# Algy/fast-slic

Hardware: AMD Instinct MI355X
Metric: megapixels/sec @10 iters (1280x720 & 4K, K=1600); % HBM roofline (higher is better)
Workload: dtype u8/u16/i32 (integer SLIC); 1 GPU; 1280x720 RGB, K=1600, 10 iters (configs[1]), 8 frames/GPU; frames_per_gpu=8, global_frames=8, slots_per_gpu=6, submissions_per_launch_group=up to 2 (dynamic batching of the pipeline), inputs=device-resident uint8 RGB, device int16 labels, parallelism=frames sharded across GPUs, no collective

## Files before the change

### fast_slic_amd/_binding.py

```python
import ctypes as C
import os
import subprocess
import threading

import numpy as np

ARCH_NAME = "hip/gfx950"
_HERE = os.path.dirname(os.path.abspath(__file__))
_LIB_PATH = os.path.join(_HERE, "libfslic_hip.so")

CLUSTER_DTYPE = np.dtype([
    ("y", "<f4"), ("x", "<f4"), ("r", "<f4"), ("g", "<f4"), ("b", "<f4"), ("a", "<f4"),
    ("number", "<u2"), ("is_active", "u1"), ("is_updatable", "u1"), ("num_members", "<u4"),
])
assert CLUSTER_DTYPE.itemsize == 32

FSLIC_OK, FSLIC_E_INVALID, FSLIC_E_UNSUPPORTED, FSLIC_E_HIP, FSLIC_E_INTERNAL = range(5)


class Params(C.Structure):
    _fields_ = [
        ("max_iter", C.c_int32), ("compactness", C.c_float), ("min_size_factor", C.c_float),
        ("subsample_stride", C.c_int32), ("convert_to_lab", C.c_int32),
        ("manhattan_spatial_dist", C.c_int32), ("preemptive", C.c_int32),
        ("preemptive_thres", C.c_float), ("num_threads", C.c_int32), ("debug_mode", C.c_int32),
        ("abi", C.c_int32), ("variant", C.c_int32), ("reserved", C.c_int32 * 4),
    ]


EXPORTS = [
    "fslic_hip_device_count", "fslic_hip_create", "fslic_hip_destroy", "fslic_hip_initialize_clusters",
    "fslic_hip_iterate", "fslic_hip_iterate_device", "fslic_hip_iterate_batch", "fslic_hip_submit_group",
    "fslic_hip_wait_group", "fslic_hip_rgb_to_lab",
    "fslic_hip_enforce_connectivity", "fslic_hip_enforce_connectivity_nodes", "fslic_hip_last_prelabels", "fslic_hip_last_timing_report",
    "fslic_hip_last_device_times", "fslic_hip_set_launch_timing", "fslic_hip_last_assign_loop", "fslic_hip_last_group_frames", "fslic_hip_last_path", "fslic_hip_last_launch_mode", "fslic_hip_group_done", "fslic_hip_last_error", "fslic_hip_version",
    "fslic_hip_get_connectivity", "fslic_hip_knn_connectivity", "fslic_hip_get_mask_density", "fslic_hip_cluster_density_to_mask",
    "fslic_hip_pipeline_submit", "fslic_hip_pipeline_drain", "fslic_hip_pipeline_batching", "fslic_hip_last_host_topk_frames",
    "fslic_hip_separate_pass_redos", "fslic_hip_uncovered_redos", "fslic_hip_copy_bandwidth", "fslic_hip_last_recorder_report",
    "fslic_hip_debug_lsc_state", "fslic_hip_debug_forms_seen", "fslic_hip_debug_forms_all",
    "fslic_hip_crf_new", "fslic_hip_crf_free", "fslic_hip_crf_copy", "fslic_hip_crf_get_params", "fslic_hip_crf_set_params",
    "fslic_hip_crf_set_compat", "fslic_hip_crf_get_compat", "fslic_hip_crf_num_classes", "fslic_hip_crf_first_time",
    "fslic_hip_crf_last_time", "fslic_hip_crf_num_frames", "fslic_hip_crf_pop_frame", "fslic_hip_crf_push_frame", "fslic_hip_crf_frame",
    "fslic_hip_crf_frame_time", "fslic_hip_crf_frame_set_clusters", "fslic_hip_crf_frame_get_clusters",
    "fslic_hip_crf_frame_set_connectivity", "fslic_hip_crf_frame_set_connectivity_csr", "fslic_hip_crf_frame_get_connectivity",
    "fslic_hip_crf_frame_set_mask", "fslic_hip_crf_frame_set_proba", "fslic_hip_crf_frame_set_unbiased", "fslic_hip_crf_frame_set_unary",
    "fslic_hip_crf_frame_get_unary", "fslic_hip_crf_frame_spatial_energy", "fslic_hip_crf_frame_temporal_energy",
    "fslic_hip_crf_frame_get_inferred", "fslic_hip_crf_frame_reset_inferred", "fslic_hip_crf_initialize", "fslic_hip_crf_inference",
    "fslic_hip_crf_expf_host", "fslic_hip_crf_expf_device",
    "fslic_hip_pool_workspace_size", "fslic_hip_pool", "fslic_hip_pool_finalize", "fslic_hip_unpool",
    "fslic_hip_rag_workspace_size", "fslic_hip_rag_accumulate", "fslic_hip_rag_compact",
    "fslic_hip_overlap_workspace_size", "fslic_hip_overlap_accumulate", "fslic_hip_overlap_compact", "fslic_hip_boundary_match",
    "fslic_hip_crf_tensor_workspace_size", "fslic_hip_crf_tensor_inference",
    "fslic_hip_crf_tensor_grad_workspace_size", "fslic_hip_crf_tensor_inference_saved", "fslic_hip_crf_tensor_backward",
    "fslic_hip_crf_tensor_energies", "fslic_hip_crf_tensor_energies_backward_workspace_size", "fslic_hip_crf_tensor_energies_backward",
    "fslic_hip_crf_tensor_inference_energies", "fslic_hip_crf_tensor_inference_saved_energies", "fslic_hip_crf_tensor_backward_energies",
]

_lib = None
_lib_lock = threading.Lock()

FORM_FAMILIES = {1: "blk", 2: "bin", 3: "pre", 4: "k32", 5: "generic", 6: "generic_rec", 7: "preempt_update"}
FORM_TABLES = {0: "notab", 1: "rowvec", 2: "rowvec16", 3: "2d", 4: "tabs16", 5: "lut"}


def form_name(code):
    code = int(code)
    family = FORM_FAMILIES.get(code & 15, "family%d" % (code & 15))
    if family == "preempt_update":
        return family + (" allpairs" if (code >> 18) & 1 else " lists")
    stride = (code >> 11) & 7
    words = [family]
    if (code >> 4) & 63:
        words.append("r%d" % ((code >> 4) & 63))
    words += ["fused" if (code >> 10) & 1 else "full", "s%d" % stride if stride else "srt",
              FORM_TABLES.get((code >> 14) & 7, "table%d" % ((code >> 14) & 7)), "nolab" if (code >> 17) & 1 else "lab"]
    return " ".join(words)


def _form_codes(fn, *extra):
    buf = (C.c_uint32 * 256)()
    n = int(fn(buf, 256, *extra))
    if n < 0 or n > 256:
        raise RuntimeError("the form record cannot be read (%d)" % n)
    return [int(buf[i]) for i in range(n)]


def forms_seen(clear=False):
    return {form_name(c) for c in _form_codes(load_library().fslic_hip_debug_forms_seen, 1 if clear else 0)}


def forms_all():
    return [form_name(c) for c in _form_codes(load_library().fslic_hip_debug_forms_all)]


def form_codes_all():
    return _form_codes(load_library().fslic_hip_debug_forms_all)


def build_library(force=False):
    csrc = os.path.join(_HERE, "csrc")
    args = ["make", "-s", "-C", csrc]
    if force:
        args.append("-B")
    subprocess.check_call(args)
    return _LIB_PATH


def _preload_torch_hip_runtime():
    import importlib.util
    import sys
    if "torch" in sys.modules:
        return
    try:
        spec = importlib.util.find_spec("torch")
    except (ImportError, ValueError):
        spec = None
    if spec is None or not spec.origin:
        return
    cand = os.path.join(os.path.dirname(spec.origin), "lib", "libamdhip64.so")
    if os.path.exists(cand):
        try:
            C.CDLL(cand, mode=C.RTLD_GLOBAL)
        except OSError:
            pass


def load_library():
    global _lib
    with _lib_lock:
        if _lib is not None:
            return _lib
        _preload_torch_hip_runtime()
        if not os.path.exists(_LIB_PATH):
            raise ImportError(
                "fast_slic_amd: %s is missing; build it with `python -c 'import __graft_entry__ as g; g.build()'` "
                "or `make -C fast_slic_amd/csrc` (there is no CPU fallback)" % _LIB_PATH)
        lib = C.CDLL(os.environ.get("FSLIC_LIB") or _LIB_PATH)
        vp, i32 = C.c_void_p, C.c_int
        lib.fslic_hip_device_count.restype = i32
        lib.fslic_hip_create.argtypes = [i32, i32, C.POINTER(vp)]
        lib.fslic_hip_destroy.argtypes = [vp]
        lib.fslic_hip_destroy.restype = None
        lib.fslic_hip_initialize_clusters.argtypes = [i32, i32, i32, vp, vp]
        lib.fslic_hip_iterate.argtypes = [vp, C.POINTER(Params), i32, i32, i32, vp, vp, vp]
        lib.fslic_hip_iterate_device.argtypes = [vp, i32, C.POINTER(Params), i32, i32, i32, vp, vp, vp]
        lib.fslic_hip_iterate_batch.argtypes = [vp, C.POINTER(Params), i32, i32, i32, i32, vp, vp, vp, i32]
        lib.fslic_hip_submit_group.argtypes = [vp, i32, C.POINTER(Params), i32, i32, i32, i32, vp, vp, vp]
        lib.fslic_hip_wait_group.argtypes = [vp, i32]
        lib.fslic_hip_pipeline_submit.argtypes = [vp, C.POINTER(Params), i32, i32, i32, i32, vp, vp, vp]
        lib.fslic_hip_pipeline_drain.argtypes = [vp, C.POINTER(C.c_double), C.POINTER(C.c_longlong), C.POINTER(C.c_longlong), C.POINTER(C.c_longlong)]
        lib.fslic_hip_pipeline_batching.argtypes = [vp, i32]
        lib.fslic_hip_last_host_topk_frames.argtypes = [vp, i32]
        lib.fslic_hip_separate_pass_redos.argtypes = [vp, i32]
        if hasattr(lib, "fslic_hip_uncovered_redos"):
            lib.fslic_hip_uncovered_redos.argtypes = [vp, i32]
        if hasattr(lib, "fslic_hip_copy_bandwidth"):
            lib.fslic_hip_copy_bandwidth.argtypes = [vp, C.c_size_t, i32, C.POINTER(C.c_double)]
        lib.fslic_hip_group_done.argtypes = [vp, i32]
        lib.fslic_hip_rgb_to_lab.argtypes = [vp, i32, i32, vp, i32, vp]
        lib.fslic_hip_enforce_connectivity.argtypes = [vp, vp, i32, i32, i32, i32]
        if hasattr(lib, "fslic_hip_enforce_connectivity_nodes"):
            lib.fslic_hip_enforce_connectivity_nodes.argtypes = [vp, vp, i32, i32, i32, i32, C.POINTER(C.c_uint32)]
        lib.fslic_hip_last_prelabels.argtypes = [vp, i32, vp]
        if hasattr(lib, "fslic_hip_debug_lsc_state"):
            lib.fslic_hip_debug_lsc_state.argtypes = [vp, i32, i32, i32, vp, vp]
        if hasattr(lib, "fslic_hip_debug_forms_seen"):
            lib.fslic_hip_debug_forms_seen.argtypes = [vp, i32, i32]
            lib.fslic_hip_debug_forms_all.argtypes = [vp, i32]
        lib.fslic_hip_last_timing_report.argtypes = [vp]
        lib.fslic_hip_last_timing_report.restype = C.c_char_p
        if hasattr(lib, "fslic_hip_last_recorder_report"):
            lib.fslic_hip_last_recorder_report.argtypes = [vp, C.POINTER(C.c_char_p), C.POINTER(C.c_size_t)]
        lib.fslic_hip_last_device_times.argtypes = [vp, i32, C.POINTER(C.c_float), C.POINTER(C.c_float)]
        lib.fslic_hip_set_launch_timing.argtypes = [vp, i32]
        lib.fslic_hip_last_assign_loop.argtypes = [vp, i32, C.POINTER(C.c_float), C.POINTER(C.c_double), C.POINTER(C.c_int)]
        lib.fslic_hip_last_group_frames.argtypes = [vp, i32]
        lib.fslic_hip_last_path.argtypes = [vp, i32]
        lib.fslic_hip_last_launch_mode.argtypes = [vp, i32]
        if hasattr(lib, "fslic_hip_lab_force_generic"):
            lib.fslic_hip_lab_force_generic.argtypes = [vp, i32]
        lib.fslic_hip_last_error.restype = C.c_char_p
        lib.fslic_hip_version.restype = C.c_char_p
        lib.fslic_hip_get_connectivity.argtypes = [vp, i32, i32, i32, vp, vp, vp]
        lib.fslic_hip_knn_connectivity.argtypes = [i32, i32, i32, vp, C.c_size_t, vp, vp]
        lib.fslic_hip_get_mask_density.argtypes = [vp, i32, i32, i32, vp, vp, vp, vp]
        lib.fslic_hip_cluster_density_to_mask.argtypes = [vp, i32, i32, i32, vp, vp, vp]
        if hasattr(lib, "fslic_hip_crf_new"):
            _declare_crf(lib)
        if hasattr(lib, "fslic_hip_pool"):
            _declare_pool(lib)
        if hasattr(lib, "fslic_hip_rag_accumulate"):
            _declare_rag(lib)
        if hasattr(lib, "fslic_hip_overlap_accumulate"):
            _declare_compare(lib)
        if hasattr(lib, "fslic_hip_crf_tensor_inference"):
            _declare_crf_tensor(lib)
        _lib = lib
        return lib


def _declare_crf(lib):
    vp, i32, sz, f32 = C.c_void_p, C.c_int, C.c_size_t, C.c_float
    for name, args in [
        ("new", [sz, sz, C.POINTER(vp)]), ("copy", [vp, C.POINTER(vp)]), ("get_params", [vp, vp]), ("set_params", [vp, vp]),
        ("set_compat", [vp, i32, f32]), ("get_compat", [vp, i32, C.POINTER(f32)]), ("num_classes", [vp, C.POINTER(sz), C.POINTER(sz)]),
        ("first_time", [vp]), ("last_time", [vp]), ("pop_frame", [vp]), ("push_frame", [vp, C.POINTER(vp)]),
        ("frame", [vp, i32, C.POINTER(vp)]), ("frame_time", [vp]), ("frame_set_clusters", [vp, vp]), ("frame_get_clusters", [vp, vp]),
        ("frame_set_connectivity", [vp, i32, vp, vp, sz]), ("frame_set_connectivity_csr", [vp, i32, vp, vp]),
        ("frame_get_connectivity", [vp, vp, vp]), ("frame_set_mask", [vp, vp, f32]), ("frame_set_proba", [vp, vp]),
        ("frame_set_unbiased", [vp]), ("frame_set_unary", [vp, vp]), ("frame_get_unary", [vp, vp]),
        ("frame_spatial_energy", [vp, i32, i32, C.POINTER(f32)]), ("frame_temporal_energy", [vp, vp, i32, C.POINTER(f32)]),
        ("frame_get_inferred", [vp, vp]), ("frame_reset_inferred", [vp]), ("initialize", [vp]), ("inference", [vp, vp, sz]),
        ("expf_host", [vp, vp, sz, i32]), ("expf_device", [vp, vp, vp, sz]),
    ]:
        f = getattr(lib, "fslic_hip_crf_" + name)
        f.argtypes = args
        f.restype = i32
    lib.fslic_hip_crf_free.argtypes = [vp]
    lib.fslic_hip_crf_free.restype = None
    lib.fslic_hip_crf_num_frames.argtypes = [vp]
    lib.fslic_hip_crf_num_frames.restype = sz


def _declare_pool(lib):
    vp, i32 = C.c_void_p, C.c_int
    lib.fslic_hip_pool_workspace_size.argtypes = [i32, i32, i32, i32, C.POINTER(C.c_size_t)]
    lib.fslic_hip_pool.argtypes = [i32, vp, i32, i32, i32, i32, i32, i32, vp, vp, i32, vp, C.c_size_t]
    lib.fslic_hip_pool_finalize.argtypes = [i32, vp, i32, i32, i32, i32, vp, C.c_size_t, vp, vp, vp]
    lib.fslic_hip_unpool.argtypes = [i32, vp, i32, i32, i32, i32, i32, vp, vp, i32, vp, C.c_float, vp]
    for name in ("pool_workspace_size", "pool", "pool_finalize", "unpool"):
        getattr(lib, "fslic_hip_" + name).restype = i32


def _declare_rag(lib):
    vp, i32, i64, sz = C.c_void_p, C.c_int, C.c_longlong, C.c_size_t
    lib.fslic_hip_rag_workspace_size.argtypes = [i32, i32, i32, i64, C.POINTER(sz)]
    lib.fslic_hip_rag_accumulate.argtypes = [i32, vp, i32, i32, i32, i32, i32, vp, i32, vp, i32, i64, vp, sz]
    lib.fslic_hip_rag_compact.argtypes = [i32, vp, i32, i32, i64, vp, sz, vp, vp, vp, i64]
# ... 108 lines not shown
        _check(load_library().fslic_hip_get_connectivity(self._h, H, W, int(K), ptr, num.ctypes.data, nb.ctypes.data))
        return num, nb

    def get_mask_density(self, clusters, labels, mask, H, W):
        lp, k1 = self._plane(labels, np.uint16)
        mp, k2 = self._plane(mask, np.uint8)
        cl = np.ascontiguousarray(clusters)
        dens = np.zeros(cl.shape[0], np.uint8)
        _check(load_library().fslic_hip_get_mask_density(self._h, H, W, cl.shape[0], cl.ctypes.data, lp, mp, dens.ctypes.data))
        return dens

    def cluster_density_to_mask(self, labels, densities, H, W, out=None):
        lp, k1 = self._plane(labels, np.uint16)
        d = np.ascontiguousarray(densities, dtype=np.uint8)
        if out is None:
            res = np.empty((H, W), np.uint8)
            op = C.c_void_p(res.ctypes.data)
        else:
            res, op = out, C.c_void_p(int(out))
        _check(load_library().fslic_hip_cluster_density_to_mask(self._h, H, W, d.shape[0], lp, d.ctypes.data, op))
        return res

    def iterate(self, image, clusters, params):
        H, W, _ = image.shape
        labels = np.empty((H, W), np.uint16)
        _check(load_library().fslic_hip_iterate(self._h, C.byref(params), H, W, clusters.shape[0],
                                                image.ctypes.data, clusters.ctypes.data, labels.ctypes.data))
        return labels

    def iterate_device(self, d_rgb_ptr, d_labels_ptr, H, W, clusters, params, slot=0):
        _check(load_library().fslic_hip_iterate_device(self._h, int(slot), C.byref(params), H, W, clusters.shape[0],
                                                       C.c_void_p(d_rgb_ptr), clusters.ctypes.data, C.c_void_p(d_labels_ptr)))

    def iterate_batch(self, rgb_ptrs, cluster_arrays, label_ptrs, H, W, params, device_ptrs):
        n = len(rgb_ptrs)
        K = cluster_arrays[0].shape[0]
        PA = C.c_void_p * n
        a_rgb = PA(*[C.c_void_p(int(p)) for p in rgb_ptrs])
        a_cl = PA(*[C.c_void_p(c.ctypes.data) for c in cluster_arrays])
        a_lab = PA(*[C.c_void_p(int(p)) for p in label_ptrs])
        _check(load_library().fslic_hip_iterate_batch(self._h, C.byref(params), H, W, K, n,
                                                      C.cast(a_rgb, C.c_void_p), C.cast(a_cl, C.c_void_p),
                                                      C.cast(a_lab, C.c_void_p), int(bool(device_ptrs))))

    @staticmethod
    def pointer_array(ptrs):
        PA = C.c_void_p * len(ptrs)
        return PA(*[C.c_void_p(int(p)) for p in ptrs])

    def submit_group(self, slot, a_rgb, a_clusters, a_labels, n, H, W, K, params):
        _check(load_library().fslic_hip_submit_group(self._h, int(slot), C.byref(params), H, W, K, n,
                                                     C.cast(a_rgb, C.c_void_p), C.cast(a_clusters, C.c_void_p),
                                                     C.cast(a_labels, C.c_void_p)))

    def wait_group(self, slot):
        _check(load_library().fslic_hip_wait_group(self._h, int(slot)))

    def pipeline_submit(self, a_rgb, a_clusters, a_labels, n, H, W, K, params):
        _check(load_library().fslic_hip_pipeline_submit(self._h, C.byref(params), H, W, K, n,
                                                        C.cast(a_rgb, C.c_void_p), C.cast(a_clusters, C.c_void_p),
                                                        C.cast(a_labels, C.c_void_p)))

    def pipeline_batching(self, max_frames_per_group):
        _check(load_library().fslic_hip_pipeline_batching(self._h, int(max_frames_per_group)))

    def pipeline_drain(self):
        ms, g, f, h = C.c_double(), C.c_longlong(), C.c_longlong(), C.c_longlong()
        _check(load_library().fslic_hip_pipeline_drain(self._h, C.byref(ms), C.byref(g), C.byref(f), C.byref(h)))
        return {"device_ms": ms.value, "groups": g.value, "frames": f.value, "host_topk_frames": h.value}

    def last_host_topk_frames(self, slot=0):
        return int(load_library().fslic_hip_last_host_topk_frames(self._h, int(slot)))

    def separate_pass_redos(self):
        return sum(int(load_library().fslic_hip_separate_pass_redos(self._h, s)) for s in range(self.n_slots))

    def uncovered_redos(self, slot=None):
        lib = load_library()
        if not hasattr(lib, "fslic_hip_uncovered_redos"):
            return 0
        slots = range(self.n_slots) if slot is None else [int(slot)]
        return sum(int(lib.fslic_hip_uncovered_redos(self._h, s)) for s in slots)

    def copy_bandwidth(self, nbytes=1 << 30, reps=5):
        v = C.c_double()
        _check(load_library().fslic_hip_copy_bandwidth(self._h, C.c_size_t(int(nbytes)), int(reps), C.byref(v)))
        return v.value

    def group_done(self, slot):
        return load_library().fslic_hip_group_done(self._h, int(slot)) != 0

    def last_launch_mode(self, slot=0):
        return int(load_library().fslic_hip_last_launch_mode(self._h, int(slot)))

    def last_prelabels(self, H, W, slot=0):
        out = np.empty((H, W), np.uint16)
        _check(load_library().fslic_hip_last_prelabels(self._h, int(slot), out.ctypes.data))
        return out

    def debug_lsc_state(self, K, z=0, slot=0):
        means, cfeat = np.empty(10, np.float32), np.empty((int(K), 10), np.float32)
        _check(load_library().fslic_hip_debug_lsc_state(self._h, int(slot), int(z), int(K), means.ctypes.data, cfeat.ctypes.data))
        return means, cfeat

    def last_timing_report(self):
        return load_library().fslic_hip_last_timing_report(self._h).decode("utf-8")

    def last_recorder_report(self):
        p, n = C.c_char_p(), C.c_size_t()
        _check(load_library().fslic_hip_last_recorder_report(self._h, C.byref(p), C.byref(n)))
        return C.string_at(p, n.value) if n.value else b""

    def last_device_times(self, slot=0):
        t, f = C.c_float(), C.c_float()
        _check(load_library().fslic_hip_last_device_times(self._h, int(slot), C.byref(t), C.byref(f)))
        return t.value, f.value

    def set_launch_timing(self, on):
        _check(load_library().fslic_hip_set_launch_timing(self._h, int(bool(on))))

    def last_assign_loop(self, slot=0):
        ms, px, n = C.c_float(), C.c_double(), C.c_int()
        _check(load_library().fslic_hip_last_assign_loop(self._h, int(slot), C.byref(ms), C.byref(px), C.byref(n)))
        return ms.value, px.value, n.value

    def last_group_frames(self, slot=0):
        return load_library().fslic_hip_last_group_frames(self._h, int(slot))

    def last_path(self, slot=0):
        return load_library().fslic_hip_last_path(self._h, int(slot))

    def lab_force_generic(self, on):
        _check(load_library().fslic_hip_lab_force_generic(self._h, int(bool(on))))


_default_engines = {}
_engine_lock = threading.Lock()


DEFAULT_ENGINE_SLOTS = 8


def default_engine(device=0):
    with _engine_lock:
        e = _default_engines.get(device)
        if e is None:
            e = Engine(device, DEFAULT_ENGINE_SLOTS)
            _default_engines[device] = e
        return e


def device_count():
    return load_library().fslic_hip_device_count()


def is_supported_arch(arch_name):
    return arch_name == ARCH_NAME


def get_supported_archs():
    return [ARCH_NAME]


def make_params(max_iter, compactness, min_size_factor, subsample_stride, convert_to_lab=True,
                manhattan_spatial_dist=True, preemptive=False, preemptive_thres=0.05, num_threads=-1,
                debug_mode=False, variant=0):
# ... 202 lines not shown
```

### fast_slic_amd/csrc/arena.cpp

```cpp
#include "engine_internal.h"

#include <algorithm>
#include <cmath>

namespace fslic {

void free_slot(Slot& s) {
    for (auto& g : s.graphs) { if (g.exec) hipGraphExecDestroy(g.exec); if (g.graph) hipGraphDestroy(g.graph); }
    s.graphs.clear();
    for (auto& e : s.ev) if (e) hipEventDestroy(e);
    for (auto& e : s.ev_it) if (e) hipEventDestroy(e);
    if (s.st) hipStreamDestroy(s.st);
    s = Slot();
}

int prepare(fslic_engine* e, Slot& s, int H, int W, int K, int S, int G) {
    const size_t N = (size_t)H * W;
    const int sh = [&] { int v = 2; while ((1 << v) < S) v++; return v; }();
    const int ncx = (W + (1 << sh) - 1) >> sh, ncy = (H + (1 << sh) - 1) >> sh;
    const size_t ncell = (size_t)ncx * ncy;
    const size_t P = (size_t)(2 * S + 1);
    if (G < s.cap_frames && s.keyH == H && s.keyW == W && s.keyK == K) G = s.cap_frames;

    int rc;
    if ((rc = s.h_cl.reserve((size_t)G * 4 * K)) || (rc = s.h_misc.reserve((size_t)kStatusWords * kMaxGroup)) ||
        (rc = s.h_lut.reserve(kLutMaxWords)) || (rc = s.h_tab.reserve(3 * kTabMaxBytes / sizeof(uint16_t))) ||
        (rc = s.h_patchf.reserve(P * P)) || (rc = s.h_patch.reserve(P * P)))
        return rc;

    size_t off = 0;
    auto take = [&](size_t bytes) { size_t o = off; off = align_up(off + bytes, 256); return o; };
    const size_t o_patch = take(P * P * 2);
    const size_t o_lut = take(kLutMaxWords * 4);
    const size_t o_tab = take(3 * kTabMaxBytes);
    const size_t o_patchf = take(P * P * 4);
    const size_t shared_bytes = off;
    off = 0;
    const size_t o_lab = take(N * 4), o_labels = take(N * 2);
    const size_t o_cl = take((size_t)K * 4 * 8);
    const size_t o_clf = take((size_t)K * 8 * 4);
    const int pre_cw = (W + 2 * S - 1) / (2 * S), pre_ch = (H + 2 * S - 1) / (2 * S);
    const size_t o_pre = take(((size_t)K * 2 + (size_t)pre_cw * pre_ch + 16) * 4);
    auto pow2ceil = [](int v) { int p2 = 1; while (p2 < v) p2 <<= 1; return p2; };
    const int nbx = pow2ceil(2 * S / 64 + 2), nby = pow2ceil(2 * S / 16 + 2);
    const size_t o_cpart = take((size_t)K * nbx * nby * 6 * 4);
    const size_t o_zero = off;
    const size_t o_sums = take((size_t)K * 6 * 4), o_sums1 = take((size_t)K * 6 * 4);
    const size_t o_cc0 = take(ncell * 4), o_cc1 = take(ncell * 4);
    const size_t o_misc = take(256);
    const size_t o_arrive = take((size_t)K * 4);
    const size_t zero_bytes = off - o_zero;
    const size_t o_ci0 = take(ncell * kCellCap * sizeof(ClusterRec)), o_ci1 = take(ncell * kCellCap * sizeof(ClusterRec));
    const size_t o_ov0 = take((size_t)K * sizeof(ClusterRec)), o_ov1 = take((size_t)K * sizeof(ClusterRec)), o_ov2 = take((size_t)K * sizeof(ClusterRec));
    const size_t ntiles = (size_t)((W + kCcaTile - 1) / kCcaTile) * ((H + kCcaTileH - 1) / kCcaTileH);
    const size_t TT = (size_t)kCcaTilePx;
    const size_t NP = ntiles * TT;
    const size_t o_lid = take(N * 2), o_nrec = take(NP * 16), o_narea = take(NP * 4);
    const size_t o_nfinal = take(NP * 2), o_vedge = take(ntiles * 2 * kCcaTileH * 4), o_roots = take(NP * 4);
    const size_t o_candl = take(ntiles * TT * 4), o_canda = take(ntiles * TT * 4);
    const size_t o_keepl = take((size_t)K * 4), o_keepb = take((size_t)K * 2);
    const size_t o_rgb = take(N * 3), o_out = take(N * 2);
    const size_t frame_bytes = off;
    const size_t total = shared_bytes + frame_bytes * (size_t)G;

    if ((rc = s.arena.reserve(total))) return rc;
    s.cap_frames = G;
    s.frame_bytes = frame_bytes;
    char* b = s.arena + shared_bytes;
    FrameDev& f = s.f;
    f.frame_bytes = frame_bytes;
    f.H = H; f.W = W; f.N = (int)N; f.K = K; f.S = S; f.T = 2 * S + 32; f.T_rcp = 0xFFFFFFFFu / (uint32_t)f.T;
    f.cs_shift = sh; f.ncx = ncx; f.ncy = ncy; f.ncell = (int)ncell;
    f.lab = (uint32_t*)(b + o_lab);
    f.labels = (uint16_t*)(b + o_labels);
    uint32_t* cl = (uint32_t*)(b + o_cl);
    f.cl_yx = cl; f.cl_lab = cl + K; f.cl_n = cl + 2 * (size_t)K; f.cl_moved = cl + 3 * (size_t)K; f.cl_tag = cl + 4 * (size_t)K;
    f.cl_shadow = cl + 5 * (size_t)K;
    f.cl_f = nullptr;
    f.cl_upd = f.cl_act = f.cell_act = f.pre_flags = nullptr;
    f.pre_cw = pre_cw; f.pre_ch = pre_ch;
    s.d_pre = (uint32_t*)(b + o_pre);
    s.d_clf = (float*)(b + o_clf);
    s.d_yx_alt[0] = cl + 6 * (size_t)K; s.d_yx_alt[1] = cl + 7 * (size_t)K;
    f.cl_yx_out = s.d_yx_alt[0];
    f.cpart = (uint32_t*)(b + o_cpart); f.cpart_ns = nbx * nby; f.nbx = nbx;
    f.sums[0] = (uint32_t*)(b + o_sums); f.sums[1] = (uint32_t*)(b + o_sums1);
    f.cell_cnt[0] = (uint32_t*)(b + o_cc0); f.cell_cnt[1] = (uint32_t*)(b + o_cc1);
    uint32_t* misc = (uint32_t*)(b + o_misc);
    s.d_misc = misc;
    f.ovf_cnt[0] = misc + kStSpill0; f.ovf_cnt[1] = misc + kStSpill1; f.err_flag = misc + kStFlags; f.ovf_cnt[2] = misc + kStSpill2;
    f.cl_arrive = (uint32_t*)(b + o_arrive);
    f.cell_items[0] = (ClusterRec*)(b + o_ci0); f.cell_items[1] = (ClusterRec*)(b + o_ci1);
    f.ovf_items[0] = (ClusterRec*)(b + o_ov0); f.ovf_items[1] = (ClusterRec*)(b + o_ov1); f.ovf_items[2] = (ClusterRec*)(b + o_ov2);
    s.d_patch = (uint16_t*)(s.arena + o_patch);
    f.patch2d = s.d_patch;
    s.d_lut = (uint32_t*)(s.arena + o_lut);
    s.d_tab = (uint16_t*)(s.arena + o_tab);
    s.d_patchf = (float*)(s.arena + o_patchf);
    s.pf_variant = -1;
    s.zero_block = b + o_zero; s.zero_bytes = zero_bytes;
    CcaDev& c = s.c;
    c.frame_bytes = frame_bytes;
    c.H = H; c.W = W; c.N = (int)N; c.K = K;
    c.tiles_x = (W + kCcaTile - 1) / kCcaTile;
    c.lid = (uint16_t*)(b + o_lid); c.nrec = (uint4*)(b + o_nrec); c.narea = (uint32_t*)(b + o_narea);
    c.nfinal = (uint16_t*)(b + o_nfinal); c.vedge = (uint32_t*)(b + o_vedge); c.roots = (uint32_t*)(b + o_roots);
    c.counters = misc + kStCca;
    c.cand_leader = (int32_t*)(b + o_candl); c.cand_area = (uint32_t*)(b + o_canda);
#if defined(FSLIC_LAB) && FSLIC_LAB == 4
    f.lab_stamps = c.cand_area;
#endif
    s.d_keep_leader = (int32_t*)(b + o_keepl); s.d_keep_label = (uint16_t*)(b + o_keepb);
    s.d_rgb_stage = (uint8_t*)(b + o_rgb); s.d_out_stage = (uint16_t*)(b + o_out);
    s.keyH = H; s.keyW = W; s.keyK = K;
    s.sp_valid = false;
    (void)e;
    if (knobs().poison) HIPCHK(hipMemsetAsync(s.arena, 0xA5, total, s.st));
    s.stamp_block = b + o_ci0; s.stamp_bytes = o_ov0 - o_ci0;
    HIPCHK(hipMemset2DAsync(s.stamp_block, frame_bytes, 0, s.stamp_bytes, (size_t)G, s.st));
    return FSLIC_OK;
}

int ensure_prepared(fslic_engine* e, Slot& s, int H, int W, int K, int S, int G) {
    G = std::max(G, std::min(e->reserve_frames.load(), (int)kMaxGroup));
    if (s.keyH == H && s.keyW == W && s.keyK == K && s.cap_frames >= G) return FSLIC_OK;
    HIPCHK(hipStreamSynchronize(s.st));
    return prepare(e, s, H, W, K, S, G);
}

int prepare_lsc(Slot& s, int H, int W, int K, int S, int G, float compactness) {
    const size_t lut_floats = 1024 + 2 * (size_t)W + 2 * (size_t)H;
    if (s.lsc_H != H || s.lsc_W != W || s.lsc_K != K || s.lsc_G < G) {
        G = std::max(G, (s.lsc_H == H && s.lsc_W == W && s.lsc_K == K) ? s.lsc_G : 0);
        size_t off = 0;
        auto take = [&](size_t bytes) { size_t o = off; off = align_up(off + bytes, 256); return o; };
        const size_t o_lut = take(lut_floats * 4);
        const size_t shared_bytes = off;
        off = 0;
        const size_t o_hist = take(768 * 4), o_extra = take((size_t)K * kLscExPitch * 8);
        const size_t zero_bytes = off - o_hist;
        const size_t o_means = take(64), o_cfeat = take((size_t)K * kLscCfPitch * 4);
        const size_t frame_bytes = off, total = shared_bytes + frame_bytes * (size_t)G;
        int rc;
        if ((rc = s.lsc_arena.reserve(total)) || (rc = s.h_lsc_lut.reserve(lut_floats))) return rc;
        char* b = s.lsc_arena + shared_bytes;
        LscDev& l = s.l;
        l.frame_bytes = frame_bytes;
        l.hist = (uint32_t*)(b + o_hist); l.extra = (long long*)(b + o_extra);
        l.means = (float*)(b + o_means); l.cfeat = (float*)(b + o_cfeat);
        const float* lut = (const float*)(s.lsc_arena + o_lut);
        l.lut_color = lut; l.lut_x = lut + 1024; l.lut_y = lut + 1024 + 2 * (size_t)W;
        s.lsc_zero = b + o_hist; s.lsc_zero_bytes = zero_bytes; s.lsc_frame_bytes = frame_bytes;
        s.lsc_H = H; s.lsc_W = W; s.lsc_K = K; s.lsc_G = G;
        s.lsc_S = 0;
        if (knobs().poison) HIPCHK(hipMemsetAsync(s.lsc_arena, 0xA5, total, s.st));
    }
    if (s.lsc_S != S || s.lsc_compactness != compactness) {
        const float C_color = 20.0f;
        const float PI = 3.1415926f, halfPI = PI / 2;
        const float ratio = compactness / 100.0f;
        const float C_spatial = C_color * ratio;
        float* t = s.h_lsc_lut;
        for (int X = 0; X < 256; X++) {
            const float theta = halfPI * (X / 255.0f);
            const float cosine = (float)cos((double)theta), sine = (float)sin((double)theta);
            t[512 + X] = C_color * cosine * 2.55f;
            t[768 + X] = C_color * sine * 2.55f;
            t[X] = (float)((double)C_color * cos((double)theta));
            t[256 + X] = (float)((double)C_color * sin((double)theta));
        }
        float* tx = t + 1024;
        float* ty = tx + 2 * (size_t)W;
        const float step = halfPI / S;
        for (int i = 0; i < W; i++) {
            const float theta = i * step;
            tx[i] = (float)((double)C_spatial * cos((double)theta));
            tx[W + i] = (float)((double)C_spatial * sin((double)theta));
        }
        for (int i = 0; i < H; i++) {
            const float theta = i * step;
            ty[i] = (float)((double)C_spatial * cos((double)theta));
            ty[H + i] = (float)((double)C_spatial * sin((double)theta));
        }
        HIPCHK(hipMemcpyAsync(const_cast<float*>(s.l.lut_color), t, lut_floats * 4, hipMemcpyHostToDevice, s.st));
        const double f_max = std::max({(double)C_color, (double)C_color * 2.55, (double)fabsf(C_spatial)});
        const double w_max = 2.0 * C_color * C_color + 4.0 * (C_color * 2.55) * (C_color * 2.55) + 4.0 * (double)C_spatial * C_spatial;
        int bits_f = 20, bits_w = 12;
        while (bits_f > 0 && 1024.0 * f_max * ldexp(1.0, bits_f) >= 2147483648.0) bits_f--;
        const double w_bias = ceil(4.0 * (double)C_spatial * C_spatial);
        while (bits_w > 0 && 1024.0 * (w_max + w_bias) * ldexp(1.0, bits_w) >= 4294967296.0) bits_w--;
        s.l.blk_bias_w = (float)w_bias;
        s.l.blk_fix_f = (float)ldexp(1.0, bits_f); s.l.blk_fix_w = (float)ldexp(1.0, bits_w);
        s.l.blk_shift_f = 20 - bits_f; s.l.blk_shift_w = 12 - bits_w;
        s.lsc_S = S; s.lsc_compactness = compactness;
    }
    return FSLIC_OK;
}

}
```

### fast_slic_amd/csrc/capi.cpp

```cpp
#include "engine_internal.h"
#include "crf.h"
#include "forms.h"

#include <algorithm>
#include <cstdio>
#include <cstdlib>
#include <cstring>
#include <mutex>

using namespace fslic;

static_assert(sizeof(fslic_cluster) == 32, "Cluster ABI (src/fast-slic-common.h:10-23)");

extern "C" {

const char* fslic_hip_last_error(void) { return last_error().c_str(); }
const char* fslic_hip_version(void) { return "fast_slic_amd 0.3 (gfx950)"; }

int fslic_hip_device_count(void) {
    int n = 0;
    if (hipGetDeviceCount(&n) != hipSuccess) return 0;
    return n;
}

int fslic_hip_create(int device, int n_slots, fslic_engine** out) {
    if (!out) return fail(FSLIC_E_INVALID, "out is NULL");
    *out = nullptr;
    if (n_slots < 1 || n_slots > 64) return fail(FSLIC_E_INVALID, "n_slots must be in [1, 64]");
    int n = 0;
    HIPCHK(hipGetDeviceCount(&n));
    if (device < 0 || device >= n) return fail(FSLIC_E_HIP, "no such HIP device");
    HIPCHK(hipSetDevice(device));
    const HostTables& ht = host_tables();
    fslic_engine* e = new fslic_engine();
    e->device = device;
    e->group_size = knobs().group_size;
    e->slots.resize(n_slots);
    for (auto& s : e->slots) {
        if (hipStreamCreateWithFlags(&s.st, hipStreamNonBlocking) != hipSuccess) { fslic_hip_destroy(e); return fail(FSLIC_E_HIP, "hipStreamCreate failed"); }
        for (auto& ev : s.ev)
            if (hipEventCreate(&ev) != hipSuccess) { fslic_hip_destroy(e); return fail(FSLIC_E_HIP, "hipEventCreate failed"); }
        for (auto& ev : s.ev_it)
            if (hipEventCreate(&ev) != hipSuccess) { fslic_hip_destroy(e); return fail(FSLIC_E_HIP, "hipEventCreate failed"); }
        if (s.d_ptrs.reserve(2 * kMaxGroup) || s.h_ptrs.reserve(2 * kMaxGroup) ||
            s.d_gen.reserve(64) || hipMemset(s.d_gen, 0, 256) != hipSuccess) { fslic_hip_destroy(e); return fail(FSLIC_E_HIP, "pointer table allocation failed"); }
    }
    if (e->d_gamma.reserve(sizeof ht.gamma / sizeof ht.gamma[0]) || e->d_labtbl.reserve(sizeof ht.lab / sizeof ht.lab[0])) { fslic_hip_destroy(e); return fail(FSLIC_E_HIP, "hipMalloc(tables) failed"); }
    if (hipMemcpy(e->d_gamma, ht.gamma, sizeof ht.gamma, hipMemcpyHostToDevice) != hipSuccess ||
        hipMemcpy(e->d_labtbl, ht.lab, sizeof ht.lab, hipMemcpyHostToDevice) != hipSuccess) { fslic_hip_destroy(e); return fail(FSLIC_E_HIP, "table upload failed"); }
    e->tables.gamma = e->d_gamma;
    e->tables.labtbl = e->d_labtbl;
    for (int i = 0; i < 9; i++) e->tables.cb[i] = ht.cb[i];
    *out = e;
    return FSLIC_OK;
}

void fslic_hip_destroy(fslic_engine* e) {
    if (!e) return;
    hipSetDevice(e->device);
    for (auto& s : e->slots) stop_slot_thread(e, s);
    for (auto& s : e->slots) {
        if (s.st) hipStreamSynchronize(s.st);
        free_slot(s);
    }
    delete e;
}

static int iterate_on(fslic_engine* e, Slot& s, const fslic_params* p, int H, int W, int K,
                      const uint8_t* d_rgb, fslic_cluster* clusters, uint16_t* d_labels) {
    GroupJob job;
    int rc = fill_job(job, p, H, W, K, 1, &d_rgb, &clusters, &d_labels);
    if (rc) return rc;
    s.launch_timing = e->launch_timing;
    rc = run_group(e, s, job, p->debug_mode != 0);
    if (rc) return rc;
    std::string report;
    rc = make_recorder_report(s, report);
    if (rc) { drain_failed(s); return rc; }
    set_thread_timing_report(make_timing_report(s));
    set_thread_recorder_report(std::move(report));
    return FSLIC_OK;
}

int fslic_hip_iterate_device(fslic_engine* e, int slot, const fslic_params* p, int H, int W, int K,
                             const uint8_t* d_rgb, fslic_cluster* clusters, uint16_t* d_labels) {
    if (!e) return fail(FSLIC_E_INVALID, "engine is NULL");
    if (slot < 0 || slot >= (int)e->slots.size()) return fail(FSLIC_E_INVALID, "slot out of range");
    HIPCHK(hipSetDevice(e->device));
    SlotLease lease(e);
    const int rc = lease.take(slot);
    return rc ? rc : iterate_on(e, e->slots[slot], p, H, W, K, d_rgb, clusters, d_labels);
}

int fslic_hip_iterate(fslic_engine* e, const fslic_params* p, int H, int W, int K, const uint8_t* rgb,
                      fslic_cluster* clusters, uint16_t* labels) {
    if (!e) return fail(FSLIC_E_INVALID, "engine is NULL");
    if (!rgb || !labels || !clusters) return fail(FSLIC_E_INVALID, "NULL pointer argument");
    HIPCHK(hipSetDevice(e->device));
    int S = 0;
    int rc = validate(p, H, W, K, S);
    if (rc) return rc;
    SlotLease lease(e);
    rc = lease.take();
    if (rc) return rc;
    Slot& s = e->slots[lease.slot];
    const size_t N = (size_t)H * W;
    rc = ensure_prepared(e, s, H, W, K, S, 1);
    if (rc) return rc;
    const double t0 = knobs().host_timing ? now_us() : 0.0;
    HIPCHK(hipMemcpyAsync(s.d_rgb_stage, rgb, N * 3, hipMemcpyHostToDevice, s.st));
    const double t1 = knobs().host_timing ? now_us() : 0.0;
    rc = iterate_on(e, s, p, H, W, K, s.d_rgb_stage, clusters, s.d_out_stage);
    if (rc) return rc;
    const double t2 = s.t_begun_us, t3 = knobs().host_timing ? now_us() : 0.0;
    HIPCHK(hipMemcpyAsync(labels, s.d_out_stage, N * 2, hipMemcpyDeviceToHost, s.st));
    HIPCHK(hipStreamSynchronize(s.st));
    if (knobs().host_timing)
        fprintf(stderr, "[fslic host] iterate: frame in %.1f us, group begin %.1f, group finish (wait + write-back) %.1f, labels out %.1f (device %.1f us)\n",
                t1 - t0, t2 - t1, t3 - t2, now_us() - t3, s.total_ms * 1e3);
    return FSLIC_OK;
}

int fslic_hip_last_recorder_report(fslic_engine* e, const char** report, size_t* length) {
    (void)e;
    if (!report || !length) return fail(FSLIC_E_INVALID, "NULL pointer argument");
    const std::string& r = thread_recorder_report();
    *report = r.c_str();
// ... 53 lines not shown
                break;
            }
        Slot& s = e->slots[si];
        GroupJob& job = jobs[(size_t)(first / G)];
        if (!device_ptrs) {
            rc = ensure_prepared(e, s, H, W, K, S, n);
            if (rc) return bail(rc);
            for (int i = 0; i < n; i++) {
                if (hipMemcpyAsync(s.at(s.d_rgb_stage, i), rgb[first + i], N * 3, hipMemcpyHostToDevice, s.st) != hipSuccess)
                    return bail(fail(FSLIC_E_HIP, "frame upload failed"));
                job.d_rgb[i] = s.at(s.d_rgb_stage, i);
                job.d_out[i] = s.at(s.d_out_stage, i);
            }
        }
        s.launch_timing = e->launch_timing;
        inflight.push_back({si, first, n});
        rc = group_begin(e, s, job);
        if (rc) return bail(rc);
    }
    while (!inflight.empty()) {
        const Pending pd = inflight.front();
        inflight.erase(inflight.begin());
        rc = finish_one(pd);
        if (rc) return bail(rc);
    }
    if (n_frames > 0) set_thread_timing_report(make_timing_report(e->slots[0]));
    release_all_slots(e);
    return FSLIC_OK;
}

int fslic_hip_last_prelabels(fslic_engine* e, int slot, uint16_t* prelabels) {
    if (!e || !prelabels) return fail(FSLIC_E_INVALID, "NULL pointer argument");
    if (slot < 0 || slot >= (int)e->slots.size()) return fail(FSLIC_E_INVALID, "slot out of range");
    HIPCHK(hipSetDevice(e->device));
    SlotLease lease(e);
    int rc = lease.take(slot);
    if (rc) return rc;
    Slot& s = e->slots[slot];
    if (!s.have_pre || s.keyH == 0) return fail(FSLIC_E_INVALID, "no frame has been processed on this slot");
    HIPCHK(hipMemcpy(prelabels, s.f.labels, (size_t)s.f.N * 2, hipMemcpyDeviceToHost));
    return FSLIC_OK;
}

int fslic_hip_debug_lsc_state(fslic_engine* e, int slot, int z, int K, float* means10, float* cfeat) {
    if (!e || !means10 || !cfeat) return fail(FSLIC_E_INVALID, "NULL pointer argument");
    if (slot < 0 || slot >= (int)e->slots.size()) return fail(FSLIC_E_INVALID, "slot out of range");
    HIPCHK(hipSetDevice(e->device));
    SlotLease lease(e);
    int rc = lease.take(slot);
    if (rc) return rc;
    Slot& s = e->slots[slot];
    if (!s.have_pre || s.keyH == 0 || s.p.variant != FSLIC_VARIANT_LSC) return fail(FSLIC_E_INVALID, "the slot's last group was not an LSC one");
    if (z < 0 || z >= s.nframes) return fail(FSLIC_E_INVALID, "no such frame in the slot's last group");
    if (K != s.K) return fail(FSLIC_E_INVALID, "K is not that of the slot's last group");
    HIPCHK(hipStreamSynchronize(s.st));
    LscDev l = s.l;
    l.select(z);
    HIPCHK(hipMemcpy(means10, l.means, sizeof(float) * kLscFeat, hipMemcpyDeviceToHost));
    HIPCHK(hipMemcpy2D(cfeat, sizeof(float) * kLscFeat, l.cfeat, sizeof(float) * kLscCfPitch, sizeof(float) * kLscFeat, (size_t)s.K, hipMemcpyDeviceToHost));
    return FSLIC_OK;
}

const char* fslic_hip_last_timing_report(fslic_engine* e) { return e ? thread_timing_report().c_str() : ""; }

int fslic_hip_last_device_times(fslic_engine* e, int slot, float* total_ms, float* full_assign_ms) {
    if (!e || slot < 0 || slot >= (int)e->slots.size()) return fail(FSLIC_E_INVALID, "bad engine/slot");
    if (total_ms) *total_ms = e->slots[slot].total_ms;
    if (full_assign_ms) *full_assign_ms = e->slots[slot].fa_ms;
    return FSLIC_OK;
}

int fslic_hip_set_launch_timing(fslic_engine* e, int on) {
    if (!e) return fail(FSLIC_E_INVALID, "engine is NULL");
    e->launch_timing = on != 0;
    return FSLIC_OK;
}

int fslic_hip_lab_force_generic(fslic_engine* e, int on) {
    if (!e) return fail(FSLIC_E_INVALID, "engine is NULL");
    e->lab_force_generic.store(on != 0);
    return FSLIC_OK;
}

int fslic_hip_last_assign_loop(fslic_engine* e, int slot, float* sum_ms, double* visited_px, int* launches) {
    if (!e || slot < 0 || slot >= (int)e->slots.size()) return fail(FSLIC_E_INVALID, "bad engine/slot");
    const Slot& s = e->slots[slot];
    if (sum_ms) *sum_ms = s.assign_loop_ms;
    if (visited_px) *visited_px = s.assign_loop_px;
    if (launches) *launches = s.n_timed_iters;
    return FSLIC_OK;
}

int fslic_hip_last_group_frames(fslic_engine* e, int slot) {
    if (!e || slot < 0 || slot >= (int)e->slots.size()) return -1;
    return e->slots[slot].nframes;
}

int fslic_hip_last_launch_mode(fslic_engine* e, int slot) {
    if (!e || slot < 0 || slot >= (int)e->slots.size()) return -1;
    return e->slots[slot].last_launch_mode;
}

int fslic_hip_last_path(fslic_engine* e, int slot) {
    if (!e || slot < 0 || slot >= (int)e->slots.size()) return -1;
    return e->slots[slot].last_path;
}

int fslic_hip_last_host_topk_frames(fslic_engine* e, int slot) {
    if (!e || slot < 0 || slot >= (int)e->slots.size()) return -1;
    return e->slots[slot].n_host_topk;
}

int fslic_hip_separate_pass_redos(fslic_engine* e, int slot) {
    if (!e || slot < 0 || slot >= (int)e->slots.size()) return -1;
    return __atomic_load_n(&e->slots[slot].n_separate_redo, __ATOMIC_RELAXED);
}

int fslic_hip_uncovered_redos(fslic_engine* e, int slot) {
    if (!e || slot < 0 || slot >= (int)e->slots.size()) return -1;
    return __atomic_load_n(&e->slots[slot].n_uncovered_redo, __ATOMIC_RELAXED);
}

int fslic_hip_debug_forms_seen(uint32_t* codes, int cap, int clear) {
    if (cap < 0 || (cap > 0 && !codes)) return -1;
    return fslic::forms_seen(codes, cap, clear != 0);
}

int fslic_hip_debug_forms_all(uint32_t* codes, int cap) {
    if (cap < 0 || (cap > 0 && !codes)) return -1;
    const int na = fslic::assign_forms(codes, cap);
    return na + fslic::preempt_forms(codes + std::min(na, cap), std::max(cap - na, 0));
}

#define CRF_LOCK(crf) std::lock_guard<std::mutex> crf_lock__((crf)->mu)

static fslic_crf_frame* crf_frame_at(fslic_crf* crf, int time) {
    if (crf->frames.empty()) return nullptr;
    const long long d = (long long)time - crf->frames.front()->time;
    if (d < 0 || d >= (long long)crf->frames.size()) return nullptr;
    return crf->frames[(size_t)d].get();
}
static void crf_touch_unary(fslic_crf_frame* f) { f->dirty_unary = true; }
static void crf_touch_q(fslic_crf_frame* f) { f->q_on_device = false; f->dirty_q = true; }

int fslic_hip_crf_new(size_t num_classes, size_t num_nodes, fslic_crf** out) {
    if (!out) return fail(FSLIC_E_INVALID, "out is NULL");
    *out = nullptr;
    if (num_classes == 0 || num_nodes == 0) return fail(FSLIC_E_INVALID, "num_classes and num_nodes must be positive");
    if (num_classes >= (1ull << 31) || num_nodes >= (1ull << 31) || (unsigned long long)num_classes * num_nodes >= (1ull << 31))
        return fail(FSLIC_E_INVALID, "num_classes * num_nodes must be below 2^31");
    fslic_crf* crf = new fslic_crf();
    crf->C = num_classes;
    crf->K = num_nodes;
    crf->compat.assign(num_classes, 1.0f);
    crf->params.spatial_w = 10; crf->params.temporal_w = 10;
    crf->params.spatial_srgb = 13; crf->params.temporal_srgb = 13;
    crf->params.spatial_sxy = 80;
    crf->params.spatial_smooth_w = 0; crf->params.spatial_smooth_sxy = 3;
    *out = crf;
    return FSLIC_OK;
}

void fslic_hip_crf_free(fslic_crf* crf) {
    if (!crf) return;
    crf_release_device(crf);
    delete crf;
}

int fslic_hip_crf_copy(fslic_crf* crf, fslic_crf** out) {
    if (!crf || !out) return fail(FSLIC_E_INVALID, "NULL pointer argument");
    *out = nullptr;
    CRF_LOCK(crf);
    for (auto& f : crf->frames) {
        int rc = crf_pull_q(crf, f.get());
        if (rc) return rc;
    }
    fslic_crf* c = new fslic_crf();
    c->C = crf->C; c->K = crf->K; c->next_time = crf->next_time; c->compat = crf->compat; c->params = crf->params;
    for (auto& f : crf->frames) {
        std::unique_ptr<fslic_crf_frame> g(new fslic_crf_frame());
        g->parent = c; g->time = f->time; g->clusters = f->clusters; g->edges = f->edges; g->unaries = f->unaries; g->q = f->q;
        c->frames.push_back(std::move(g));
    }
    *out = c;
    return FSLIC_OK;
}

int fslic_hip_crf_get_params(fslic_crf* crf, fslic_crf_params* out) {
    if (!crf || !out) return fail(FSLIC_E_INVALID, "NULL pointer argument");
    CRF_LOCK(crf);
    *out = crf->params;
    return FSLIC_OK;
}

int fslic_hip_crf_set_params(fslic_crf* crf, const fslic_crf_params* params) {
    if (!crf || !params) return fail(FSLIC_E_INVALID, "NULL pointer argument");
    CRF_LOCK(crf);
    crf->params = *params;
    return FSLIC_OK;
}

int fslic_hip_crf_set_compat(fslic_crf* crf, int cls, float compat_value) {
    if (!crf) return fail(FSLIC_E_INVALID, "NULL pointer argument");
// ... 279 lines not shown
```

### fast_slic_amd/csrc/cca.hip

```cpp
#include "device_common.h"

namespace fslic {

constexpr uint32_t kNoAdopt = 0xFFFFFFFFu;
static __device__ __forceinline__ uint32_t* n_parent(const CcaDev& c, uint32_t n) { return reinterpret_cast<uint32_t*>(c.nrec + n); }
static __device__ __forceinline__ uint32_t n_leader(const CcaDev& c, uint32_t n) { return reinterpret_cast<const uint32_t*>(c.nrec + n)[1]; }
static __device__ __forceinline__ uint32_t n_local(const CcaDev& c, uint32_t n) { return reinterpret_cast<const uint32_t*>(c.nrec + n)[2]; }
static __device__ __forceinline__ uint32_t n_adopt(const CcaDev& c, uint32_t n) { return reinterpret_cast<const uint32_t*>(c.nrec + n)[3]; }

static __device__ __forceinline__ uint32_t lds_ld(uint32_t* p) {
    return __hip_atomic_load(p, __ATOMIC_RELAXED, __HIP_MEMORY_SCOPE_WORKGROUP);
}
static __device__ __forceinline__ void lds_st(uint32_t* p, uint32_t v) {
    __hip_atomic_store(p, v, __ATOMIC_RELAXED, __HIP_MEMORY_SCOPE_WORKGROUP);
}
typedef unsigned long long u64;
static __device__ __forceinline__ uint32_t lane_left0(uint32_t v) { return (uint32_t)__builtin_amdgcn_update_dpp(0, (int)v, 0x138 , 0xF, 0xF, true); }
static __device__ __forceinline__ uint32_t lane_left_or(uint32_t old, uint32_t v) { return (uint32_t)__builtin_amdgcn_update_dpp((int)old, (int)v, 0x138, 0xF, 0xF, false); }
static __device__ __forceinline__ uint32_t rank_in(u64 m) { return __builtin_amdgcn_mbcnt_hi((uint32_t)(m >> 32), __builtin_amdgcn_mbcnt_lo((uint32_t)m, 0u)); }
static __device__ __forceinline__ uint32_t* lds_at(uint32_t* base, uint32_t off) { return reinterpret_cast<uint32_t*>(reinterpret_cast<char*>(base) + off); }
static __device__ __forceinline__ void ldsb_union(uint32_t* par, uint32_t a, uint32_t b) {
    for (;;) {
        for (;;) {
            const uint32_t pa = lds_ld(lds_at(par, a)), pb = lds_ld(lds_at(par, b));
// ... 804 lines not shown
    if (cap > kSelCap) cap = kSelCap;
    const size_t lds = (3 * (size_t)cap + 3 * (size_t)kSelBuckets) * sizeof(uint32_t);
    static_assert(kSelBins <= 3 * kSelBuckets, "the selection histogram reuses the ranking buckets");
    static std::atomic<int> attr_state[64];
    if (!max_dynamic_lds_on_this_device(k_cca_select, (int)((3 * (size_t)kSelCap + 3 * (size_t)kSelBuckets) * sizeof(uint32_t)), attr_state)) {
        while (cap > 1024 && (3 * (size_t)cap + 3 * (size_t)kSelBuckets) * sizeof(uint32_t) > 64 * 1024) cap >>= 1;
        const size_t lds_small = (3 * (size_t)cap + 3 * (size_t)kSelBuckets) * sizeof(uint32_t);
        launch(k_cca_select, dim3(nframes), dim3(1024), lds_small, st, c, cap);
        return;
    }
    launch(k_cca_select, dim3(nframes), dim3(1024), lds, st, c, cap);
}

__global__ __launch_bounds__(256) void k_cca_reset_final(CcaDev c) {
    const uint32_t n = c.counters[0];
    for (uint32_t i = blockIdx.x * blockDim.x + threadIdx.x; i < n; i += gridDim.x * blockDim.x) {
        const uint32_t r = c.roots[i];
        if (*n_parent(c, r) == r) c.nfinal[r] = 0xFFFFu;
    }
}
__global__ void k_cca_set_kept(CcaDev c, const int32_t* __restrict__ leaders, const uint16_t* __restrict__ labels, int n) {
    const int i = blockIdx.x * blockDim.x + threadIdx.x;
    if (i < n) c.nfinal[node_of(c, (uint32_t)leaders[i])] = labels[i];
}
__global__ void k_cca_gather_area(CcaDev c) {
    const uint32_t M = c.counters[1];
    for (uint32_t i = blockIdx.x * blockDim.x + threadIdx.x; i < M; i += gridDim.x * blockDim.x) c.cand_area[i] = c.narea[node_of(c, (uint32_t)c.cand_leader[i])];
}
void launch_cca_gather_area(const CcaDev& c, hipStream_t st) {
    launch(k_cca_gather_area, dim3(64), dim3(256), 0, st, c);
}

void launch_cca_set_kept(const CcaDev& c, const int32_t* d_leaders, const uint16_t* d_labels, int n, hipStream_t st) {
    launch(k_cca_reset_final, dim3(root_pass_blocks(c)), dim3(256), 0, st, c);
    if (n <= 0) return;
    launch(k_cca_set_kept, dim3((n + 255) / 256), dim3(256), 0, st, c, d_leaders, d_labels, n);
}

static __device__ __forceinline__ uint32_t chase_final(const CcaDev& c, uint32_t g) {
    const uint32_t W = (uint32_t)c.W;
    for (;;) {
        const uint32_t cur = n_leader(c, g);
        if (cur == 0) return 0u;
        uint32_t a = n_adopt(c, g);
        if (a == kNoAdopt) {
            const uint32_t t = (cur % W > 0) ? cur - 1 : cur - W;
            a = node_of(c, t);
        }
        g = *n_parent(c, a);
        const uint32_t f = __hip_atomic_load(c.nfinal + g, __ATOMIC_RELAXED, __HIP_MEMORY_SCOPE_AGENT);
        if (f != 0xFFFFu) return f;
    }
}

__global__ __launch_bounds__(256) void k_cca_chain(CcaDev c) {
    c.select(blockIdx.y);
    const uint32_t i0 = blockIdx.x * blockDim.x + threadIdx.x;
    const uint32_t r0 = c.roots[i0];
    const uint32_t n = c.counters[0];
    const uint32_t gstride = gridDim.x * blockDim.x;
    for (uint32_t i = i0; i < n; i += gstride) {
        const uint32_t r = i == i0 ? r0 : c.roots[i];
        const uint32_t g = *n_parent(c, r);
        uint32_t f = __hip_atomic_load(c.nfinal + g, __ATOMIC_RELAXED, __HIP_MEMORY_SCOPE_AGENT);
        if (f == 0xFFFFu) f = chase_final(c, g);
        __hip_atomic_store(c.nfinal + r, (uint16_t)f, __ATOMIC_RELAXED, __HIP_MEMORY_SCOPE_AGENT);
    }
}

static __device__ __forceinline__ uint32_t wave_max_u32(uint32_t v) {
#define FSLIC_DPP_MAX(ctrl) v = max(v, (uint32_t)__builtin_amdgcn_update_dpp(0, (int)v, ctrl, 0xF, 0xF, false))
    FSLIC_DPP_MAX(0xB1); FSLIC_DPP_MAX(0x4E); FSLIC_DPP_MAX(0x141); FSLIC_DPP_MAX(0x140);
#undef FSLIC_DPP_MAX
    return max(max((uint32_t)__builtin_amdgcn_readlane((int)v, 0), (uint32_t)__builtin_amdgcn_readlane((int)v, 16)),
               max((uint32_t)__builtin_amdgcn_readlane((int)v, 32), (uint32_t)__builtin_amdgcn_readlane((int)v, 48)));
}

__global__ __launch_bounds__(256) void k_cca_relabel(CcaDev c, ExportDev ex, int relabel_blocks) {
    const int z = blockIdx.y;
    if ((int)blockIdx.x >= relabel_blocks) {
        const size_t d = (size_t)z * ex.frame_bytes;
        const uint32_t* yx = ex.yx_cur; const uint32_t* rest = ex.lab_n_moved; const uint32_t* misc = ex.misc0;
        FrameDev::adv(yx, d); FrameDev::adv(rest, d); FrameDev::adv(misc, d);
        uint32_t* out = ex.h_cl + (size_t)z * ex.h_stride;
        const int K = ex.K;
        for (int i = ((int)blockIdx.x - relabel_blocks) * blockDim.x + threadIdx.x; i < 4 * K; i += ((int)gridDim.x - relabel_blocks) * blockDim.x)
            out[i] = i < K ? yx[i] : rest[i - K];
        if ((int)blockIdx.x == relabel_blocks && threadIdx.x < kStatusWords) ex.h_misc[kStatusWords * (size_t)z + threadIdx.x] = misc[threadIdx.x];
        return;
    }
    c.select(z);
    constexpr int T = kCcaTile, TH = kCcaTileH;
    const int tiles_x = c.tiles_x, tiles_y = (c.H + TH - 1) / TH;
    const int ntiles = tiles_x * tiles_y;
    const int aligned8 = ((reinterpret_cast<uintptr_t>(c.out) & 7) == 0) ? 1 : 0;
    const bool vec = (c.W & 3) == 0 && aligned8;
    __shared__ __attribute__((aligned(16))) uint16_t s_fin[kCcaTilePx];
    __shared__ uint32_t s_max;
    for (int tile = blockIdx.x; tile < ntiles; tile += relabel_blocks) {
        const int ty = tile / tiles_x, tx = tile - ty * tiles_x;
        const uint16_t* __restrict__ gfin = c.nfinal + (size_t)tile * kCcaTilePx;
        const int x0 = tx * T + 4 * (int)(threadIdx.x & 15);
        const int r0 = (int)(threadIdx.x >> 4);
        if (tile != (int)blockIdx.x) __syncthreads();
        if (threadIdx.x == 0) s_max = 0u;
        __syncthreads();
        if (vec) {
            uint2 v[2];
            bool ok[2];
            uint32_t mx = 0;
#pragma unroll
            for (int h = 0; h < 2; ++h) {
                const int y = ty * TH + r0 + 16 * h;
                ok[h] = y < c.H && x0 < c.W;
                v[h] = make_uint2(0u, 0u);
                if (ok[h]) v[h] = *reinterpret_cast<const uint2*>(c.lid + (size_t)y * c.W + x0);
                mx = max(max(mx, max(v[h].x & 0xFFFFu, v[h].x >> 16)), max(v[h].y & 0xFFFFu, v[h].y >> 16));
            }
            mx = wave_max_u32(mx);
            if ((threadIdx.x & 63) == 0) atomicMax(&s_max, mx);
            __syncthreads();
            const uint32_t cnt = min(s_max + 1u, (uint32_t)kCcaTilePx);
            for (uint32_t i = threadIdx.x; i * 8u < cnt; i += 256u) reinterpret_cast<uint4*>(s_fin)[i] = reinterpret_cast<const uint4*>(gfin)[i];
            __syncthreads();
#pragma unroll
            for (int h = 0; h < 2; ++h) {
                if (!ok[h]) continue;
                const int y = ty * TH + r0 + 16 * h;
                uint2 o;
                o.x = (uint32_t)s_fin[v[h].x & 0xFFFFu] | ((uint32_t)s_fin[v[h].x >> 16] << 16);
                o.y = (uint32_t)s_fin[v[h].y & 0xFFFFu] | ((uint32_t)s_fin[v[h].y >> 16] << 16);
                st_stream(reinterpret_cast<uint2*>(c.out + (size_t)y * c.W + x0), o);
            }
        } else {
#pragma unroll
            for (int h = 0; h < 2; ++h) {
                const int y = ty * TH + r0 + 16 * h;
                if (y >= c.H) continue;
                for (int q = 0; q < 4; ++q) {
                    const int x = x0 + q;
                    if (x < c.W) st_stream(c.out + (size_t)y * c.W + x, gfin[c.lid[(size_t)y * c.W + x]]);
                }
            }
        }
    }
}

void launch_cca_phase2(const CcaDev& c, int nframes, hipStream_t st, const ExportDev* ex_) {
    launch(k_cca_chain, dim3(root_pass_blocks(c), nframes), dim3(256), 0, st, c);
    int blocks = c.tiles_x * ((c.H + kCcaTileH - 1) / kCcaTileH);
    const int cap = (16384 + nframes - 1) / nframes;
    if (blocks > cap) blocks = cap;
    if (blocks < 1) blocks = 1;
    ExportDev ex{};
    if (ex_) ex = *ex_;
    const int eb = ex.K > 0 ? (4 * ex.K + 1023) / 1024 : 0;
    launch(k_cca_relabel, dim3(blocks + eb, nframes), dim3(256), 0, st, c, ex, blocks);
}

}
```

### fast_slic_amd/csrc/engine_internal.h

```cpp
#pragma once
#include "kernels.h"
#include "launch.h"
#include "../../include/fslic_hip.h"

#include <algorithm>
#include <atomic>
#include <condition_variable>
#include <deque>
#include <cstdint>
#include <memory>
#include <mutex>
#include <string>
#include <thread>
#include <vector>

namespace fslic {

int fail(int code, const std::string& msg);
const std::string& last_error();
void set_last_error(const std::string& msg);

#define HIPCHK(expr)                                                                            \
    do {                                                                                        \
        hipError_t e__ = (expr);                                                                \
        if (e__ != hipSuccess)                                                                  \
            return ::fslic::fail(FSLIC_E_HIP, std::string(#expr) + ": " + hipGetErrorString(e__)); \
    } while (0)

inline int clampi(int v, int lo, int hi) { return v < lo ? lo : (v > hi ? hi : v); }
inline float clampf(float v, float lo, float hi) { return v < lo ? lo : (v > hi ? hi : v); }
inline size_t align_up(size_t v, size_t a) { return (v + a - 1) / a * a; }
double now_us();

template <class T, bool kDevice>
class Buffer {
    T* p_ = nullptr;
    size_t cap_ = 0;
public:
    Buffer() = default;
    Buffer(Buffer&& o) noexcept : p_(o.p_), cap_(o.cap_) { o.p_ = nullptr; o.cap_ = 0; }
    Buffer& operator=(Buffer&& o) noexcept { std::swap(p_, o.p_); std::swap(cap_, o.cap_); return *this; }
    ~Buffer() { release(); }
    operator T*() const { return p_; }
    T* get() const { return p_; }
    void release() {
        if (p_) (void)(kDevice ? hipFree(p_) : hipHostFree(p_));
        p_ = nullptr; cap_ = 0;
    }
    int reserve(size_t count) {
        if (p_ && cap_ >= count) return FSLIC_OK;
        release();
        const size_t bytes = std::max<size_t>(count * sizeof(T), 16);
        const hipError_t err = kDevice ? hipMalloc((void**)&p_, bytes) : hipHostMalloc((void**)&p_, bytes);
        if (err != hipSuccess) {
            p_ = nullptr;
            return fail(FSLIC_E_HIP, std::string(kDevice ? "hipMalloc(" : "hipHostMalloc(") + std::to_string(bytes) + " bytes): " + hipGetErrorString(err));
        }
        cap_ = count;
        return FSLIC_OK;
    }
};
template <class T> using Pinned = Buffer<T, false>;
template <class T> using Device = Buffer<T, true>;

struct GroupJob {
    fslic_params p{};
    int H = 0, W = 0, K = 0, n = 0;
    const uint8_t* d_rgb[kMaxGroup] = {};
    fslic_cluster* clusters[kMaxGroup] = {};
    uint16_t* d_out[kMaxGroup] = {};
    void append(const GroupJob& j) {
        for (int i = 0; i < j.n; i++) { d_rgb[n + i] = j.d_rgb[i]; clusters[n + i] = j.clusters[i]; d_out[n + i] = j.d_out[i]; }
        n += j.n;
    }
};

struct Knobs {
    int group_size;
    bool use_graphs, poison, host_timing;
    int fuse_bin;
    int blocks_scale;
};
const Knobs& knobs();

constexpr int kDenseCap = 8192;
constexpr size_t kTabMaxBytes = 40960;
constexpr size_t kLutMaxWords = 12288;

struct HostTables {
    uint16_t gamma[256];
    uint16_t lab[8194];
    int cb[9];
};
const HostTables& host_tables();

struct Slot {
    hipStream_t st = nullptr;
    hipEvent_t ev[6] = {nullptr, nullptr, nullptr, nullptr, nullptr, nullptr};
    static constexpr int kMaxTimedIters = 16;
    hipEvent_t ev_it[2 * kMaxTimedIters] = {};
    int n_timed_iters = 0;
    float assign_loop_ms = 0;
    double assign_loop_px = 0;
    Device<char> arena;
    int cap_frames = 0;
    size_t frame_bytes = 0;
    FrameDev f{};
    CcaDev c{};
    char* zero_block = nullptr;
    size_t zero_bytes = 0;
    char* stamp_block = nullptr;
    size_t stamp_bytes = 0;
    uint32_t* d_misc = nullptr;
    uint32_t* d_yx_alt[2] = {nullptr, nullptr};
    uint8_t* d_rgb_stage = nullptr;
    uint16_t* d_out_stage = nullptr;
    int32_t* d_keep_leader = nullptr;
    uint16_t* d_keep_label = nullptr;
    Device<void*> d_ptrs;
    Pinned<void*> h_ptrs;
    uint16_t* d_patch = nullptr;
    uint32_t* d_lut = nullptr;
    Pinned<uint32_t> h_lut;
    uint16_t* d_tab = nullptr;
    Pinned<uint16_t> h_tab;
    Pinned<uint32_t> h_cl;
    Pinned<uint32_t> h_misc;
    Pinned<uint16_t> h_patch;
    Pinned<int32_t> h_cand_leader;
    Pinned<uint32_t> h_cand_area;
    Device<uint32_t> d_gen;
    uint64_t gen_host = 0;
    uint32_t gen_span_prev = 0;
    uint32_t gen_step = 0;
    int keyH = 0, keyW = 0, keyK = 0;
    struct GraphEntry {
        std::vector<unsigned char> key;
        hipGraph_t graph = nullptr;
        hipGraphExec_t exec = nullptr;
        int seen = 0;
        bool failed = false;
    };
    std::vector<GraphEntry> graphs;
    int last_launch_mode = 0;
    bool launch_timing = false;
    double t_begun_us = 0;
    bool nap_wait = false;
    double recent_wait_us[4] = {1e30, 1e30, 1e30, 1e30};
    unsigned recent_wait_i = 0;
    unsigned long long recent_wait_key = 0;
    int H = 0, W = 0, K = 0, S = 0;
    int nframes = 0;
    bool generic = false;
    fslic_params p{};
    fslic_cluster* clusters[kMaxGroup] = {};
    float total_ms = 0, fa_ms = 0, lab_ms = 0, loop_ms = 0, cca_ms = 0;
    int last_path = 0;
    int n_host_topk = 0;
    int n_separate_redo = 0;
    int n_uncovered_redo = 0;
    bool store_labels = false;
    bool store_seen_credit = false;
    int store_H = 0, store_W = 0, store_K = 0;
    fslic_params store_p{};
    bool have_pre = false;
    bool busy = false;
    bool pending = false;
    int wanted = 0;
    struct Async {
        std::thread worker;
        bool has_job = false, done = false, quit = false;
        GroupJob job;
        int rc = 0;
        std::string err;
        bool from_queue = false;
        int jobs = 0;
    };
    std::unique_ptr<Async> async;
    uint32_t* d_pre = nullptr;
    Pinned<uint32_t> h_upd;
    float* d_clf = nullptr;
    Pinned<float> h_clf;
    float* d_patchf = nullptr;
    Pinned<float> h_patchf;
    int pf_S = 0, pf_shift = -1, pf_variant = -1;
    float pf_compactness = -1.0f;
    bool pf_manhattan = true;
    Device<char> lsc_arena;
    size_t lsc_frame_bytes = 0, lsc_zero_bytes = 0;
    char* lsc_zero = nullptr;
    LscDev l{};
    Pinned<float> h_lsc_lut;
    int lsc_H = 0, lsc_W = 0, lsc_K = 0, lsc_G = 0, lsc_S = 0;
    float lsc_compactness = -1.0f;
    bool sp_valid = false, sp_tiled_ok = false, sp_manhattan = true, sp_patch_uploaded = false;
    int sp_S = 0, sp_shift = 0, sp_stride = 0;
    float sp_compactness = 0.0f;
    bool recording = false;
    Device<char> d_rec;
    std::vector<fslic_cluster> rec_clusters;

    template <class T> T* at(T* p, int frame) const { return reinterpret_cast<T*>(reinterpret_cast<char*>(p) + (size_t)frame * frame_bytes); }
};

inline uint32_t* status(const Slot& s, int frame) { return s.h_misc + (size_t)kStatusWords * frame; }

inline void cluster_position(bool moved, uint32_t yx, const float* centroid, const fslic_cluster& in, int H, int W, float& y, float& x) {
    if (moved && centroid) { y = centroid[0]; x = centroid[1]; }
    else if (moved) { y = (float)(yx >> 16); x = (float)(yx & 0xFFFFu); }
    else { x = clampf(in.x, 0.0f, (float)(W - 1)); y = clampf(in.y, 0.0f, (float)(H - 1)); }
}

}

struct fslic_engine {
    int device = 0;
    int group_size = 8;
    bool launch_timing = false;
    std::vector<fslic::Slot> slots;
    fslic::Device<uint16_t> d_gamma, d_labtbl;
    fslic::LabTables tables{};
    std::mutex mu;
    std::condition_variable cv;
    std::condition_variable cv_work;
    int pipe_rc = 0;
    std::string pipe_err;
    double pipe_device_ms = 0;
    long long pipe_groups = 0, pipe_frames = 0, pipe_host_topk = 0;
    std::deque<fslic::GroupJob> pipe_q;
    int pipe_inflight = 0;
    int pipe_batch_frames = 0;
    bool pipe_gathering = false;
    double pipe_last_submit_us = 0;
    std::atomic<int> reserve_frames{0};
    int sync_waiters = 0;
    std::atomic<int> lab_force_generic{0};
};

extern "C" int fslic_hip_lab_force_generic(fslic_engine* e, int on);

namespace fslic {

int configure_spatial(Slot& s, int S, const fslic_params* p);
int configure_patchf(Slot& s, int S, const fslic_params* p);

void free_slot(Slot& s);
int prepare(fslic_engine* e, Slot& s, int H, int W, int K, int S, int G);
int ensure_prepared(fslic_engine* e, Slot& s, int H, int W, int K, int S, int G);
int prepare_lsc(Slot& s, int H, int W, int K, int S, int G, float compactness);

int validate(const fslic_params* p, int H, int W, int K, int& S);
int fill_job(GroupJob& j, const fslic_params* p, int H, int W, int K, int n,
             const uint8_t* const* d_rgb, fslic_cluster* const* clusters, uint16_t* const* d_out);
int check_job(const GroupJob& j, int& S);
int upload_ptrs(Slot& s, int n, const uint8_t* const* d_rgb, uint16_t* const* d_out);
CcaDev cca_view(const Slot& s, int i0, const uint16_t* d_in0, size_t in_stride, int K, int min_threshold);
void cca_enqueue(Slot& s, const CcaDev& c, int i0, int n, const ExportDev* ex = nullptr);
int cca_finish_group(Slot& s, int first, int n, const uint16_t* d_in0, size_t in_stride, int K, int thres);
int group_begin(fslic_engine* e, Slot& s, const GroupJob& job, bool record = false);
int group_finish(fslic_engine* e, Slot& s);
void drain_failed(Slot& s);
int run_group(fslic_engine* e, Slot& s, const GroupJob& job, bool record = false);
std::string make_timing_report(const Slot& s);
void set_thread_timing_report(const std::string& json);
const std::string& thread_timing_report();
int make_recorder_report(Slot& s, std::string& out);
void set_thread_recorder_report(std::string&& json);
const std::string& thread_recorder_report();

int acquire_slot(fslic_engine* e, int want, int& slot);
int acquire_all_slots(fslic_engine* e);
void release_slot(fslic_engine* e, int slot);
void release_all_slots(fslic_engine* e);
void stop_slot_thread(fslic_engine* e, Slot& s);
struct SlotLease {
    fslic_engine* e;
    int slot = -1;
    explicit SlotLease(fslic_engine* e_) : e(e_) {}
    int take(int want = -1) { return acquire_slot(e, want, slot); }
    ~SlotLease() { if (slot >= 0) release_slot(e, slot); }
};

}
```

### fast_slic_amd/csrc/group.cpp

```cpp
#include "engine_internal.h"
#include "forms.h"

#include <time.h>

#include <algorithm>
#include <charconv>
#include <chrono>
#include <cmath>
#include <cstdio>
#include <cstring>
#include <numeric>

namespace fslic {

double now_us() {
    return std::chrono::duration<double, std::micro>(std::chrono::steady_clock::now().time_since_epoch()).count();
}

int validate(const fslic_params* p, int H, int W, int K, int& S) {
    if (!p) return fail(FSLIC_E_INVALID, "params is NULL");
    static_assert(sizeof(fslic_params) == 64 && offsetof(fslic_params, abi) == 40 && offsetof(fslic_params, variant) == 44, "fslic_params layout (include/fslic_hip.h)");
    if (p->abi != FSLIC_PARAMS_ABI) return fail(FSLIC_E_INVALID, "fslic_params.abi != FSLIC_PARAMS_ABI: the caller was built against another layout of the struct (include/fslic_hip.h)");
    if (p->reserved[0] | p->reserved[1] | p->reserved[2] | p->reserved[3]) return fail(FSLIC_E_INVALID, "fslic_params.reserved must be 0");
    if (H <= 0 || W <= 0) return fail(FSLIC_E_INVALID, "H and W must be positive");
    if (H > 32767 || W > 32767) return fail(FSLIC_E_INVALID, "H and W must fit int16 (src/context.cpp:262)");
    if ((long long)H * W >= (1ll << 31)) return fail(FSLIC_E_INVALID, "H*W must fit int32");
    if (K <= 0 || K >= 65534) return fail(FSLIC_E_INVALID, "num_components must be in [1, 65533] (cfast_slic.pyx:24-27)");
    if (p->subsample_stride < 1 || p->subsample_stride > 255) return fail(FSLIC_E_INVALID, "subsample_stride must be in [1, 255]");
    if (p->max_iter < 0) return fail(FSLIC_E_INVALID, "max_iter must be >= 0");
    if (p->preemptive && !std::isfinite(p->preemptive_thres)) return fail(FSLIC_E_INVALID, "preemptive_thres must be finite");
    if (p->variant < FSLIC_VARIANT_SLIC || p->variant > FSLIC_VARIANT_REALDIST_NOQ) return fail(FSLIC_E_UNSUPPORTED, "unknown variant");
    if (!(p->compactness > 0.0f) || !std::isfinite(p->compactness)) return fail(FSLIC_E_INVALID, "compactness must be a positive finite number");
    S = (int)(int16_t)sqrt(H * W / K);
    if (S < 1) return fail(FSLIC_E_INVALID, "num_components exceeds the number of pixels (S == 0)");
    return FSLIC_OK;
}

int fill_job(GroupJob& j, const fslic_params* p, int H, int W, int K, int n,
             const uint8_t* const* d_rgb, fslic_cluster* const* clusters, uint16_t* const* d_out) {
    if (n < 1 || n > (int)kMaxGroup || !d_rgb || !clusters || !d_out) return fail(FSLIC_E_INVALID, "bad group arguments");
    if (!p) return fail(FSLIC_E_INVALID, "params is NULL");
    for (int i = 0; i < n; i++)
        if (reinterpret_cast<uintptr_t>(d_out[i]) & 1) return fail(FSLIC_E_INVALID, "d_labels[" + std::to_string(i) + "] is not 2-byte aligned");
    j.p = *p; j.H = H; j.W = W; j.K = K; j.n = n;
    for (int i = 0; i < n; i++) { j.d_rgb[i] = d_rgb[i]; j.clusters[i] = clusters[i]; j.d_out[i] = d_out[i]; }
    return FSLIC_OK;
}

int check_job(const GroupJob& j, int& S) {
    if (j.n < 1 || j.n > (int)kMaxGroup) return fail(FSLIC_E_INVALID, "bad group arguments");
    const int rc = validate(&j.p, j.H, j.W, j.K, S);
    if (rc) return rc;
    for (int i = 0; i < j.n; i++)
        if (!j.clusters[i] || !j.d_rgb[i] || !j.d_out[i]) return fail(FSLIC_E_INVALID, "NULL pointer argument");
    return FSLIC_OK;
}

void select_kept_sorted(const int32_t* leader, const uint32_t* area, uint32_t M, int K,
                        int32_t* keep_leader, uint16_t* keep_label, uint32_t& n_keep) {
    if ((size_t)K >= (size_t)M) {
        for (uint32_t i = 0; i < M; i++) { keep_leader[i] = leader[i]; keep_label[i] = (uint16_t)i; }
        n_keep = M;
        return;
    }
    std::vector<uint32_t> order(M);
    std::iota(order.begin(), order.end(), 0u);
    auto by_area = [&](uint32_t a, uint32_t b) { return area[a] > area[b]; };
    std::partial_sort(order.begin(), order.begin() + K, order.end(), by_area);
    std::vector<uint8_t> kept(M, 0);
    for (int i = 0; i < K; i++) kept[order[i]] = 1;
    uint32_t n = 0;
    for (uint32_t i = 0; i < M; i++)
        if (kept[i]) { keep_leader[n] = leader[i]; keep_label[n] = (uint16_t)n; n++; }
    n_keep = n;
}

CcaDev cca_view(const Slot& s, int i0, const uint16_t* d_in0, size_t in_stride, int K, int min_threshold) {
    CcaDev c = s.c;
    c.in = d_in0; c.in_stride = in_stride; c.K = K; c.min_threshold = min_threshold;
    c.outs = nullptr;
    c.out = nullptr;
    FrameDev::adv(c.in, (size_t)i0 * in_stride);
    const size_t d = (size_t)i0 * c.frame_bytes;
    FrameDev::adv(c.lid, d); FrameDev::adv(c.nrec, d); FrameDev::adv(c.narea, d);
    FrameDev::adv(c.nfinal, d); FrameDev::adv(c.vedge, d); FrameDev::adv(c.roots, d);
    FrameDev::adv(c.counters, d);
    FrameDev::adv(c.cand_leader, d); FrameDev::adv(c.cand_area, d);
    c.outs = reinterpret_cast<uint16_t* const*>(s.d_ptrs + kMaxGroup + i0);
    return c;
}

int upload_ptrs(Slot& s, int n, const uint8_t* const* d_rgb, uint16_t* const* d_out) {
    for (int i = 0; i < kMaxGroup; i++) {
        s.h_ptrs[i] = (i < n && d_rgb) ? const_cast<uint8_t*>(d_rgb[i]) : nullptr;
        s.h_ptrs[kMaxGroup + i] = (i < n && d_out) ? d_out[i] : nullptr;
    }
    HIPCHK(hipMemcpyAsync(s.d_ptrs, s.h_ptrs, sizeof(void*) * 2 * kMaxGroup, hipMemcpyHostToDevice, s.st));
    return FSLIC_OK;
}

void cca_enqueue(Slot& s, const CcaDev& c, int i0, int n, const ExportDev* ex) {
    (void)i0;
    launch_cca_phase1(c, n, s.st);
    launch_cca_select(c, n, s.st);
    launch_cca_phase2(c, n, s.st, ex);
}

int cca_finish_group(Slot& s, int first, int n, const uint16_t* d_in0, size_t in_stride, int K, int thres) {
    int n_slow = 0;
    for (int i = first; i < first + n; i++) n_slow += status(s, i)[kStSelect] == kSelectHost;
    if (n_slow == 0) return FSLIC_OK;
    for (int i = first; i < first + n && n_slow; i++) {
        const uint32_t* hm = status(s, i);
        if (hm[kStSelect] != kSelectHost) continue;
        const CcaDev c1 = cca_view(s, i, d_in0, in_stride, K, thres);
        int32_t* d_dl = s.at(s.c.cand_leader, i);
        uint32_t* d_da = s.at(s.c.cand_area, i);
        const uint32_t M = hm[kStCands];
        const size_t cap = std::max<size_t>((size_t)M * 2, 16384);
        int rc;
        if ((rc = s.h_cand_leader.reserve(cap)) || (rc = s.h_cand_area.reserve(cap))) return rc;
        launch_cca_gather_area(c1, s.st);
        HIPCHK(hipMemcpyAsync(s.h_cand_leader, d_dl, sizeof(int32_t) * M, hipMemcpyDeviceToHost, s.st));
        HIPCHK(hipMemcpyAsync(s.h_cand_area, d_da, sizeof(uint32_t) * M, hipMemcpyDeviceToHost, s.st));
        HIPCHK(hipStreamSynchronize(s.st));
        std::vector<uint32_t> order(M);
        std::iota(order.begin(), order.end(), 0u);
        std::sort(order.begin(), order.end(), [&](uint32_t a, uint32_t b) { return s.h_cand_leader[a] < s.h_cand_leader[b]; });
        int32_t* sl = s.h_cand_leader + M;
        uint32_t* sa = s.h_cand_area + M;
        for (uint32_t q = 0; q < M; q++) { sl[q] = s.h_cand_leader[order[q]]; sa[q] = s.h_cand_area[order[q]]; }
        int32_t* kl = s.h_cand_leader;
        uint16_t* kb = reinterpret_cast<uint16_t*>(s.h_cand_area.get());
        uint32_t n_keep = 0;
        select_kept_sorted(sl, sa, M, K, kl, kb, n_keep);
        int32_t* d_kl = s.at(s.d_keep_leader, i);
        uint16_t* d_kb = s.at(s.d_keep_label, i);
        if (n_keep) {
            HIPCHK(hipMemcpyAsync(d_kl, kl, sizeof(int32_t) * n_keep, hipMemcpyHostToDevice, s.st));
            HIPCHK(hipMemcpyAsync(d_kb, kb, sizeof(uint16_t) * n_keep, hipMemcpyHostToDevice, s.st));
        }
        launch_cca_set_kept(c1, d_kl, d_kb, (int)n_keep, s.st);
        launch_cca_phase2(c1, 1, s.st);
    }
    HIPCHK(hipStreamSynchronize(s.st));
    return FSLIC_OK;
}

void stage_group(fslic_engine* e, Slot& s, int i0, int n, bool timed) {
    const int H = s.H, W = s.W, K = s.K;
    for (int z = 0; z < n; z++) {
        const fslic_cluster* cl = s.clusters[i0 + z];
        uint32_t* h = s.h_cl + (size_t)(i0 + z) * 4 * K;
        for (int k = 0; k < K; k++) {
            const int y = clampi((int)cl[k].y, 0, H - 1), x = clampi((int)cl[k].x, 0, W - 1);
            h[k] = ((uint32_t)y << 16) | (uint32_t)x;
        }
    }
    if (s.p.variant == FSLIC_VARIANT_REALDIST_NOQ) {
        for (int z = 0; z < n; z++) {
            const fslic_cluster* cl = s.clusters[i0 + z];
            float* h = s.h_clf + (size_t)(i0 + z) * 8 * K;
            for (int k = 0; k < K; k++) {
                h[8 * k + 0] = clampf(cl[k].y, 0.0f, (float)(H - 1));
                h[8 * k + 1] = clampf(cl[k].x, 0.0f, (float)(W - 1));
                for (int q = 2; q < 8; q++) h[8 * k + q] = 0.0f;
            }
        }
    }
    if (timed) {
        s.n_timed_iters = 0; s.assign_loop_px = 0;
        const int stride = s.p.subsample_stride;
        int rem = 0;
        for (int it = 0; it < s.p.max_iter && s.launch_timing && it < Slot::kMaxTimedIters; it++) {
            s.n_timed_iters = it + 1;
            s.assign_loop_px += (double)visited_rows(H, rem, stride) * W * n;
            rem = (rem + 1) % stride;
        }
    }
}

static bool cluster_pass_fused(const FrameDev& f, const fslic_params& p, int n, int W, int H, bool generic, bool separate_cluster_pass) {
    const int stride = p.subsample_stride;
    const int assign_blocks = assign_blocks8(W, visited_rows(H, 0, stride), n);
#if defined(FSLIC_LAB) && FSLIC_LAB == 3
    const bool fuse_wanted = false;
    (void)assign_blocks;
#else
    const bool fuse_wanted = knobs().fuse_bin == 2 || (knobs().fuse_bin == 1 && assign_blocks <= kBlocksFuseBin);
#endif
    const bool plain_slic = p.variant == FSLIC_VARIANT_SLIC && p.preemptive == 0;
    const bool every_pass_has_rows = H >= stride;
    return fuse_wanted && !separate_cluster_pass && plain_slic && !generic && every_pass_has_rows && blk_kernel_applies(f, stride);
}

static bool label_free_allowed(const Slot& s) { return !s.store_labels; }

static int min_size_threshold(const Slot& s) { return (int)round((double)(s.S * s.S) * (double)s.p.min_size_factor); }

constexpr int kRecWords = 16;
struct RecLayout {
    size_t N, K, nsnap, dsize, dist_off, cl_off, bytes;
};
static RecLayout rec_layout(const Slot& s) {
    RecLayout L{};
    L.N = (size_t)s.H * s.W; L.K = (size_t)s.K; L.nsnap = (size_t)s.p.max_iter + 1;
    L.dsize = s.p.variant == FSLIC_VARIANT_SLIC ? 2 : 4;
    auto up = [](size_t v) { return (v + 255) & ~(size_t)255; };
    L.dist_off = up(L.nsnap * L.N * 2);
    L.cl_off = L.dist_off + up(L.nsnap * L.N * L.dsize);
    L.bytes = L.cl_off + up(L.nsnap * kRecWords * L.K * 4);
    return L;
}

int enqueue_frames(fslic_engine* e, Slot& s, int i0, int n, bool generic, bool timed, bool separate_cluster_pass = false, bool store_labels = false) {
    const fslic_params* p = &s.p;
    const int K = s.K, S = s.S;
    FrameDev f = s.f;
    f.rgbs = nullptr;
    f.select(i0);
    f.rgbs = reinterpret_cast<const uint8_t* const*>(s.d_ptrs + i0);
    const size_t fb = s.frame_bytes;

    const bool need_patch = generic || (p->preemptive != 0 && p->variant == FSLIC_VARIANT_SLIC && !blk_kernel_applies(f, p->subsample_stride));
    if ((p->preemptive != 0 || p->variant == FSLIC_VARIANT_REALDIST_NOQ || (need_patch && !s.sp_patch_uploaded)) && recording_unsupported()) return FSLIC_OK;
    if (need_patch && !s.sp_patch_uploaded) {
        HIPCHK(hipMemcpyAsync(s.d_patch, s.h_patch, (size_t)(2 * S + 1) * (2 * S + 1) * sizeof(uint16_t), hipMemcpyHostToDevice, s.st));
        s.sp_patch_uploaded = true;
    }
    const bool pre = p->preemptive != 0;
    if (pre) {
        uint32_t* base = s.at(s.d_pre, i0);
        f.cl_upd = base; f.cl_act = base + K; f.cell_act = base + 2 * (size_t)K; f.pre_flags = f.cell_act + (size_t)f.pre_cw * f.pre_ch;
        for (int z = 0; z < n; z++) {
            uint32_t* bz = s.at(s.d_pre, i0 + z);
            HIPCHK(hipMemsetD32Async((hipDeviceptr_t)bz, 2, (size_t)K, s.st));
            HIPCHK(hipMemsetD32Async((hipDeviceptr_t)(bz + 2 * (size_t)K + (size_t)f.pre_cw * f.pre_ch), 1, 1, s.st));
        }
    }
    const bool noq = p->variant == FSLIC_VARIANT_REALDIST_NOQ;
    if (noq) {
        f.cl_f = s.at(s.d_clf, i0);
        HIPCHK(hipMemcpy2DAsync(f.cl_f, fb, s.h_clf + (size_t)i0 * 8 * K, sizeof(float) * 8 * (size_t)K,
                                sizeof(float) * 8 * (size_t)K, (size_t)n, hipMemcpyHostToDevice, s.st));
    }

    if (timed) HIPCHK(hipEventRecord(s.ev[0], s.st));
    f.gen_base = s.d_gen;
    const bool fusebin = cluster_pass_fused(f, *p, n, s.W, s.H, generic, separate_cluster_pass);
    const bool lazy_labels = p->variant == FSLIC_VARIANT_SLIC && !generic && p->preemptive == 0 && !fusebin;
    const bool label_free = lazy_labels && !store_labels && label_free_allowed(s) && p->max_iter >= 1 && !s.recording && blk_kernel_applies(f, p->subsample_stride);
    launch_rgb_to_lab(f, n, p->convert_to_lab, e->tables, !lazy_labels, s.st, s.gen_step,
                      s.at(s.zero_block, i0), s.zero_bytes, f.cl_n, 2 * (size_t)K, s.h_cl + (size_t)i0 * 4 * K, 4 * (size_t)K);
    if (timed) HIPCHK(hipEventRecord(s.ev[1], s.st));
    f.gen_off = 1;
    PassGeom pg{};
    uint32_t* const yx_up = f.cl_yx;
    uint32_t* const yx_a = yx_up + 6 * (size_t)K;
    uint32_t* const yx_b = yx_up + 7 * (size_t)K;
    f.cl_yx = yx_up; f.cl_yx_out = yx_a;
    const int stride = p->subsample_stride;
    const bool lsc = p->variant == FSLIC_VARIANT_LSC;
    launch_bin_clusters(f, n, 0, 0, 0, pg, s.st);
    uint32_t* yx_cur = yx_a;
    int rem = 0;
    LscDev l = s.l;
    if (lsc) {
        l.select(i0);
        HIPCHK(clear_rows(s.lsc_zero + (size_t)i0 * s.lsc_frame_bytes, s.lsc_frame_bytes, s.lsc_zero_bytes, (size_t)n, s.st));
        launch_lsc_prepare(f, l, n, s.st);
    }
    const bool rec = s.recording && n == 1;
    const RecLayout rl = rec ? rec_layout(s) : RecLayout{};
    auto rec_dist = [&](int idx) -> void* { return rec ? s.d_rec + rl.dist_off + (size_t)idx * rl.N * rl.dsize : nullptr; };
    auto snapshot = [&](int idx, const uint32_t* yx) -> int {
        HIPCHK(hipMemcpyAsync(s.d_rec + (size_t)idx * rl.N * 2, f.labels, rl.N * 2, hipMemcpyDeviceToDevice, s.st));
        uint32_t* c = reinterpret_cast<uint32_t*>(s.d_rec + rl.cl_off) + (size_t)idx * kRecWords * K;
        const size_t kb = sizeof(uint32_t) * (size_t)K;
        HIPCHK(hipMemcpyAsync(c, yx, kb, hipMemcpyDeviceToDevice, s.st));
        HIPCHK(hipMemcpyAsync(c + K, f.cl_lab, kb, hipMemcpyDeviceToDevice, s.st));
        HIPCHK(hipMemcpyAsync(c + 2 * (size_t)K, f.cl_n, kb, hipMemcpyDeviceToDevice, s.st));
        HIPCHK(hipMemcpyAsync(c + 3 * (size_t)K, f.cl_moved, kb, hipMemcpyDeviceToDevice, s.st));
        if (pre) {
            HIPCHK(hipMemcpyAsync(c + 4 * (size_t)K, f.cl_upd, kb, hipMemcpyDeviceToDevice, s.st));
            HIPCHK(hipMemcpyAsync(c + 5 * (size_t)K, f.cl_act, kb, hipMemcpyDeviceToDevice, s.st));
        }
        if (noq) HIPCHK(hipMemcpyAsync(c + 6 * (size_t)K, f.cl_f, 8 * kb, hipMemcpyDeviceToDevice, s.st));
        return FSLIC_OK;
    };
    if (rec) {
        HIPCHK(hipMemsetAsync(s.d_rec + rl.dist_off, 0, rl.N * rl.dsize, s.st));
        if (p->max_iter > 0) {
            if (rl.dsize == 2) HIPCHK(hipMemsetAsync(rec_dist(1), 0xFF, (size_t)p->max_iter * rl.N * 2, s.st));
            else HIPCHK(hipMemsetD32Async((hipDeviceptr_t)rec_dist(1), 0x7F7FFFFFu, (size_t)p->max_iter * rl.N, s.st));
        }
        HIPCHK(hipMemsetAsync(s.d_rec + rl.cl_off, 0, rl.nsnap * kRecWords * rl.K * 4, s.st));
        const int rc = snapshot(0, yx_up);
        if (rc) return rc;
    }
    const bool rd = p->variant == FSLIC_VARIANT_REALDIST || p->variant == FSLIC_VARIANT_REALDIST_L2 || noq;
    const bool rd_l2 = p->variant == FSLIC_VARIANT_REALDIST_L2;
    float noq_coef = 1.0f / ((float)S / p->compactness);
    noq_coef *= (1 << (p->convert_to_lab ? 1 : 0));
    const bool noq_manhattan = p->manhattan_spatial_dist != 0;
    const float pre_l1_thres = std::max(roundf(2 * S * p->preemptive_thres), 1.0f);
    for (int it = 0; rd && it < p->max_iter; it++) {
        const bool tme = timed && s.launch_timing && it < Slot::kMaxTimedIters;
        f.cl_yx = yx_cur; f.cl_yx_out = (yx_cur == yx_a) ? yx_b : yx_a;
        if (tme) HIPCHK(hipEventRecord(s.ev_it[2 * it], s.st));
        float* const dist = static_cast<float*>(rec_dist(it + 1));
        if (noq) launch_noq_assign(f, noq_coef, noq_manhattan, n, rem, stride, it & 1, it & 1, true, s.st, dist);
        else launch_rd_assign(f, s.d_patchf, rd_l2, n, rem, stride, it & 1, it & 1, true, s.st, dist);
        if (tme) HIPCHK(hipEventRecord(s.ev_it[2 * it + 1], s.st));
        launch_member_sums(f, n, rem, stride, it & 1, noq ? 1 : 0, s.st);
        f.gen_off++;
        pg = PassGeom{};
        if (pre) launch_preempt_update(f, n, (it + 1) & 1, it & 1, false, pre_l1_thres, s.st);
        else launch_bin_clusters(f, n, 1, (it + 1) & 1, it & 1, pg, s.st);
        yx_cur = f.cl_yx_out;
        if (rec) { const int rc = snapshot(it + 1, yx_cur); if (rc) return rc; }
        rem = (rem + 1) % stride;
    }
    for (int it = 0; lsc && it < p->max_iter; it++) {
        const bool tme = timed && s.launch_timing && it < Slot::kMaxTimedIters;
        f.cl_yx = yx_cur; f.cl_yx_out = (yx_cur == yx_a) ? yx_b : yx_a;
        if (tme) HIPCHK(hipEventRecord(s.ev_it[2 * it], s.st));
        launch_lsc_assign(f, l, n, rem, stride, it & 1, it & 1, !pre, s.st, static_cast<float*>(rec_dist(it + 1)));
        if (tme) HIPCHK(hipEventRecord(s.ev_it[2 * it + 1], s.st));
        if (pre) {
            launch_lsc_pre_sums(f, n, rem, stride, it & 1, s.st);
            f.gen_off++;
            launch_preempt_update(f, n, (it + 1) & 1, it & 1, false, pre_l1_thres, s.st);
            launch_lsc_pre_feats(f, l, n, rem, stride, s.st);
        } else {
            f.gen_off++;
            pg = PassGeom{};
            launch_bin_clusters_lsc(f, l, n, (it + 1) & 1, it & 1, s.st);
        }
        yx_cur = f.cl_yx_out;
        if (rec) { const int rc = snapshot(it + 1, yx_cur); if (rc) return rc; }
        rem = (rem + 1) % stride;
    }
    int full_obuf = -1;
    for (int it = 0; fusebin && it < p->max_iter; it++) {
        const bool tme = timed && s.launch_timing && it < Slot::kMaxTimedIters;
        f.cl_yx = yx_a; f.cl_yx_out = yx_a;
        f.fv_mod = lazy_labels && it < stride ? 1 : 0; f.fv_from = 0;
        if (tme) HIPCHK(hipEventRecord(s.ev_it[2 * it], s.st));
        launch_assign_fused_bin(f, n, rem, stride, it, s.st);
        if (tme) HIPCHK(hipEventRecord(s.ev_it[2 * it + 1], s.st));
        f.gen_off++;
        yx_cur = yx_a;
        rem = (rem + 1) % stride;
        full_obuf = (it + 1) % 3;
    }
    if (fusebin && full_obuf < 0) full_obuf = 0;
    for (int it = 0; !fusebin && !lsc && !rd && it < p->max_iter; it++) {
        pg = PassGeom{};
        const bool tme = timed && s.launch_timing && it < Slot::kMaxTimedIters;
        if (tme) HIPCHK(hipEventRecord(s.ev_it[2 * it], s.st));
        f.fv_mod = lazy_labels && it < stride ? 1 : 0; f.fv_from = 0;
        if (rec) launch_assign_generic(f, n, rem, stride, it & 1, it & 1, true, s.st, static_cast<uint16_t*>(rec_dist(it + 1)));
        else if (generic || (pre && !launch_assign_pre(f, n, rem, stride, it & 1, it & 1, s.st))) launch_assign_generic(f, n, rem, stride, it & 1, it & 1, true, s.st);
        else if (!pre) pg = launch_assign(f, n, rem, stride, it & 1, it & 1, true, s.st, -1, label_free);
        if (tme) HIPCHK(hipEventRecord(s.ev_it[2 * it + 1], s.st));
        f.gen_off++;
        f.cl_yx = yx_cur; f.cl_yx_out = (yx_cur == yx_a) ? yx_b : yx_a;
        if (pre) launch_preempt_update(f, n, (it + 1) & 1, it & 1, false, pre_l1_thres, s.st);
        else launch_bin_clusters(f, n, 1, (it + 1) & 1, it & 1, pg, s.st);
        yx_cur = f.cl_yx_out;
        if (rec) { const int rc = snapshot(it + 1, yx_cur); if (rc) return rc; }
        rem = (rem + 1) % stride;
    }
    int full_buf = p->max_iter & 1;
    if (pre) {
        f.gen_off++;
        f.cl_yx = yx_cur;
        launch_preempt_update(f, n, (p->max_iter + 1) & 1, 0, true, pre_l1_thres, s.st);
        full_buf = (p->max_iter + 1) & 1;
    }
    if (timed) HIPCHK(hipEventRecord(s.ev[2], s.st));
    f.fv_mod = lazy_labels && p->max_iter < stride ? stride : 0; f.fv_from = p->max_iter < stride ? std::max(p->max_iter, 0) : 0;
    if (label_free) { f.fv_mod = 1; f.fv_from = 0; }
    f.fv_rcp = f.fv_mod > 1 ? 0xFFFFFFFFu / (uint32_t)f.fv_mod : 0u;
    if (lsc) { f.cl_yx = yx_cur; launch_lsc_assign(f, l, n, 0, 1, full_buf, 0, false, s.st); }
    else if (noq) { f.cl_yx = yx_cur; launch_noq_assign(f, noq_coef, noq_manhattan, n, 0, 1, full_buf, 0, false, s.st); }
    else if (rd) { f.cl_yx = yx_cur; launch_rd_assign(f, s.d_patchf, rd_l2, n, 0, 1, full_buf, 0, false, s.st); }
    else if (generic) launch_assign_generic(f, n, 0, 1, full_buf, 0, false, s.st);
    else (void)launch_assign(f, n, 0, 1, full_buf, 0, false, s.st, full_obuf, label_free);
    if (timed) HIPCHK(hipEventRecord(s.ev[3], s.st));
    const CcaDev c = cca_view(s, i0, s.f.labels, fb, K, min_size_threshold(s));
    ExportDev ex{};
    ex.frame_bytes = fb; ex.K = K; ex.yx_cur = yx_cur; ex.lab_n_moved = yx_up + K; ex.misc0 = s.at(s.d_misc, i0);
    ex.h_cl = s.h_cl + (size_t)i0 * 4 * K; ex.h_stride = 4 * (size_t)K; ex.h_misc = status(s, i0);
    cca_enqueue(s, c, i0, n, &ex);
    if (timed) HIPCHK(hipEventRecord(s.ev[4], s.st));
    if (pre) HIPCHK(hipMemcpy2DAsync(s.h_upd + (size_t)i0 * K, sizeof(uint32_t) * (size_t)K, f.cl_upd, fb,
                                     sizeof(uint32_t) * (size_t)K, (size_t)n, hipMemcpyDeviceToHost, s.st));
    if (noq) HIPCHK(hipMemcpy2DAsync(s.h_clf + (size_t)i0 * 8 * K, sizeof(float) * 8 * (size_t)K, f.cl_f, fb,
                                     sizeof(float) * 8 * (size_t)K, (size_t)n, hipMemcpyDeviceToHost, s.st));
    return FSLIC_OK;
}

GraphRecorder*& current_recorder() {
    static thread_local GraphRecorder* rec = nullptr;
    return rec;
}

int launch_group(fslic_engine* e, Slot& s, int n) {
    s.last_launch_mode = 0;
    {
        const uint64_t span = (uint64_t)s.p.max_iter + 3u;
        if (s.gen_host + 2 * (s.gen_span_prev + span) >= 0xC0000000ull) {
            HIPCHK(hipMemsetAsync(s.d_gen, 0, 256, s.st));
            HIPCHK(hipMemset2DAsync(s.stamp_block, s.frame_bytes, 0, s.stamp_bytes, (size_t)s.cap_frames, s.st));
            s.gen_host = 0;
        }
        s.gen_step = s.gen_span_prev ? s.gen_span_prev : (uint32_t)span;
        s.gen_span_prev = (uint32_t)span;
        s.gen_host += s.gen_step;
    }
    if (s.recording) return enqueue_frames(e, s, 0, n, s.generic, true, true);
    if (!knobs().use_graphs || s.launch_timing) return enqueue_frames(e, s, 0, n, s.generic, true);
    std::vector<unsigned char> key;
    auto put = [&](const void* p, size_t bytes) { const unsigned char* b = (const unsigned char*)p; key.insert(key.end(), b, b + bytes); };
    const int hdr[9] = {s.H, s.W, s.K, s.S, n, s.generic ? 1 : 0, (int)s.gen_step, s.sp_patch_uploaded ? 1 : 0, label_free_allowed(s) ? 1 : 0};
    const void* const ptrs[9] = {s.h_cl, s.h_misc, s.d_ptrs, s.h_patch, s.d_gen, s.lsc_zero, s.d_patchf, s.h_clf, s.h_upd};
    put(hdr, sizeof hdr); put(ptrs, sizeof ptrs); put(&s.p, sizeof s.p); put(&s.f, sizeof s.f); put(&s.c, sizeof s.c);
    if (s.p.variant == FSLIC_VARIANT_LSC) put(&s.l, sizeof s.l);
    Slot::GraphEntry* ge = nullptr;
    for (auto& g : s.graphs) if (g.key == key) { ge = &g; break; }
    if (!ge) {
        if (s.graphs.size() >= 8) {
            if (s.graphs.front().exec) hipGraphExecDestroy(s.graphs.front().exec);
            if (s.graphs.front().graph) hipGraphDestroy(s.graphs.front().graph);
            s.graphs.erase(s.graphs.begin());
        }
        s.graphs.emplace_back();
        ge = &s.graphs.back();
        ge->key = key;
        if (s.store_seen_credit && s.store_labels) ge->seen = 1;
        s.store_seen_credit = false;
    }
    if (!ge->exec) {
        if (ge->failed || ge->seen++ == 0) return enqueue_frames(e, s, 0, n, s.generic, true);
        GraphRecorder rec;
        if (hipGraphCreate(&rec.graph, 0) != hipSuccess) { ge->failed = true; (void)hipGetLastError(); return enqueue_frames(e, s, 0, n, s.generic, true); }
        current_recorder() = &rec;
        const int rc = enqueue_frames(e, s, 0, n, s.generic, false);
        current_recorder() = nullptr;
        if (rc != FSLIC_OK || rec.err != hipSuccess || rec.nodes == 0 || hipGraphInstantiate(&ge->exec, rec.graph, nullptr, nullptr, 0) != hipSuccess) {
            hipGraphDestroy(rec.graph);
            ge->exec = nullptr; ge->failed = true;
            (void)hipGetLastError();
            if (rc != FSLIC_OK) return rc;
            return enqueue_frames(e, s, 0, n, s.generic, true);
        }
        ge->graph = rec.graph;
        s.last_launch_mode = 1;
    } else {
        s.last_launch_mode = 2;
    }
    HIPCHK(hipEventRecord(s.ev[0], s.st));
    HIPCHK(hipGraphLaunch(ge->exec, s.st));
    HIPCHK(hipEventRecord(s.ev[4], s.st));
    return FSLIC_OK;
}

int group_begin(fslic_engine* e, Slot& s, const GroupJob& job, bool record) {
    const double t_begin = now_us();
    const fslic_params* p = &job.p;
    const int H = job.H, W = job.W, K = job.K, n = job.n;
    int S = 0;
    s.recording = false;
    int rc = check_job(job, S);
    if (rc) return rc;
    if (record && n != 1) return fail(FSLIC_E_INTERNAL, "a recording group holds one frame");
    rc = ensure_prepared(e, s, H, W, K, S, n);
    if (rc) return rc;
    const int cap_frames = s.cap_frames;
    s.H = H; s.W = W; s.K = K; s.S = S; s.p = *p; s.nframes = n;
    if (s.store_labels && !(H == s.store_H && W == s.store_W && K == s.store_K && memcmp(&s.store_p, p, sizeof(fslic_params)) == 0)) { s.store_labels = false; s.store_seen_credit = false; }
    std::copy(job.clusters, job.clusters + n, s.clusters);
    rc = configure_spatial(s, S, p);
    if (rc) return rc;
    if (p->variant == FSLIC_VARIANT_LSC) {
        rc = prepare_lsc(s, H, W, K, S, cap_frames, p->compactness);
        if (rc) return rc;
    }
    if (p->variant == FSLIC_VARIANT_REALDIST || p->variant == FSLIC_VARIANT_REALDIST_L2) {
        rc = configure_patchf(s, S, p);
        if (rc) return rc;
    }
    if (p->variant == FSLIC_VARIANT_REALDIST_NOQ && (rc = s.h_clf.reserve((size_t)s.cap_frames * K * 8))) return rc;
    rc = upload_ptrs(s, n, job.d_rgb, job.d_out);
    if (rc) return rc;
    if (record) {
        s.rec_clusters.assign(job.clusters[0], job.clusters[0] + K);
        s.recording = true;
        const size_t need = rec_layout(s).bytes;
        if (s.d_rec.reserve(need)) {
            (void)hipGetLastError();
            s.recording = false;
            return fail(FSLIC_E_HIP, "debug_mode: hipMalloc of the snapshot ring (" + std::to_string(need) + " bytes) failed");
        }
    }
    s.generic = p->variant == FSLIC_VARIANT_SLIC && (e->lab_force_generic.load() != 0 || !s.sp_tiled_ok || record);
    if (p->preemptive && (rc = s.h_upd.reserve((size_t)s.cap_frames * K))) return rc;
    stage_group(e, s, 0, n, true);
    rc = launch_group(e, s, n);
    if (rc) return rc;
    s.have_pre = true;
    s.last_path = s.generic ? 1 : 0;
    if (knobs().host_timing) {
        fprintf(stderr, "[fslic host] group_begin n=%d: %.1f us | slot %d begin %.1f .. %.1f\n", n, now_us() - t_begin, (int)(&s - e->slots.data()), t_begin, now_us());
        s.t_begun_us = now_us();
    }
    return FSLIC_OK;
}

static int nap_wait(Slot& s) {
    const double t0 = now_us();
    HIPCHK(hipEventRecord(s.ev[5], s.st));
    const unsigned long long key = ((unsigned long long)(uint32_t)s.H << 48) ^ ((unsigned long long)(uint32_t)s.W << 32) ^ ((unsigned long long)(uint32_t)s.K << 16) ^
                                   ((unsigned long long)(uint32_t)s.nframes << 8) ^ ((unsigned long long)(uint32_t)s.p.max_iter << 4) ^ (unsigned long long)(uint32_t)s.p.variant ^
                                   ((unsigned long long)(uint32_t)s.p.preemptive << 60) ^ ((unsigned long long)(uint32_t)s.p.subsample_stride << 56);
    if (key != s.recent_wait_key) {
        s.recent_wait_key = key;
        for (double& w : s.recent_wait_us) w = 1e30;
    }
    double shortest = 1e30;
    for (double w : s.recent_wait_us) shortest = std::min(shortest, w);
    auto nap = [](double us) { struct timespec ts; ts.tv_sec = 0; ts.tv_nsec = (long)(us * 1000.0); nanosleep(&ts, nullptr); };
    if (shortest < 1e29 && shortest * 0.5 > 30.0) nap(std::min(shortest * 0.5, 20000.0));
    for (;;) {
        const hipError_t q = hipEventQuery(s.ev[5]);
        if (q == hipSuccess) break;
        if (q != hipErrorNotReady) return fail(FSLIC_E_HIP, std::string("hipEventQuery: ") + hipGetErrorString(q));
        nap(10.0);
    }
    s.recent_wait_us[s.recent_wait_i++ & 3] = now_us() - t0;
    return FSLIC_OK;
}

int group_finish(fslic_engine* e, Slot& s) {
    const double t_begin = now_us();
    if (s.nap_wait) { const int rc = nap_wait(s); if (rc) return rc; }
    HIPCHK(hipStreamSynchronize(s.st));
    const double t_sync = now_us();
    const int n = s.nframes, K = s.K, H = s.H, W = s.W;
    auto elapsed = [](float& ms, hipEvent_t a, hipEvent_t b) { if (hipEventElapsedTime(&ms, a, b) != hipSuccess) { ms = 0; (void)hipGetLastError(); } };
    elapsed(s.total_ms, s.ev[0], s.ev[4]);
    if (s.last_launch_mode == 0) {
        elapsed(s.lab_ms, s.ev[0], s.ev[1]);
        elapsed(s.loop_ms, s.ev[1], s.ev[2]);
        elapsed(s.fa_ms, s.ev[2], s.ev[3]);
        elapsed(s.cca_ms, s.ev[3], s.ev[4]);
    } else {
        s.lab_ms = s.loop_ms = s.fa_ms = s.cca_ms = 0;
    }
    s.assign_loop_ms = 0;
    for (int it = 0; it < s.n_timed_iters; it++) {
        float ms = 0;
        elapsed(ms, s.ev_it[2 * it], s.ev_it[2 * it + 1]);
        s.assign_loop_ms += ms;
    }
    const int thres = min_size_threshold(s);
    const double t_ev = now_us();
    int n_host_topk = 0;
    for (int i = 0; i < n; i++) {
        const uint32_t* hm = status(s, i);
        n_host_topk += hm[kStSelect] == kSelectHost;
        for (int attempt = 0; attempt < 2 && !s.generic && hm[kStFlags] != 0; attempt++) {
            const bool overflow = (hm[kStFlags] & kFlagListOverflow) != 0;
            const bool uncovered = (hm[kStFlags] & kFlagUncoveredPixel) != 0;
            if (uncovered && !overflow) {
                if (!s.store_labels) s.store_seen_credit = true;
                s.store_labels = true; s.store_H = H; s.store_W = W; s.store_K = K; s.store_p = s.p;
                __atomic_fetch_add(&s.n_uncovered_redo, 1, __ATOMIC_RELAXED);
            }
            if (knobs().host_timing) fprintf(stderr, "[fslic host] frame %d redone with %s\n", i, overflow ? "the generic kernel (candidate-list overflow)" : uncovered ? "storing assign passes (uncovered pixel)" : "the separate cluster pass (stale pixel)");
            stage_group(e, s, i, 1, false);
            s.gen_step = s.gen_span_prev;
            s.gen_host += s.gen_step;
            int rc = enqueue_frames(e, s, i, 1, overflow, false, true, true);
            if (rc) return rc;
            HIPCHK(hipStreamSynchronize(s.st));
            if (overflow) {
                if (hm[kStFlags] != 0) return fail(FSLIC_E_INTERNAL, "generic path reported a candidate overflow");
                s.last_path = 1;
            } else if (!uncovered) {
                __atomic_fetch_add(&s.n_separate_redo, 1, __ATOMIC_RELAXED);
            }
        }
        if (!s.generic && hm[kStFlags] != 0) return fail(FSLIC_E_INTERNAL, "a redone frame still carries a kernel flag");
    }
    {
        int rc = cca_finish_group(s, 0, n, s.f.labels, s.frame_bytes, K, thres);
        if (rc) return rc;
    }
    s.n_host_topk = n_host_topk;
    const double t_cca = now_us();
    const bool noq = s.p.variant == FSLIC_VARIANT_REALDIST_NOQ;
    for (int i = 0; i < n; i++) {
        const uint32_t* yx = s.h_cl + (size_t)i * 4 * K;
        const uint32_t* lab = yx + K;
        const uint32_t* nm = yx + 2 * (size_t)K;
        const uint32_t* moved = yx + 3 * (size_t)K;
        fslic_cluster* cl = s.clusters[i];
        for (int k = 0; k < K; k++) {
            cl[k].r = (float)(lab[k] & 255u);
            cl[k].g = (float)((lab[k] >> 8) & 255u);
            cl[k].b = (float)((lab[k] >> 16) & 255u);
            const float* c = noq ? s.h_clf + ((size_t)i * K + k) * 8 : nullptr;
            if (moved[k] && c) { cl[k].r = c[2]; cl[k].g = c[3]; cl[k].b = c[4]; }
            cluster_position(moved[k] != 0, yx[k], c, cl[k], H, W, cl[k].y, cl[k].x);
            if (s.p.max_iter > 0) cl[k].num_members = nm[k];
            cl[k].is_updatable = s.p.preemptive ? (uint8_t)s.h_upd[(size_t)i * K + k] : 2;
            cl[k].is_active = 1;
        }
    }
    if (knobs().host_timing)
        fprintf(stderr, "[fslic host] group_finish n=%d slot %d at %.1f .. %.1f: sync wait %.1f us, events %.1f us, host top-K (%d frames) %.1f us, write-back %.1f us (device %.1f us)\n",
                n, (int)(&s - e->slots.data()), t_begin, now_us(), t_sync - t_begin, t_ev - t_sync, n_host_topk, t_cca - t_ev, now_us() - t_cca, s.total_ms * 1e3);
    return FSLIC_OK;
}

void drain_failed(Slot& s) {
    const std::string msg = last_error();
    (void)hipStreamSynchronize(s.st);
    (void)hipGetLastError();
    set_last_error(msg);
}

int run_group(fslic_engine* e, Slot& s, const GroupJob& job, bool record) {
    int rc = group_begin(e, s, job, record);
    if (rc == FSLIC_OK) rc = group_finish(e, s);
    if (rc != FSLIC_OK) drain_failed(s);
    return rc;
}

std::string make_timing_report(const Slot& s) {
    char buf[1024];
    auto us = [](float ms) { return (long long)(ms * 1000.0f); };
    snprintf(buf, sizeof buf,
             "{\"name\": \"iterate\", \"duration\": %lld, \"children\": ["
             "{\"name\": \"cielab_conversion\", \"duration\": %lld, \"children\": []},"
             "{\"name\": \"assign_update_loop\", \"duration\": %lld, \"children\": []},"
             "{\"name\": \"full_assign\", \"duration\": %lld, \"children\": []},"
             "{\"name\": \"enforce_connectivity\", \"duration\": %lld, \"children\": []}]}",
             us(s.total_ms), us(s.lab_ms), us(s.loop_ms), us(s.fa_ms), us(s.cca_ms));
    return buf;
}

namespace {
thread_local std::string t_timing;
thread_local std::string t_recorder;

inline char* put_u(char* o, uint64_t v) { return std::to_chars(o, o + 24, v).ptr; }
inline char* put_i(char* o, int64_t v) { return std::to_chars(o, o + 24, v).ptr; }
inline char* put_f(char* o, float v) { return std::to_chars(o, o + 32, (double)v, std::chars_format::general, 6).ptr; }
inline char* put_s(char* o, const char* s) { const size_t n = strlen(s); memcpy(o, s, n); return o + n; }
inline char* header(char* o, int H, int W) {
    o = put_s(o, "{\"height\": "); o = put_i(o, H);
    o = put_s(o, ", \"width\": "); o = put_i(o, W);
    return put_s(o, ", \"snapshots\": [");
}
}

void set_thread_timing_report(const std::string& json) { t_timing = json; }
const std::string& thread_timing_report() { return t_timing; }
void set_thread_recorder_report(std::string&& json) { t_recorder = std::move(json); }
const std::string& thread_recorder_report() { return t_recorder; }

int make_recorder_report(Slot& s, std::string& out) {
    const int H = s.H, W = s.W, K = s.K;
    if (!s.recording) {
        char buf[96];
        char* o = header(buf, H, W);
        o = put_s(o, "]}");
        out.assign(buf, o);
        return FSLIC_OK;
    }
    const RecLayout L = rec_layout(s);
    std::vector<char> ring(L.bytes);
    HIPCHK(hipMemcpyAsync(ring.data(), s.d_rec, L.bytes, hipMemcpyDeviceToHost, s.st));
    HIPCHK(hipStreamSynchronize(s.st));
    const bool pre = s.p.preemptive != 0, noq = s.p.variant == FSLIC_VARIANT_REALDIST_NOQ;
    const size_t per_dist = L.dsize == 2 ? 6 : 16;
    out.resize(96 + L.nsnap * (96 + L.K * 320 + L.N * (6 + per_dist)));
    char* const o0 = &out[0];
    char* o = header(o0, H, W);
    const fslic_cluster* const cin = s.rec_clusters.data();
    for (size_t i = 0; i < L.nsnap; i++) {
        if (i) *o++ = ',';
        o = put_s(o, "{\"iteration\": "); o = put_i(o, (int64_t)i - 1);
        o = put_s(o, ", \"clusters\": [");
        const uint32_t* c = reinterpret_cast<const uint32_t*>(ring.data() + L.cl_off) + i * kRecWords * L.K;
        for (int k = 0; k < K; k++) {
            const fslic_cluster& a = cin[k];
            const uint32_t lab = c[K + k];
            float y = a.y, x = a.x, r = (float)(lab & 255u), g = (float)((lab >> 8) & 255u), b = (float)((lab >> 16) & 255u);
            uint32_t upd = 2, act = a.is_active, nm = a.num_members;
            if (i > 0) {
                const bool moved = c[3 * (size_t)K + k] != 0;
                const float* cf = noq ? reinterpret_cast<const float*>(c + 6 * (size_t)K) + 8 * (size_t)k : nullptr;
                if (moved && cf) { r = cf[2]; g = cf[3]; b = cf[4]; }
                cluster_position(moved, c[k], cf, a, H, W, y, x);
// ... 41 lines not shown
```

### fast_slic_amd/csrc/host_utils.cpp

```cpp
#include "engine_internal.h"
#include "forms.h"

#include <algorithm>
#include <cmath>
#include <cstring>
#include <mutex>

using namespace fslic;

extern "C" {

int fslic_hip_initialize_clusters(int H, int W, int K, const uint8_t* rgb, fslic_cluster* cl) {
    if (!rgb || !cl) return fail(FSLIC_E_INVALID, "NULL pointer argument");
    if (H <= 0 || W <= 0 || K <= 0) return FSLIC_OK;
    const int n_y = (int)sqrt((double)K);
    std::vector<int> n_xs(n_y, K / n_y);
    int remainder = K % n_y, row = 0;
    while (remainder-- > 0) {
        n_xs[row]++;
        row += 2;
        if (row >= n_y) row = 1 % n_y;
    }
    const int h = (H + n_y - 1) / n_y;
    int acc = 0;
// ... 197 lines not shown
        if ((rc = device_scratch((size_t)cap * 4, d_pair)) || (rc = device_scratch((size_t)cap * 8, d_key)) || (rc = device_scratch(8, d_cnt))) return rc;
        HIPCHK(hipMemsetAsync(d_pair.p, 0xFF, (size_t)cap * 4, st));
        HIPCHK(hipMemsetAsync(d_key.p, 0xFF, (size_t)cap * 8, st));
        HIPCHK(hipMemsetAsync(d_cnt.p, 0, 8, st));
        launch_adjacent_pairs((const uint16_t*)d_lab.p, H, W, K, (uint32_t*)d_pair.p, (unsigned long long*)d_key.p, cap, (uint32_t*)d_cnt.p, st);
        uint32_t cnt[2] = {0, 0};
        HIPCHK(hipMemcpyAsync(cnt, d_cnt.p, 8, hipMemcpyDeviceToHost, st));
        HIPCHK(hipStreamSynchronize(st));
        if (cnt[1] != 0 || cnt[0] > cap / 2) continue;
        h_pair.resize(cap); h_key.resize(cap);
        HIPCHK(hipMemcpyAsync(h_pair.data(), d_pair.p, (size_t)cap * 4, hipMemcpyDeviceToHost, st));
        HIPCHK(hipMemcpyAsync(h_key.data(), d_key.p, (size_t)cap * 8, hipMemcpyDeviceToHost, st));
        HIPCHK(hipStreamSynchronize(st));
        break;
    }
    std::vector<std::pair<unsigned long long, uint32_t>> ev;
    for (uint32_t i = 0; i < cap; i++)
        if (h_pair[i] != 0xFFFFFFFFu) ev.emplace_back(h_key[i], h_pair[i]);
    std::sort(ev.begin(), ev.end());
    for (const auto& x : ev) {
        const uint32_t a = x.second >> 16, b = x.second & 0xFFFFu;
        if (num_neighbors[a] >= kMaxConn || num_neighbors[b] >= kMaxConn) continue;
        neighbors[(size_t)a * kMaxConn + num_neighbors[a]++] = b;
        neighbors[(size_t)b * kMaxConn + num_neighbors[b]++] = a;
    }
    return FSLIC_OK;
}

int fslic_hip_knn_connectivity(int H, int W, int K, const fslic_cluster* clusters, size_t n_neighbors, int* num_neighbors, uint32_t* neighbors) {
    if (!clusters || !num_neighbors || (!neighbors && n_neighbors)) return fail(FSLIC_E_INVALID, "NULL pointer argument");
    if (H <= 0 || W <= 0 || K <= 0) return fail(FSLIC_E_INVALID, "H, W and K must be positive");
    const int S = std::max((int)std::sqrt((double)(H * W / K)), 1);
    const int nh = (H + S - 1) / S, nw = (W + S - 1) / S;
    std::vector<std::vector<int>> cells((size_t)nh * nw);
    for (int i = 0; i < K; i++) {
        const float v = std::fmaf(clusters[i].y / (float)S, (float)nw, clusters[i].x / (float)S);
        if (!(v >= 0.0f) || (size_t)v >= cells.size()) return fail(FSLIC_E_INVALID, "cluster centre outside the image");
        cells[(size_t)v].push_back(i);
    }
    std::vector<std::pair<int, int>> heap;
    for (int i = 0; i < K; i++) {
        const fslic_cluster& c = clusters[i];
        const int ccx = (int)(c.x / (float)S), ccy = (int)(c.y / (float)S);
        heap.clear();
        for (int cy = std::max(ccy - 3, 0); cy < std::min(nh, ccy + 3); cy++) {
            for (int cx = std::max(ccx - 3, 0); cx < std::min(nw, ccx + 3); cx++) {
                for (int j : cells[(size_t)cy * nw + cx]) {
                    if (j == i) continue;
                    const float dx = clusters[j].x - c.x, dy = clusters[j].y - c.y;
                    const int distance = (int)((dx < 0 ? -dx : dx) + (dy < 0 ? -dy : dy));
                    if (!heap.empty() && heap.front().first <= distance) continue;
                    heap.push_back(std::pair<int, int>(distance, j));
                    std::push_heap(heap.begin(), heap.end());
                    while (heap.size() > n_neighbors) {
                        std::pop_heap(heap.begin(), heap.end());
                        heap.pop_back();
                    }
                }
            }
        }
        num_neighbors[i] = (int)heap.size();
        for (size_t j = 0; j < n_neighbors; j++) neighbors[(size_t)i * n_neighbors + j] = j < heap.size() ? clusters[heap[j].second].number : 0u;
    }
    return FSLIC_OK;
}

int fslic_hip_copy_bandwidth(fslic_engine* e, size_t bytes, int reps, double* gb_per_s) {
    if (!e || !gb_per_s) return fail(FSLIC_E_INVALID, "NULL pointer argument");
    if (bytes < 16 || reps < 1) return fail(FSLIC_E_INVALID, "bytes and reps must be positive");
    bytes &= ~(size_t)15;
    SlotLease lease(e);
    int rc = lease.take();
    if (rc) return rc;
    Slot& s = e->slots[lease.slot];
    HIPCHK(hipSetDevice(e->device));
    Device<char> a, b;
    if (a.reserve(bytes) || b.reserve(bytes)) {
        (void)hipGetLastError();
        return fail(FSLIC_E_HIP, "hipMalloc failed for the copy probe");
    }
    hipError_t err = hipMemsetAsync(a, 1, bytes, s.st);
    double best = 0.0;
    for (int r = 0; r <= reps && err == hipSuccess; r++) {
        err = hipEventRecord(s.ev[0], s.st);
        launch_copy16(a, b, bytes, s.st);
        if (err == hipSuccess) err = hipEventRecord(s.ev[1], s.st);
        if (err == hipSuccess) err = hipStreamSynchronize(s.st);
        float ms = 0.0f;
        if (err == hipSuccess) err = hipEventElapsedTime(&ms, s.ev[0], s.ev[1]);
        if (r > 0 && ms > 0.0f) best = std::max(best, 2.0 * (double)bytes / ((double)ms * 1e-3) / 1e9);
    }
    if (err != hipSuccess) return fail(FSLIC_E_HIP, std::string("copy probe: ") + hipGetErrorString(err));
    *gb_per_s = best;
    return FSLIC_OK;
}

}

namespace fslic {
namespace {
constexpr int kFormCap = 128;
std::mutex g_forms_mu;
uint32_t g_forms[kFormCap];
int g_nforms = 0;
bool g_forms_overflow = false;
}
void note_form(uint32_t code) {
    std::lock_guard<std::mutex> lock(g_forms_mu);
    for (int i = 0; i < g_nforms; i++)
        if (g_forms[i] == code) return;
    if (g_nforms < kFormCap) g_forms[g_nforms++] = code;
    else g_forms_overflow = true;
}
int forms_seen(uint32_t* codes, int cap, bool clear) {
    std::lock_guard<std::mutex> lock(g_forms_mu);
    const int n = g_forms_overflow ? -2 : g_nforms;
    for (int i = 0; codes && i < g_nforms && i < cap; i++) codes[i] = g_forms[i];
    if (clear) { g_nforms = 0; g_forms_overflow = false; }
    return n;
}
}
```

### fast_slic_amd/csrc/kernels.h

```cpp
#pragma once
#include <hip/hip_runtime.h>
#include <stdint.h>

#ifndef FSLIC_EXP
#define FSLIC_EXP 0
#endif

namespace fslic {

constexpr int kTileW = 64;
constexpr int kWavesPerBlock = 4;
constexpr int kRowsPerWave = 8;
constexpr int kCellCap = 8;
constexpr int kAccSlots = 16;
constexpr int kAccCopies = 8;
#ifndef FSLIC_BLK_COPIES
#define FSLIC_BLK_COPIES 4
#endif
constexpr int kBlkCopies = FSLIC_BLK_COPIES;
constexpr uint32_t kHuge = 0x40000000u;
constexpr int kCcaTile = 64;
constexpr int kCcaTileH = 32;
constexpr int kCcaTilePx = kCcaTile * kCcaTileH;
#ifndef FSLIC_MAX_GROUP
// ... 101 lines not shown
        adv(sums[0], d); adv(sums[1], d); adv(cpart, d);
        adv(cell_cnt[0], d); adv(cell_cnt[1], d); adv(cell_items[0], d); adv(cell_items[1], d);
        adv(ovf_cnt[0], d); adv(ovf_cnt[1], d); adv(ovf_cnt[2], d); adv(ovf_items[0], d); adv(ovf_items[1], d); adv(ovf_items[2], d);
        adv(cl_arrive, d);
        adv(err_flag, d);
#if defined(FSLIC_LAB) && FSLIC_LAB == 4
        adv(lab_stamps, d);
#endif
    }
};

struct PassGeom {
    int rem, stride, Hv;
    int BH;
    int use_slots;
};
inline int visited_rows(int H, int rem, int stride) { return (H - rem + stride - 1) / stride; }
int blocks_scale();
inline int assign_blocks8(int W, int Hv, int nframes) {
    const long long b = (long long)nframes * ((W + kTileW - 1) / kTileW) * ((Hv + kWavesPerBlock * 8 - 1) / (kWavesPerBlock * 8)) * blocks_scale();
    return b > 0x7FFFFFFFll ? 0x7FFFFFFF : (int)b;
}

struct CcaDev {
    size_t frame_bytes;
    uint16_t* const* outs;
    size_t in_stride;
    int H, W, N, K;
    int min_threshold;
    const uint16_t* in;
    uint16_t* out;
    int tiles_x;
    uint16_t* lid;
    uint4* nrec;
    uint32_t* narea;
    uint16_t* nfinal;
    uint32_t* vedge;
    uint32_t* roots;
    uint32_t* counters;
    int32_t* cand_leader;
    uint32_t* cand_area;
    __host__ __device__ __forceinline__ void select(int z) {
        out = outs[z];
        FrameDev::adv(in, (size_t)z * in_stride);
        const size_t d = (size_t)z * frame_bytes;
        FrameDev::adv(lid, d); FrameDev::adv(nrec, d); FrameDev::adv(narea, d);
        FrameDev::adv(nfinal, d); FrameDev::adv(vedge, d); FrameDev::adv(roots, d);
        FrameDev::adv(counters, d);
        FrameDev::adv(cand_leader, d); FrameDev::adv(cand_area, d);
    }
};

constexpr int kLscFeat = 10;
constexpr int kLscCfPitch = 16;
constexpr int kLscExPitch = 12;
constexpr float kLscFixF = 1048576.0f, kLscFixW = 4096.0f;
struct LscDev {
    size_t frame_bytes;
    uint32_t* hist;
    float* means;
    float* cfeat;
    long long* extra;
    const float* lut_color;
    const float* lut_x;
    const float* lut_y;
    float blk_fix_f, blk_fix_w;
    int blk_shift_f, blk_shift_w;
    float blk_bias_w;
    __host__ __device__ __forceinline__ void select(int z) {
        const size_t d = (size_t)z * frame_bytes;
        FrameDev::adv(hist, d); FrameDev::adv(means, d);
        FrameDev::adv(cfeat, d); FrameDev::adv(extra, d);
    }
};

struct LabTables {
    const uint16_t* gamma;
    const uint16_t* labtbl;
    int cb[9];
};

void launch_rgb_to_lab(const FrameDev& f, int nframes, int convert, const LabTables& t, bool init_labels, hipStream_t st, uint32_t gen_step = 0,
                       void* zero_a = nullptr, size_t zero_a_bytes = 0, uint32_t* zero_b = nullptr, size_t zero_b_words = 0,
                       const uint32_t* stage_yx = nullptr, size_t stage_stride = 0);
void launch_bin_clusters(const FrameDev& f, int nframes, int mode, int buf, int sbuf, const PassGeom& pg, hipStream_t st,
                         const uint32_t* src_yx = nullptr, size_t src_stride = 0);
void launch_bin_clusters_lsc(const FrameDev& f, const LscDev& l, int nframes, int buf, int sbuf, hipStream_t st);

bool blk_kernel_applies(const FrameDev& f, int stride);
PassGeom launch_assign(const FrameDev& f, int nframes, int rem, int stride, int buf, int sbuf, bool fuse_update, hipStream_t st, int obuf = -1,
                       bool label_free = false);
void launch_assign_fused_bin(const FrameDev& f, int nframes, int rem, int stride, int it, hipStream_t st);
void launch_assign_generic(const FrameDev& f, int nframes, int rem, int stride, int buf, int sbuf, bool fuse_update, hipStream_t st,
                           uint16_t* rec_dist = nullptr);
bool launch_assign_pre(const FrameDev& f, int nframes, int rem, int stride, int buf, int sbuf, hipStream_t st);
void launch_lsc_prepare(const FrameDev& f, const LscDev& l, int nframes, hipStream_t st);
void launch_lsc_assign(const FrameDev& f, const LscDev& l, int nframes, int rem, int stride, int buf, int sbuf, bool stale_sums, hipStream_t st,
                       float* rec_dist = nullptr);
void launch_lsc_pre_sums(const FrameDev& f, int nframes, int rem, int stride, int sbuf, hipStream_t st);
void launch_lsc_pre_feats(const FrameDev& f, const LscDev& l, int nframes, int rem, int stride, hipStream_t st);
void launch_rd_assign(const FrameDev& f, const float* patchf, bool l2, int nframes, int rem, int stride, int buf, int sbuf, bool stale_sums, hipStream_t st,
                      float* rec_dist = nullptr);
void launch_member_sums(const FrameDev& f, int nframes, int rem, int stride, int sbuf, int margin, hipStream_t st);
void launch_noq_assign(const FrameDev& f, float coef, bool manhattan, int nframes, int rem, int stride, int buf, int sbuf, bool stale_sums, hipStream_t st,
                       float* rec_dist = nullptr);
void launch_preempt_update(const FrameDev& f, int nframes, int buf, int sbuf, bool rebin_all, float l1_thres, hipStream_t st);
void launch_cca_phase1(const CcaDev& c, int nframes, hipStream_t st);
void launch_cca_select(const CcaDev& c, int nframes, hipStream_t st);
struct ExportDev {
    size_t frame_bytes;
    int K;
    const uint32_t* yx_cur;
    const uint32_t* lab_n_moved;
    const uint32_t* misc0;
    uint32_t* h_cl;
    size_t h_stride;
    uint32_t* h_misc;
};
void launch_cca_phase2(const CcaDev& c, int nframes, hipStream_t st, const ExportDev* ex = nullptr);
void launch_cca_gather_area(const CcaDev& c, hipStream_t st);
void launch_cca_set_kept(const CcaDev& c, const int32_t* d_leaders, const uint16_t* d_labels, int n, hipStream_t st);

void launch_mask_sums(const uint16_t* labels, const uint8_t* mask, uint32_t* sums, int H, int W, int K, hipStream_t st);
void launch_density_to_mask(const uint16_t* labels, const uint8_t* dens, uint8_t* out, size_t N, int K, hipStream_t st);
void launch_adjacent_pairs(const uint16_t* labels, int H, int W, int K, uint32_t* tab_pair, unsigned long long* tab_key,
                           uint32_t cap, uint32_t* counters, hipStream_t st);

void launch_copy16(const void* src, void* dst, size_t bytes, hipStream_t st);

}
```

### fast_slic_amd/csrc/lab.hip

```cpp
#include <cstdio>
#include <cstdlib>
#include "device_common.h"

namespace fslic {

struct LabConst { uint32_t c01[3], c2[3]; };
typedef unsigned short lab_us2 __attribute__((ext_vector_type(2)));

static __device__ __forceinline__ uint32_t lab_px(uint32_t R, uint32_t G, uint32_t B,
                                                  const uint32_t* sg, const uint16_t* sl, const LabConst& k) {
    const uint32_t sr = sg[R << 5], sgv = sg[G << 5], sb = sg[B << 5];
    const lab_us2 rg = __builtin_bit_cast(lab_us2, sr | (sgv << 16));
    auto row = [&](int i) -> int {
        return (int)(__builtin_amdgcn_udot2(rg, __builtin_bit_cast(lab_us2, k.c01[i]), __umul24(k.c2[i], sb), false) >> 16);
    };
    const int xr = row(0), yr = row(1), zr = row(2);
    const int fx = sl[xr], fy = sl[yr], fz = sl[zr];
    const int ciel = 116 * fy - (16 << 13);
    const int ciea = 500 * (fx - fy) + (128 << 13);
    const int cieb = 200 * (fy - fz) + (128 << 13);
    int l = (int)((unsigned)ciel >> 12);
    int a = (int)((unsigned)ciea >> 12) - 128;
    int b = (int)((unsigned)cieb >> 12) - 128;
    l = min(max(l, 0), 255);
    a = min(max(a, 0), 255);
    b = min(max(b, 0), 255);
    return (uint32_t)l | ((uint32_t)a << 8) | ((uint32_t)b << 16);
}

template <bool CONVERT>
__global__ __launch_bounds__(1024) void k_rgb_to_lab(FrameDev f, const uint16_t* __restrict__ g_gamma,
                                                     const uint16_t* __restrict__ g_labtbl, LabConst kc, int init_labels, uint32_t gen_step,
                                                     char* zero_a, unsigned zero_a_quads, uint32_t* zero_b, unsigned zero_b_words,
                                                     const uint32_t* __restrict__ stage_yx, size_t stage_stride, int stage_K, int conv_blocks) {
    __shared__ uint32_t s_gamma32[CONVERT ? 256 * 32 : 1];
    __shared__ uint16_t s_lab[8194];
    if (gen_step && blockIdx.x == 0 && blockIdx.y == 0 && threadIdx.x == 0) *f.gen_base += gen_step;
    f.select(blockIdx.y);
    if ((int)blockIdx.x >= conv_blocks) {
        const uint32_t* src = stage_yx + (size_t)blockIdx.y * stage_stride;
        for (int i = ((int)blockIdx.x - conv_blocks) * (int)blockDim.x + (int)threadIdx.x; i < stage_K; i += ((int)gridDim.x - conv_blocks) * (int)blockDim.x)
            f.cl_yx[i] = src[i];
        return;
    }
    const uint8_t* __restrict__ rgb = f.rgb;
    uint32_t* __restrict__ lab = f.lab;
    uint16_t* __restrict__ labels_init = init_labels ? f.labels : nullptr;
    const int N = f.N;
    const int aligned4 = ((reinterpret_cast<uintptr_t>(rgb) & 3) == 0) ? 1 : 0;
    const int nquad = aligned4 ? (N >> 2) : 0;
    const int gstride = conv_blocks * blockDim.x;
    int q = blockIdx.x * blockDim.x + threadIdx.x;
    uint32_t w0 = 0, w1 = 0, w2 = 0;
    if (q < nquad) {
        const uint32_t* src = reinterpret_cast<const uint32_t*>(rgb) + 3 * (size_t)q;
        w0 = src[0]; w1 = src[1]; w2 = src[2];
    }
    uint32_t tg0 = 0, tg1 = 0, tg2 = 0, tg3 = 0, tl0 = 0, tl1 = 0, tl2 = 0, tl3 = 0, tl4 = 0;
    if (CONVERT) {
        const uint32_t* gt = reinterpret_cast<const uint32_t*>(g_labtbl);
        const uint32_t* gg = reinterpret_cast<const uint32_t*>(g_gamma) + 4 * (threadIdx.x >> 5);
        tg0 = gg[0]; tg1 = gg[1]; tg2 = gg[2]; tg3 = gg[3];
        tl0 = gt[threadIdx.x]; tl1 = gt[1024 + threadIdx.x]; tl2 = gt[2048 + threadIdx.x]; tl3 = gt[3072 + threadIdx.x];
        if (threadIdx.x == 0) tl4 = gt[4096];
    }
    const uint32_t* const s_gamma = s_gamma32 + (CONVERT ? (threadIdx.x & 31) : 0);
    if (CONVERT) {
        uint32_t* sl = reinterpret_cast<uint32_t*>(s_lab);
        uint32_t* const gd = s_gamma32 + ((threadIdx.x >> 5) * 8) * 32 + (threadIdx.x & 31);
        gd[0 * 32] = tg0 & 0xFFFFu; gd[1 * 32] = tg0 >> 16; gd[2 * 32] = tg1 & 0xFFFFu; gd[3 * 32] = tg1 >> 16;
        gd[4 * 32] = tg2 & 0xFFFFu; gd[5 * 32] = tg2 >> 16; gd[6 * 32] = tg3 & 0xFFFFu; gd[7 * 32] = tg3 >> 16;
        sl[threadIdx.x] = tl0; sl[1024 + threadIdx.x] = tl1; sl[2048 + threadIdx.x] = tl2; sl[3072 + threadIdx.x] = tl3;
        if (threadIdx.x == 0) sl[4096] = tl4;
        __syncthreads();
    }
    while (q < nquad) {
        const int qn = q + gstride;
        uint32_t n0 = 0, n1 = 0, n2 = 0;
        if (qn < nquad) {
            const uint32_t* src = reinterpret_cast<const uint32_t*>(rgb) + 3 * (size_t)qn;
            n0 = src[0]; n1 = src[1]; n2 = src[2];
        }
        uint32_t r0 = w0 & 255, g0 = (w0 >> 8) & 255, b0 = (w0 >> 16) & 255;
        uint32_t r1 = w0 >> 24, g1 = w1 & 255, b1 = (w1 >> 8) & 255;
        uint32_t r2 = (w1 >> 16) & 255, g2 = w1 >> 24, b2 = w2 & 255;
        uint32_t r3 = (w2 >> 8) & 255, g3 = (w2 >> 16) & 255, b3 = w2 >> 24;
        uint4 o;
        if (CONVERT) {
            o.x = lab_px(r0, g0, b0, s_gamma, s_lab, kc);
            o.y = lab_px(r1, g1, b1, s_gamma, s_lab, kc);
            o.z = lab_px(r2, g2, b2, s_gamma, s_lab, kc);
            o.w = lab_px(r3, g3, b3, s_gamma, s_lab, kc);
        } else {
            o.x = r0 | (g0 << 8) | (b0 << 16);
            o.y = r1 | (g1 << 8) | (b1 << 16);
            o.z = r2 | (g2 << 8) | (b2 << 16);
            o.w = r3 | (g3 << 8) | (b3 << 16);
        }
        st_stream(reinterpret_cast<uint4*>(lab) + q, o);
        if (labels_init) st_stream(reinterpret_cast<uint2*>(labels_init) + q, make_uint2(0xFFFFFFFFu, 0xFFFFFFFFu));
        w0 = n0; w1 = n1; w2 = n2;
        q = qn;
    }
    for (int p = (nquad << 2) + blockIdx.x * blockDim.x + threadIdx.x; p < N; p += gstride) {
        const uint32_t r = rgb[3 * (size_t)p], g = rgb[3 * (size_t)p + 1], b = rgb[3 * (size_t)p + 2];
        st_stream(lab + p, CONVERT ? lab_px(r, g, b, s_gamma, s_lab, kc) : (r | (g << 8) | (b << 16)));
        if (labels_init) st_stream(labels_init + p, (uint16_t)0xFFFFu);
    }
    {
        const size_t fo = (size_t)blockIdx.y * f.frame_bytes;
        const unsigned t0 = blockIdx.x * blockDim.x + threadIdx.x, ts = (unsigned)conv_blocks * blockDim.x;
        if (zero_a) { uint4* za = reinterpret_cast<uint4*>(zero_a + fo); for (unsigned i = t0; i < zero_a_quads; i += ts) za[i] = make_uint4(0u, 0u, 0u, 0u); }
        if (zero_b) { uint32_t* zb = reinterpret_cast<uint32_t*>(reinterpret_cast<char*>(zero_b) + fo); for (unsigned i = t0; i < zero_b_words; i += ts) zb[i] = 0u; }
    }
}

void launch_rgb_to_lab(const FrameDev& f, int nframes, int convert, const LabTables& t, bool init_labels, hipStream_t st, uint32_t gen_step,
                       void* zero_a, size_t zero_a_bytes, uint32_t* zero_b, size_t zero_b_words, const uint32_t* stage_yx, size_t stage_stride) {
    LabConst kc;
    for (int i = 0; i < 3; i++) {
        for (int j = 0; j < 3; j++)
            if (t.cb[3 * i + j] < 0 || t.cb[3 * i + j] > 0xFFFF) { fprintf(stderr, "fslic: RGB->XYZ coefficient outside 16 bits\n"); abort(); }
        kc.c01[i] = (uint32_t)t.cb[3 * i] | ((uint32_t)t.cb[3 * i + 1] << 16);
        kc.c2[i] = (uint32_t)t.cb[3 * i + 2];
    }
    int blocks = (f.N / 4 + 1023) / 1024;
    const int cap = (512 + nframes - 1) / nframes;
    if (blocks > cap) blocks = cap;
    if (blocks < 1) blocks = 1;
    const int stage_blocks = stage_yx ? (f.K + 1023) / 1024 : 0;
    if (convert)
        launch(k_rgb_to_lab<true>, dim3(blocks + stage_blocks, nframes), dim3(1024), 0, st, f, t.gamma, t.labtbl, kc, init_labels ? 1 : 0, gen_step, (char*)zero_a, (unsigned)(zero_a_bytes / 16), zero_b, (unsigned)zero_b_words,
               stage_yx, stage_stride, f.K, blocks);
    else
        launch(k_rgb_to_lab<false>, dim3(blocks + stage_blocks, nframes), dim3(1024), 0, st, f, t.gamma, t.labtbl, kc, init_labels ? 1 : 0, gen_step, (char*)zero_a, (unsigned)(zero_a_bytes / 16), zero_b, (unsigned)zero_b_words,
               stage_yx, stage_stride, f.K, blocks);
}

}
```

### fast_slic_amd/csrc/pipeline.cpp

```cpp
#include "engine_internal.h"

#include <algorithm>
#include <chrono>
#include <cstdio>
#include <cstdlib>
#include <cstring>

#include <sys/prctl.h>

namespace fslic {

namespace {
thread_local std::string g_err;
}
int fail(int code, const std::string& msg) {
    g_err = msg;
    return code;
}
const std::string& last_error() { return g_err; }
void set_last_error(const std::string& msg) { g_err = msg; }

namespace {
Knobs read_knobs() {
    Knobs k;
// ... 12 lines not shown
const Knobs g_knobs = read_knobs();
}
const Knobs& knobs() { return g_knobs; }
int blocks_scale() { return g_knobs.blocks_scale; }

namespace {
bool self_collecting(const Slot& s) { return s.pending && s.async && s.async->from_queue; }
}

namespace {
struct WakeWorkers {
    fslic_engine* e; bool armed = false;
    explicit WakeWorkers(fslic_engine* e_) : e(e_) {}
    ~WakeWorkers() { if (armed) e->cv_work.notify_all(); }
};
}

int acquire_slot(fslic_engine* e, int want, int& slot) {
    WakeWorkers wake(e);
    std::unique_lock<std::mutex> lk(e->mu);
    const int ns = (int)e->slots.size();
    if (want >= ns) return fail(FSLIC_E_INVALID, "slot out of range");
    auto got = [&](int i) { e->slots[i].busy = true; slot = i; return FSLIC_OK; };
    for (;;) {
        if (want >= 0) {
            Slot& s = e->slots[want];
            if (s.pending && !self_collecting(s)) return fail(FSLIC_E_INVALID, "the slot still owns an unfinished group (call fslic_hip_wait_group first)");
            if (!s.pending && !s.busy) return got(want);
        } else {
            bool any_usable = false;
            for (int i = 0; i < ns; i++) {
                Slot& s = e->slots[i];
                if (s.pending) { any_usable = any_usable || self_collecting(s); continue; }
                any_usable = true;
                if (!s.busy) return got(i);
            }
            if (!any_usable) return fail(FSLIC_E_INVALID, "every slot owns an unfinished asynchronous group");
        }
        int& waiting = want >= 0 ? e->slots[want].wanted : e->sync_waiters;
        waiting++;
        e->cv.wait(lk);
        waiting--;
        wake.armed = true;
    }
}

int acquire_all_slots(fslic_engine* e) {
    WakeWorkers wake(e);
    std::unique_lock<std::mutex> lk(e->mu);
    for (;;) {
        bool free_all = true;
        for (const Slot& s : e->slots) {
            if (s.pending && !self_collecting(s)) return fail(FSLIC_E_INVALID, "a slot still owns an unfinished group");
            free_all = free_all && !s.busy && !s.pending;
        }
        if (free_all) break;
        e->sync_waiters++;
        e->cv.wait(lk);
        e->sync_waiters--;
        wake.armed = true;
    }
    for (Slot& s : e->slots) s.busy = true;
    return FSLIC_OK;
}

void release_slot(fslic_engine* e, int slot) {
    {
        std::lock_guard<std::mutex> lk(e->mu);
        e->slots[slot].busy = false;
    }
    e->cv.notify_all(); e->cv_work.notify_all();
}

void release_all_slots(fslic_engine* e) {
    {
        std::lock_guard<std::mutex> lk(e->mu);
        for (Slot& s : e->slots) s.busy = false;
    }
    e->cv.notify_all(); e->cv_work.notify_all();
}

namespace {

void pipeline_collect(fslic_engine* e, Slot& s) {
    Slot::Async& a = *s.async;
    if (a.rc != FSLIC_OK && e->pipe_rc == FSLIC_OK) { e->pipe_rc = a.rc; e->pipe_err = a.err; }
    e->pipe_device_ms += s.total_ms;
    e->pipe_groups += 1;
    e->pipe_frames += s.nframes;
    e->pipe_host_topk += s.n_host_topk;
    s.pending = false;
}

bool same_work(const GroupJob& a, const GroupJob& b) {
    return a.H == b.H && a.W == b.W && a.K == b.K && memcmp(&a.p, &b.p, sizeof(fslic_params)) == 0;
}

void slot_worker(fslic_engine* e, Slot* s) {
    Slot::Async& a = *s->async;
    (void)hipSetDevice(e->device);
    (void)prctl(PR_SET_TIMERSLACK, 1000UL);
    for (;;) {
        bool took = false;
        {
            std::unique_lock<std::mutex> lk(e->mu);
            e->cv_work.wait(lk, [&] { return a.has_job || a.quit || (!e->pipe_q.empty() && !e->pipe_gathering && !s->busy && !s->pending && e->sync_waiters == 0 && s->wanted == 0); });
            if (a.quit) return;
            if (!a.has_job) {
                GroupJob& g = a.job;
                const int unit = e->pipe_q.front().n;
                g = e->pipe_q.front(); g.n = 0; a.jobs = 0;
                const int limit = std::min(e->pipe_batch_frames, (int)kMaxGroup);
                auto gather = [&](int max_jobs) {
                    while (!e->pipe_q.empty() && a.jobs < max_jobs) {
                        const GroupJob& j = e->pipe_q.front();
                        if (a.jobs > 0 && (!same_work(j, g) || g.n + j.n > limit)) break;
                        g.append(j); a.jobs++;
                        e->pipe_q.pop_front();
                    }
                };
                gather(kMaxGroup);
                s->pending = true;
                a.done = false; a.from_queue = true;
                e->pipe_inflight++;
                if (g.n + unit <= limit && e->pipe_q.empty() && !e->pipe_gathering && now_us() - e->pipe_last_submit_us < 50.0) {
                    e->pipe_gathering = true;
                    e->cv_work.wait_for(lk, std::chrono::microseconds(100), [&] { return !e->pipe_q.empty() || a.quit; });
                    e->pipe_gathering = false;
                    gather(kMaxGroup);
                }
                s->launch_timing = e->launch_timing;
                a.has_job = true;
                took = true;
            }
        }
        if (took) { e->cv.notify_all(); e->cv_work.notify_all(); }
        s->nap_wait = true;
        const int rc = run_group(e, *s, a.job);
        s->nap_wait = false;
        {
            std::lock_guard<std::mutex> lk(e->mu);
            a.rc = rc;
            a.err = rc ? last_error() : std::string();
            a.has_job = false;
            a.done = true;
            if (a.from_queue) {
                pipeline_collect(e, *s);
                a.from_queue = false;
                e->pipe_inflight--;
            }
        }
        e->cv.notify_all();
    }
}

void ensure_worker(fslic_engine* e, Slot& s) {
    if (s.async) return;
    s.async.reset(new Slot::Async());
    s.async->worker = std::thread(slot_worker, e, &s);
}

void hand_over(fslic_engine* e, Slot& s, const GroupJob& job) {
    ensure_worker(e, s);
    Slot::Async& a = *s.async;
    a.job = job; a.from_queue = false; a.jobs = 1;
    s.launch_timing = e->launch_timing;
    a.done = false;
    a.has_job = true;
    s.pending = true;
}

int checked_job(GroupJob& job, fslic_engine* e, const fslic_params* p, int H, int W, int K, int n_frames,
                const uint8_t* const* d_rgb, fslic_cluster* const* clusters, uint16_t* const* d_labels) {
    if (!e) return fail(FSLIC_E_INVALID, "engine is NULL");
    int S = 0;
    const int rc = fill_job(job, p, H, W, K, n_frames, d_rgb, clusters, d_labels);
    return rc ? rc : check_job(job, S);
}

}

void stop_slot_thread(fslic_engine* e, Slot& s) {
    if (!s.async) return;
    {
        std::lock_guard<std::mutex> lk(e->mu);
        s.async->quit = true;
    }
    e->cv_work.notify_all();
    if (s.async->worker.joinable()) s.async->worker.join();
    s.async.reset();
}

}

using namespace fslic;

extern "C" {

int fslic_hip_submit_group(fslic_engine* e, int slot, const fslic_params* p, int H, int W, int K, int n_frames,
                           const uint8_t* const* d_rgb, fslic_cluster* const* clusters, uint16_t* const* d_labels) {
    GroupJob job;
    int rc = checked_job(job, e, p, H, W, K, n_frames, d_rgb, clusters, d_labels);
    if (rc) return rc;
    if (slot < 0 || slot >= (int)e->slots.size()) return fail(FSLIC_E_INVALID, "slot out of range");
    {
        std::unique_lock<std::mutex> lk(e->mu);
        Slot& s = e->slots[slot];
        for (;;) {
            if (s.pending && !self_collecting(s)) return fail(FSLIC_E_INVALID, "the slot still owns an unfinished group (call fslic_hip_wait_group first)");
            if (!s.busy && !s.pending) break;
            e->cv.wait(lk);
        }
        hand_over(e, s, job);
    }
    e->cv_work.notify_all();
    return FSLIC_OK;
}

int fslic_hip_wait_group(fslic_engine* e, int slot) {
    if (!e) return fail(FSLIC_E_INVALID, "engine is NULL");
    if (slot < 0 || slot >= (int)e->slots.size()) return fail(FSLIC_E_INVALID, "slot out of range");
    Slot& s = e->slots[slot];
    int rc;
    {
        std::unique_lock<std::mutex> lk(e->mu);
        if (!s.pending) return FSLIC_OK;
        Slot::Async& a = *s.async;
        e->cv.wait(lk, [&] { return a.done; });
        rc = a.rc;
        if (rc) set_last_error(a.err);
        s.pending = false;
        if (rc == FSLIC_OK) set_thread_timing_report(make_timing_report(s));
    }
    e->cv.notify_all(); e->cv_work.notify_all();
    return rc;
}

int fslic_hip_group_done(fslic_engine* e, int slot) {
    if (!e || slot < 0 || slot >= (int)e->slots.size()) return -1;
    std::lock_guard<std::mutex> lk(e->mu);
    Slot& s = e->slots[slot];
    if (!s.pending) return 1;
    return s.async->done ? 1 : 0;
}

int fslic_hip_pipeline_submit(fslic_engine* e, const fslic_params* p, int H, int W, int K, int n_frames,
                              const uint8_t* const* d_rgb, fslic_cluster* const* clusters, uint16_t* const* d_labels) {
    GroupJob job;
    int rc = checked_job(job, e, p, H, W, K, n_frames, d_rgb, clusters, d_labels);
    if (rc) return rc;
    {
        std::unique_lock<std::mutex> lk(e->mu);
        for (Slot& s : e->slots) ensure_worker(e, s);
        const size_t cap = 2 * e->slots.size();
        e->cv.wait(lk, [&] { return e->pipe_rc != FSLIC_OK || e->pipe_q.size() < cap; });
        if (e->pipe_rc != FSLIC_OK) { set_last_error(e->pipe_err); return e->pipe_rc; }
        e->pipe_q.push_back(job);
        e->pipe_last_submit_us = now_us();
    }
    e->cv_work.notify_all();
    return FSLIC_OK;
}

int fslic_hip_pipeline_batching(fslic_engine* e, int max_frames_per_group) {
    if (!e) return fail(FSLIC_E_INVALID, "engine is NULL");
    if (max_frames_per_group < 0 || max_frames_per_group > (int)kMaxGroup) return fail(FSLIC_E_INVALID, "frames per group out of range");
    std::lock_guard<std::mutex> lk(e->mu);
    e->pipe_batch_frames = max_frames_per_group;
    e->reserve_frames.store(max_frames_per_group);
    return FSLIC_OK;
}

int fslic_hip_pipeline_drain(fslic_engine* e, double* device_ms, long long* groups, long long* frames, long long* host_topk_frames) {
    if (!e) return fail(FSLIC_E_INVALID, "engine is NULL");
    int rc;
    {
        std::unique_lock<std::mutex> lk(e->mu);
        e->cv.wait(lk, [&] { return e->pipe_q.empty() && e->pipe_inflight == 0; });
        rc = e->pipe_rc;
        if (rc) set_last_error(e->pipe_err);
        if (device_ms) *device_ms = e->pipe_device_ms;
        if (groups) *groups = e->pipe_groups;
        if (frames) *frames = e->pipe_frames;
        if (host_topk_frames) *host_topk_frames = e->pipe_host_topk;
        e->pipe_rc = FSLIC_OK; e->pipe_err.clear();
        e->pipe_device_ms = 0; e->pipe_groups = 0; e->pipe_frames = 0; e->pipe_host_topk = 0;
    }
    e->cv.notify_all();
    return rc;
}

}
```

### include/fslic_hip.h

```cpp
#ifndef FSLIC_HIP_H
#define FSLIC_HIP_H

#include <stddef.h>
#include <stdint.h>

#ifdef __cplusplus
extern "C" {
#endif

#define FSLIC_HIP_ARCH_NAME "hip/gfx950"

enum {
    FSLIC_OK = 0,
    FSLIC_E_INVALID = 1,
    FSLIC_E_UNSUPPORTED = 2,
    FSLIC_E_HIP = 3,
    FSLIC_E_INTERNAL = 4
};

typedef struct fslic_cluster {
    float y, x, r, g, b, a;
    uint16_t number;
    uint8_t is_active;
    uint8_t is_updatable;
// ... 18 lines not shown
#define FSLIC_PARAMS_ABI 0x46533033

enum {
    FSLIC_VARIANT_SLIC = 0,
    FSLIC_VARIANT_LSC = 1,
    FSLIC_VARIANT_REALDIST = 2,
    FSLIC_VARIANT_REALDIST_L2 = 3,
    FSLIC_VARIANT_REALDIST_NOQ = 4
};

typedef struct fslic_engine fslic_engine;

int fslic_hip_device_count(void);

int fslic_hip_create(int device, int n_slots, fslic_engine** out);
void fslic_hip_destroy(fslic_engine* e);

int fslic_hip_initialize_clusters(int H, int W, int K, const uint8_t* rgb, fslic_cluster* clusters);

int fslic_hip_iterate(fslic_engine* e, const fslic_params* p, int H, int W, int K,
                      const uint8_t* rgb, fslic_cluster* clusters, uint16_t* labels);

int fslic_hip_iterate_device(fslic_engine* e, int slot, const fslic_params* p, int H, int W, int K,
                             const uint8_t* d_rgb, fslic_cluster* clusters, uint16_t* d_labels);

int fslic_hip_iterate_batch(fslic_engine* e, const fslic_params* p, int H, int W, int K, int n_frames,
                            const uint8_t* const* rgb, fslic_cluster* const* clusters,
                            uint16_t* const* labels, int device_ptrs);

int fslic_hip_submit_group(fslic_engine* e, int slot, const fslic_params* p, int H, int W, int K, int n_frames,
                           const uint8_t* const* d_rgb, fslic_cluster* const* clusters, uint16_t* const* d_labels);
int fslic_hip_wait_group(fslic_engine* e, int slot);
int fslic_hip_group_done(fslic_engine* e, int slot);

int fslic_hip_pipeline_submit(fslic_engine* e, const fslic_params* p, int H, int W, int K, int n_frames,
                              const uint8_t* const* d_rgb, fslic_cluster* const* clusters, uint16_t* const* d_labels);
int fslic_hip_pipeline_drain(fslic_engine* e, double* device_ms, long long* groups, long long* frames,
                             long long* host_topk_frames);
int fslic_hip_pipeline_batching(fslic_engine* e, int max_frames_per_group);


int fslic_hip_rgb_to_lab(fslic_engine* e, int H, int W, const uint8_t* rgb, int convert, uint8_t* lab4);

int fslic_hip_enforce_connectivity(fslic_engine* e, uint16_t* labels, int H, int W, int K, int min_threshold);
int fslic_hip_enforce_connectivity_nodes(fslic_engine* e, uint16_t* labels, int H, int W, int K, int min_threshold, uint32_t* n_nodes);


int fslic_hip_get_connectivity(fslic_engine* e, int H, int W, int K, const uint16_t* labels,
                               int* num_neighbors, uint32_t* neighbors);

int fslic_hip_knn_connectivity(int H, int W, int K, const fslic_cluster* clusters, size_t n_neighbors,
                               int* num_neighbors, uint32_t* neighbors);

int fslic_hip_get_mask_density(fslic_engine* e, int H, int W, int K, const fslic_cluster* clusters,
                               const uint16_t* labels, const uint8_t* mask, uint8_t* densities);

int fslic_hip_cluster_density_to_mask(fslic_engine* e, int H, int W, int K, const uint16_t* labels,
                                      const uint8_t* densities, uint8_t* result);

int fslic_hip_last_prelabels(fslic_engine* e, int slot, uint16_t* prelabels);

int fslic_hip_debug_lsc_state(fslic_engine* e, int slot, int z, int K, float* means10, float* cfeat);

const char* fslic_hip_last_timing_report(fslic_engine* e);

int fslic_hip_last_recorder_report(fslic_engine* e, const char** report, size_t* length);

int fslic_hip_last_device_times(fslic_engine* e, int slot, float* total_ms, float* full_assign_ms);

int fslic_hip_set_launch_timing(fslic_engine* e, int on);
int fslic_hip_last_assign_loop(fslic_engine* e, int slot, float* sum_ms, double* visited_px, int* launches);

int fslic_hip_last_group_frames(fslic_engine* e, int slot);

int fslic_hip_last_launch_mode(fslic_engine* e, int slot);

int fslic_hip_last_path(fslic_engine* e, int slot);

int fslic_hip_last_host_topk_frames(fslic_engine* e, int slot);

int fslic_hip_separate_pass_redos(fslic_engine* e, int slot);

int fslic_hip_uncovered_redos(fslic_engine* e, int slot);

int fslic_hip_debug_forms_seen(uint32_t* codes, int cap, int clear);
int fslic_hip_debug_forms_all(uint32_t* codes, int cap);

int fslic_hip_copy_bandwidth(fslic_engine* e, size_t bytes, int reps, double* gb_per_s);

typedef struct fslic_crf fslic_crf;
typedef struct fslic_crf_frame fslic_crf_frame;
typedef struct fslic_crf_params {
    float spatial_w, temporal_w, spatial_srgb, temporal_srgb, spatial_sxy, spatial_smooth_w, spatial_smooth_sxy;
} fslic_crf_params;

int fslic_hip_crf_new(size_t num_classes, size_t num_nodes, fslic_crf** out);
void fslic_hip_crf_free(fslic_crf* crf);
int fslic_hip_crf_copy(fslic_crf* crf, fslic_crf** out);
int fslic_hip_crf_get_params(fslic_crf* crf, fslic_crf_params* out);
int fslic_hip_crf_set_params(fslic_crf* crf, const fslic_crf_params* params);
int fslic_hip_crf_set_compat(fslic_crf* crf, int cls, float compat_value);
int fslic_hip_crf_get_compat(fslic_crf* crf, int cls, float* out);
int fslic_hip_crf_num_classes(fslic_crf* crf, size_t* num_classes, size_t* num_nodes);
int fslic_hip_crf_first_time(fslic_crf* crf);
int fslic_hip_crf_last_time(fslic_crf* crf);
size_t fslic_hip_crf_num_frames(fslic_crf* crf);
int fslic_hip_crf_pop_frame(fslic_crf* crf);
int fslic_hip_crf_push_frame(fslic_crf* crf, fslic_crf_frame** out);
int fslic_hip_crf_frame(fslic_crf* crf, int time, fslic_crf_frame** out);
int fslic_hip_crf_frame_time(fslic_crf_frame* frame);
int fslic_hip_crf_frame_set_clusters(fslic_crf_frame* frame, const fslic_cluster* clusters);
int fslic_hip_crf_frame_get_clusters(fslic_crf_frame* frame, fslic_cluster* clusters);
int fslic_hip_crf_frame_set_connectivity(fslic_crf_frame* frame, int num_rows, const int* num_neighbors, const uint32_t* neighbors,
                                         size_t stride);
int fslic_hip_crf_frame_set_connectivity_csr(fslic_crf_frame* frame, int num_rows, const int64_t* offsets, const uint32_t* indices);
int fslic_hip_crf_frame_get_connectivity(fslic_crf_frame* frame, int64_t* offsets, uint32_t* indices);
int fslic_hip_crf_frame_set_mask(fslic_crf_frame* frame, const int32_t* classes, float confidence);
int fslic_hip_crf_frame_set_proba(fslic_crf_frame* frame, const float* probas);
int fslic_hip_crf_frame_set_unbiased(fslic_crf_frame* frame);
int fslic_hip_crf_frame_set_unary(fslic_crf_frame* frame, const float* unary_energies);
int fslic_hip_crf_frame_get_unary(fslic_crf_frame* frame, float* unary_energies);
int fslic_hip_crf_frame_spatial_energy(fslic_crf_frame* frame, int node_i, int node_j, float* out);
int fslic_hip_crf_frame_temporal_energy(fslic_crf_frame* frame, fslic_crf_frame* other_frame, int node_i, float* out);
int fslic_hip_crf_frame_get_inferred(fslic_crf_frame* frame, float* probas);
int fslic_hip_crf_frame_reset_inferred(fslic_crf_frame* frame);
int fslic_hip_crf_initialize(fslic_crf* crf);
int fslic_hip_crf_inference(fslic_crf* crf, fslic_engine* e, size_t max_iter);
int fslic_hip_crf_expf_host(const float* in, float* out, size_t n, int use_libm);
int fslic_hip_crf_expf_device(fslic_engine* e, const float* in, float* out, size_t n);

enum { FSLIC_POOL_SUM = 0, FSLIC_POOL_MEAN = 1, FSLIC_POOL_MAX = 2 };
enum { FSLIC_LABEL_U16 = 0 , FSLIC_LABEL_I32 = 1, FSLIC_LABEL_I64 = 2 };
int fslic_hip_pool_workspace_size(int N, int C, int K, int reduce, size_t* bytes);
int fslic_hip_pool(int device, void* stream, int N, int C, int H, int W, int K, int reduce, const float* features,
                   const void* labels, int label_type, void* workspace, size_t workspace_bytes);
int fslic_hip_pool_finalize(int device, void* stream, int N, int C, int K, int reduce, const void* workspace, size_t workspace_bytes,
                            float* values, int32_t* counts, int32_t* argmax);
int fslic_hip_unpool(int device, void* stream, int N, int C, int H, int W, int K, const float* values, const void* labels,
                     int label_type, const int32_t* argmax, float fill, float* out);

int fslic_hip_rag_workspace_size(int N, int K, int C, long long capacity, size_t* bytes);
int fslic_hip_rag_accumulate(int device, void* stream, int N, int H, int W, int K, int connectivity, const void* labels, int label_type,
                             const uint8_t* image, int C, long long capacity, void* workspace, size_t workspace_bytes);
int fslic_hip_rag_compact(int device, void* stream, int N, int C, long long capacity, void* workspace, size_t workspace_bytes,
                          int64_t* keys, int32_t* boundary, int64_t* contrast, long long max_edges);

int fslic_hip_overlap_workspace_size(int N, long long capacity, size_t* bytes);
int fslic_hip_overlap_accumulate(int device, void* stream, int N, int H, int W, int K, int M, const void* labels, int label_type,
                                 const void* other, int other_type, long long capacity, void* workspace, size_t workspace_bytes);
int fslic_hip_overlap_compact(int device, void* stream, int N, long long capacity, void* workspace, size_t workspace_bytes,
                              int64_t* keys, int32_t* count, long long max_pairs);
int fslic_hip_boundary_match(int device, void* stream, int N, int H, int W, const void* labels, int label_type,
                             const void* other, int other_type, int tolerance, int64_t* counts);

int fslic_hip_crf_tensor_workspace_size(int N, int C, int K, long long nnz, size_t* bytes);
int fslic_hip_crf_tensor_inference(int device, void* stream, int N, int C, int K, int temporal, int max_iter,
                                   const fslic_crf_params* params, const float* compat, const float* yxrgb, const int32_t* members,
                                   const int64_t* offsets, const int32_t* indices, long long nnz,
                                   const float* unaries, const float* q0 , float* q_out,
                                   void* workspace, size_t workspace_bytes);

int fslic_hip_crf_tensor_grad_workspace_size(int N, int C, int K, long long nnz, int backward, int with_compat, size_t* bytes);
int fslic_hip_crf_tensor_inference_saved(int device, void* stream, int N, int C, int K, int temporal, int max_iter,
                                         const fslic_crf_params* params, const float* compat, const float* yxrgb, const int32_t* members,
                                         const int64_t* offsets, const int32_t* indices, long long nnz,
                                         const float* unaries, const float* q0 , float* q_all,
// ... 42 lines not shown
```

Before: 69220 megapixels/sec.

## Double-buffer pinned staging per slot to overlap consecutive pipeline groups

Each slot now keeps two pinned host buffer sets (cluster export, status, pointer table, events) selected by a parity index. Kernels reach these buffers through a device pointer table instead of baked-in host pointers. The pipeline worker can therefore start the next queued group on a slot before finishing host-side completion of the previous one, overlapping host postprocessing and launch overhead with device work. The cost is much more complex in-flight bookkeeping: a host-fallback path re-makes the earlier group current, and this adds risk around error handling and ordering.

```diff
diff --git a/fast_slic_amd/_binding.py b/fast_slic_amd/_binding.py
--- a/fast_slic_amd/_binding.py
+++ b/fast_slic_amd/_binding.py
@@ -36,7 +36,7 @@
     "fslic_hip_last_device_times", "fslic_hip_set_launch_timing", "fslic_hip_last_assign_loop", "fslic_hip_last_group_frames", "fslic_hip_last_path", "fslic_hip_last_launch_mode", "fslic_hip_group_done", "fslic_hip_last_error", "fslic_hip_version",
     "fslic_hip_get_connectivity", "fslic_hip_knn_connectivity", "fslic_hip_get_mask_density", "fslic_hip_cluster_density_to_mask",
     "fslic_hip_pipeline_submit", "fslic_hip_pipeline_drain", "fslic_hip_pipeline_batching", "fslic_hip_last_host_topk_frames",
-    "fslic_hip_separate_pass_redos", "fslic_hip_uncovered_redos", "fslic_hip_copy_bandwidth", "fslic_hip_last_recorder_report",
+    "fslic_hip_separate_pass_redos", "fslic_hip_uncovered_redos", "fslic_hip_overlapped_groups", "fslic_hip_pipeline_overlap", "fslic_hip_copy_bandwidth", "fslic_hip_last_recorder_report",
     "fslic_hip_debug_lsc_state", "fslic_hip_debug_forms_seen", "fslic_hip_debug_forms_all",
     "fslic_hip_crf_new", "fslic_hip_crf_free", "fslic_hip_crf_copy", "fslic_hip_crf_get_params", "fslic_hip_crf_set_params",
     "fslic_hip_crf_set_compat", "fslic_hip_crf_get_compat", "fslic_hip_crf_num_classes", "fslic_hip_crf_first_time",
@@ -154,6 +154,10 @@
         lib.fslic_hip_separate_pass_redos.argtypes = [vp, i32]
         if hasattr(lib, "fslic_hip_uncovered_redos"):
             lib.fslic_hip_uncovered_redos.argtypes = [vp, i32]
+        if hasattr(lib, "fslic_hip_overlapped_groups"):
+            lib.fslic_hip_overlapped_groups.argtypes = [vp]
+            lib.fslic_hip_overlapped_groups.restype = C.c_longlong
+            lib.fslic_hip_pipeline_overlap.argtypes = [vp, i32]
         if hasattr(lib, "fslic_hip_copy_bandwidth"):
             lib.fslic_hip_copy_bandwidth.argtypes = [vp, C.c_size_t, i32, C.POINTER(C.c_double)]
         lib.fslic_hip_group_done.argtypes = [vp, i32]
@@ -428,6 +432,15 @@
         slots = range(self.n_slots) if slot is None else [int(slot)]
         return sum(int(lib.fslic_hip_uncovered_redos(self._h, s)) for s in slots)
 
+    def overlapped_groups(self):
+        lib = load_library()
+        if not hasattr(lib, "fslic_hip_overlapped_groups"):
+            return 0
+        return int(lib.fslic_hip_overlapped_groups(self._h))
+
+    def pipeline_overlap(self, on):
+        _check(load_library().fslic_hip_pipeline_overlap(self._h, int(bool(on))))
+
     def copy_bandwidth(self, nbytes=1 << 30, reps=5):
         v = C.c_double()
         _check(load_library().fslic_hip_copy_bandwidth(self._h, C.c_size_t(int(nbytes)), int(reps), C.byref(v)))
diff --git a/fast_slic_amd/csrc/arena.cpp b/fast_slic_amd/csrc/arena.cpp
--- a/fast_slic_amd/csrc/arena.cpp
+++ b/fast_slic_amd/csrc/arena.cpp
@@ -8,7 +8,7 @@
 void free_slot(Slot& s) {
     for (auto& g : s.graphs) { if (g.exec) hipGraphExecDestroy(g.exec); if (g.graph) hipGraphDestroy(g.graph); }
     s.graphs.clear();
-    for (auto& e : s.ev) if (e) hipEventDestroy(e);
+    for (auto& ps : s.set) for (auto& e : ps.ev) if (e) hipEventDestroy(e);
     for (auto& e : s.ev_it) if (e) hipEventDestroy(e);
     if (s.st) hipStreamDestroy(s.st);
     s = Slot();
@@ -23,8 +23,9 @@
     if (G < s.cap_frames && s.keyH == H && s.keyW == W && s.keyK == K) G = s.cap_frames;
 
     int rc;
-    if ((rc = s.h_cl.reserve((size_t)G * 4 * K)) || (rc = s.h_misc.reserve((size_t)kStatusWords * kMaxGroup)) ||
-        (rc = s.h_lut.reserve(kLutMaxWords)) || (rc = s.h_tab.reserve(3 * kTabMaxBytes / sizeof(uint16_t))) ||
+    for (PinnedSet& ps : s.set)
+        if ((rc = ps.h_cl.reserve((size_t)G * 4 * K)) || (rc = ps.h_misc.reserve((size_t)kStatusWords * kMaxGroup))) return rc;
+    if ((rc = s.h_lut.reserve(kLutMaxWords)) || (rc = s.h_tab.reserve(3 * kTabMaxBytes / sizeof(uint16_t))) ||
         (rc = s.h_patchf.reserve(P * P)) || (rc = s.h_patch.reserve(P * P)))
         return rc;
 
@@ -121,9 +122,14 @@
     return FSLIC_OK;
 }
 
+bool prepared_for(const fslic_engine* e, const Slot& s, int H, int W, int K, int G) {
+    G = std::max(G, std::min(e->reserve_frames.load(), (int)kMaxGroup));
+    return s.keyH == H && s.keyW == W && s.keyK == K && s.cap_frames >= G;
+}
+
 int ensure_prepared(fslic_engine* e, Slot& s, int H, int W, int K, int S, int G) {
+    if (prepared_for(e, s, H, W, K, G)) return FSLIC_OK;
     G = std::max(G, std::min(e->reserve_frames.load(), (int)kMaxGroup));
-    if (s.keyH == H && s.keyW == W && s.keyK == K && s.cap_frames >= G) return FSLIC_OK;
     HIPCHK(hipStreamSynchronize(s.st));
     return prepare(e, s, H, W, K, S, G);
 }
diff --git a/fast_slic_amd/csrc/capi.cpp b/fast_slic_amd/csrc/capi.cpp
--- a/fast_slic_amd/csrc/capi.cpp
+++ b/fast_slic_amd/csrc/capi.cpp
@@ -38,11 +38,11 @@
     e->slots.resize(n_slots);
     for (auto& s : e->slots) {
         if (hipStreamCreateWithFlags(&s.st, hipStreamNonBlocking) != hipSuccess) { fslic_hip_destroy(e); return fail(FSLIC_E_HIP, "hipStreamCreate failed"); }
-        for (auto& ev : s.ev)
+        for (auto& ps : s.set) for (auto& ev : ps.ev)
             if (hipEventCreate(&ev) != hipSuccess) { fslic_hip_destroy(e); return fail(FSLIC_E_HIP, "hipEventCreate failed"); }
         for (auto& ev : s.ev_it)
             if (hipEventCreate(&ev) != hipSuccess) { fslic_hip_destroy(e); return fail(FSLIC_E_HIP, "hipEventCreate failed"); }
-        if (s.d_ptrs.reserve(2 * kMaxGroup) || s.h_ptrs.reserve(2 * kMaxGroup) ||
+        if (s.d_ptrs.reserve(kPtrTable) || s.set[0].h_ptrs.reserve(kPtrTable) || s.set[1].h_ptrs.reserve(kPtrTable) ||
             s.d_gen.reserve(64) || hipMemset(s.d_gen, 0, 256) != hipSuccess) { fslic_hip_destroy(e); return fail(FSLIC_E_HIP, "pointer table allocation failed"); }
     }
     if (e->d_gamma.reserve(sizeof ht.gamma / sizeof ht.gamma[0]) || e->d_labtbl.reserve(sizeof ht.lab / sizeof ht.lab[0])) { fslic_hip_destroy(e); return fail(FSLIC_E_HIP, "hipMalloc(tables) failed"); }
@@ -262,6 +262,14 @@
     return FSLIC_OK;
 }
 
+int fslic_hip_debug_fail_group(fslic_engine* e, int what, int after) {
+    if (!e || what < -1 || what > 2 || after < 0) return fail(FSLIC_E_INVALID, "bad arguments");
+    e->debug_fail_what.store(-1);
+    e->debug_fail_after.store(after);
+    e->debug_fail_what.store(what);
+    return FSLIC_OK;
+}
+
 int fslic_hip_last_assign_loop(fslic_engine* e, int slot, float* sum_ms, double* visited_px, int* launches) {
     if (!e || slot < 0 || slot >= (int)e->slots.size()) return fail(FSLIC_E_INVALID, "bad engine/slot");
     const Slot& s = e->slots[slot];
@@ -299,6 +307,11 @@
 int fslic_hip_uncovered_redos(fslic_engine* e, int slot) {
     if (!e || slot < 0 || slot >= (int)e->slots.size()) return -1;
     return __atomic_load_n(&e->slots[slot].n_uncovered_redo, __ATOMIC_RELAXED);
+}
+
+long long fslic_hip_overlapped_groups(fslic_engine* e) {
+    if (!e) return -1;
+    return e->overlapped_groups.load(std::memory_order_relaxed);
 }
 
 int fslic_hip_debug_forms_seen(uint32_t* codes, int cap, int clear) {
diff --git a/fast_slic_amd/csrc/cca.hip b/fast_slic_amd/csrc/cca.hip
--- a/fast_slic_amd/csrc/cca.hip
+++ b/fast_slic_amd/csrc/cca.hip
@@ -910,11 +910,11 @@
         const size_t d = (size_t)z * ex.frame_bytes;
         const uint32_t* yx = ex.yx_cur; const uint32_t* rest = ex.lab_n_moved; const uint32_t* misc = ex.misc0;
         FrameDev::adv(yx, d); FrameDev::adv(rest, d); FrameDev::adv(misc, d);
-        uint32_t* out = ex.h_cl + (size_t)z * ex.h_stride;
+        uint32_t* out = ex.tab[0] + ex.h_off + (size_t)z * ex.h_stride;
         const int K = ex.K;
         for (int i = ((int)blockIdx.x - relabel_blocks) * blockDim.x + threadIdx.x; i < 4 * K; i += ((int)gridDim.x - relabel_blocks) * blockDim.x)
             out[i] = i < K ? yx[i] : rest[i - K];
-        if ((int)blockIdx.x == relabel_blocks && threadIdx.x < kStatusWords) ex.h_misc[kStatusWords * (size_t)z + threadIdx.x] = misc[threadIdx.x];
+        if ((int)blockIdx.x == relabel_blocks && threadIdx.x < kStatusWords) ex.tab[1][ex.misc_off + kStatusWords * (size_t)z + threadIdx.x] = misc[threadIdx.x];
         return;
     }
     c.select(z);
diff --git a/fast_slic_amd/csrc/engine_internal.h b/fast_slic_amd/csrc/engine_internal.h
--- a/fast_slic_amd/csrc/engine_internal.h
+++ b/fast_slic_amd/csrc/engine_internal.h
@@ -94,9 +94,33 @@
 };
 const HostTables& host_tables();
 
+constexpr int kPtrStage = 2 * kMaxGroup, kPtrExport = kPtrStage + 1, kPtrStatus = kPtrStage + 2, kPtrTable = kPtrStage + 3;
+
+struct PinnedSet {
+    hipEvent_t ev[6] = {nullptr, nullptr, nullptr, nullptr, nullptr, nullptr};
+    Pinned<uint32_t> h_cl;
+    Pinned<uint32_t> h_misc;
+    Pinned<void*> h_ptrs;
+};
+
+struct InFlight {
+    GroupJob job;
+    int S = 0;
+    int par = 0;
+    bool generic = false;
+    int launch_mode = 0;
+    double t_begun_us = 0;
+    float total_ms = 0;
+    int n_host_topk = 0;
+};
+
 struct Slot {
     hipStream_t st = nullptr;
-    hipEvent_t ev[6] = {nullptr, nullptr, nullptr, nullptr, nullptr, nullptr};
+    PinnedSet set[2];
+    int par = 0;
+    InFlight fl[2];
+    PinnedSet& pin() { return set[par]; }
+    const PinnedSet& pin() const { return set[par]; }
     static constexpr int kMaxTimedIters = 16;
     hipEvent_t ev_it[2 * kMaxTimedIters] = {};
     int n_timed_iters = 0;
@@ -118,14 +142,11 @@
     int32_t* d_keep_leader = nullptr;
     uint16_t* d_keep_label = nullptr;
     Device<void*> d_ptrs;
-    Pinned<void*> h_ptrs;
     uint16_t* d_patch = nullptr;
     uint32_t* d_lut = nullptr;
     Pinned<uint32_t> h_lut;
     uint16_t* d_tab = nullptr;
     Pinned<uint16_t> h_tab;
-    Pinned<uint32_t> h_cl;
-    Pinned<uint32_t> h_misc;
     Pinned<uint16_t> h_patch;
     Pinned<int32_t> h_cand_leader;
     Pinned<uint32_t> h_cand_area;
@@ -203,7 +224,8 @@
     template <class T> T* at(T* p, int frame) const { return reinterpret_cast<T*>(reinterpret_cast<char*>(p) + (size_t)frame * frame_bytes); }
 };
 
-inline uint32_t* status(const Slot& s, int frame) { return s.h_misc + (size_t)kStatusWords * frame; }
+inline uint32_t* status(const Slot& s, int frame) { return s.pin().h_misc + (size_t)kStatusWords * frame; }
+inline uint32_t* status(const Slot& s, int par, int frame) { return s.set[par].h_misc + (size_t)kStatusWords * frame; }
 
 inline void cluster_position(bool moved, uint32_t yx, const float* centroid, const fslic_cluster& in, int H, int W, float& y, float& x) {
     if (moved && centroid) { y = centroid[0]; x = centroid[1]; }
@@ -234,10 +256,14 @@
     double pipe_last_submit_us = 0;
     std::atomic<int> reserve_frames{0};
     int sync_waiters = 0;
+    std::atomic<bool> pipe_overlap{true};
+    std::atomic<long long> overlapped_groups{0};
     std::atomic<int> lab_force_generic{0};
+    std::atomic<int> debug_fail_what{-1}, debug_fail_after{0};
 };
 
 extern "C" int fslic_hip_lab_force_generic(fslic_engine* e, int on);
+extern "C" int fslic_hip_debug_fail_group(fslic_engine* e, int what, int after);
 
 namespace fslic {
 
@@ -247,6 +273,7 @@
 void free_slot(Slot& s);
 int prepare(fslic_engine* e, Slot& s, int H, int W, int K, int S, int G);
 int ensure_prepared(fslic_engine* e, Slot& s, int H, int W, int K, int S, int G);
+bool prepared_for(const fslic_engine* e, const Slot& s, int H, int W, int K, int G);
 int prepare_lsc(Slot& s, int H, int W, int K, int S, int G, float compactness);
 
 int validate(const fslic_params* p, int H, int W, int K, int& S);
@@ -259,6 +286,11 @@
 int cca_finish_group(Slot& s, int first, int n, const uint16_t* d_in0, size_t in_stride, int K, int thres);
 int group_begin(fslic_engine* e, Slot& s, const GroupJob& job, bool record = false);
 int group_finish(fslic_engine* e, Slot& s);
+int group_wait(Slot& s, InFlight& g, bool successor);
+bool group_prewait(Slot& s, const InFlight& g, int& rc);
+bool group_needs_host(const Slot& s, const InFlight& g);
+int make_current(Slot& s, const InFlight& g);
+int group_complete(fslic_engine* e, Slot& s, InFlight& g, bool from_scratch);
 void drain_failed(Slot& s);
 int run_group(fslic_engine* e, Slot& s, const GroupJob& job, bool record = false);
 std::string make_timing_report(const Slot& s);
diff --git a/fast_slic_amd/csrc/group.cpp b/fast_slic_amd/csrc/group.cpp
--- a/fast_slic_amd/csrc/group.cpp
+++ b/fast_slic_amd/csrc/group.cpp
@@ -91,11 +91,15 @@
 }
 
 int upload_ptrs(Slot& s, int n, const uint8_t* const* d_rgb, uint16_t* const* d_out) {
+    PinnedSet& ps = s.pin();
     for (int i = 0; i < kMaxGroup; i++) {
-        s.h_ptrs[i] = (i < n && d_rgb) ? const_cast<uint8_t*>(d_rgb[i]) : nullptr;
-        s.h_ptrs[kMaxGroup + i] = (i < n && d_out) ? d_out[i] : nullptr;
-    }
-    HIPCHK(hipMemcpyAsync(s.d_ptrs, s.h_ptrs, sizeof(void*) * 2 * kMaxGroup, hipMemcpyHostToDevice, s.st));
+        ps.h_ptrs[i] = (i < n && d_rgb) ? const_cast<uint8_t*>(d_rgb[i]) : nullptr;
+        ps.h_ptrs[kMaxGroup + i] = (i < n && d_out) ? d_out[i] : nullptr;
+    }
+    ps.h_ptrs[kPtrStage] = ps.h_cl.get();
+    ps.h_ptrs[kPtrExport] = ps.h_cl.get();
+    ps.h_ptrs[kPtrStatus] = ps.h_misc.get();
+    HIPCHK(hipMemcpyAsync(s.d_ptrs, ps.h_ptrs, sizeof(void*) * kPtrTable, hipMemcpyHostToDevice, s.st));
     return FSLIC_OK;
 }
 
@@ -151,7 +155,7 @@
     const int H = s.H, W = s.W, K = s.K;
     for (int z = 0; z < n; z++) {
         const fslic_cluster* cl = s.clusters[i0 + z];
-        uint32_t* h = s.h_cl + (size_t)(i0 + z) * 4 * K;
+        uint32_t* h = s.pin().h_cl + (size_t)(i0 + z) * 4 * K;
         for (int k = 0; k < K; k++) {
             const int y = clampi((int)cl[k].y, 0, H - 1), x = clampi((int)cl[k].x, 0, W - 1);
             h[k] = ((uint32_t)y << 16) | (uint32_t)x;
@@ -216,6 +220,7 @@
 int enqueue_frames(fslic_engine* e, Slot& s, int i0, int n, bool generic, bool timed, bool separate_cluster_pass = false, bool store_labels = false) {
     const fslic_params* p = &s.p;
     const int K = s.K, S = s.S;
+    hipEvent_t* const ev = s.pin().ev;
     FrameDev f = s.f;
     f.rgbs = nullptr;
     f.select(i0);
@@ -245,14 +250,15 @@
                                 sizeof(float) * 8 * (size_t)K, (size_t)n, hipMemcpyHostToDevice, s.st));
     }
 
-    if (timed) HIPCHK(hipEventRecord(s.ev[0], s.st));
+    if (timed) HIPCHK(hipEventRecord(ev[0], s.st));
     f.gen_base = s.d_gen;
     const bool fusebin = cluster_pass_fused(f, *p, n, s.W, s.H, generic, separate_cluster_pass);
     const bool lazy_labels = p->variant == FSLIC_VARIANT_SLIC && !generic && p->preemptive == 0 && !fusebin;
     const bool label_free = lazy_labels && !store_labels && label_free_allowed(s) && p->max_iter >= 1 && !s.recording && blk_kernel_applies(f, p->subsample_stride);
     launch_rgb_to_lab(f, n, p->convert_to_lab, e->tables, !lazy_labels, s.st, s.gen_step,
-                      s.at(s.zero_block, i0), s.zero_bytes, f.cl_n, 2 * (size_t)K, s.h_cl + (size_t)i0 * 4 * K, 4 * (size_t)K);
-    if (timed) HIPCHK(hipEventRecord(s.ev[1], s.st));
+                      s.at(s.zero_block, i0), s.zero_bytes, f.cl_n, 2 * (size_t)K,
+                      reinterpret_cast<const uint32_t* const*>(s.d_ptrs + kPtrStage), (size_t)i0 * 4 * K, 4 * (size_t)K);
+    if (timed) HIPCHK(hipEventRecord(ev[1], s.st));
     f.gen_off = 1;
     PassGeom pg{};
     uint32_t* const yx_up = f.cl_yx;
@@ -379,7 +385,7 @@
         launch_preempt_update(f, n, (p->max_iter + 1) & 1, 0, true, pre_l1_thres, s.st);
         full_buf = (p->max_iter + 1) & 1;
     }
-    if (timed) HIPCHK(hipEventRecord(s.ev[2], s.st));
+    if (timed) HIPCHK(hipEventRecord(ev[2], s.st));
     f.fv_mod = lazy_labels && p->max_iter < stride ? stride : 0; f.fv_from = p->max_iter < stride ? std::max(p->max_iter, 0) : 0;
     if (label_free) { f.fv_mod = 1; f.fv_from = 0; }
     f.fv_rcp = f.fv_mod > 1 ? 0xFFFFFFFFu / (uint32_t)f.fv_mod : 0u;
@@ -388,13 +394,14 @@
     else if (rd) { f.cl_yx = yx_cur; launch_rd_assign(f, s.d_patchf, rd_l2, n, 0, 1, full_buf, 0, false, s.st); }
     else if (generic) launch_assign_generic(f, n, 0, 1, full_buf, 0, false, s.st);
     else (void)launch_assign(f, n, 0, 1, full_buf, 0, false, s.st, full_obuf, label_free);
-    if (timed) HIPCHK(hipEventRecord(s.ev[3], s.st));
+    if (timed) HIPCHK(hipEventRecord(ev[3], s.st));
     const CcaDev c = cca_view(s, i0, s.f.labels, fb, K, min_size_threshold(s));
     ExportDev ex{};
     ex.frame_bytes = fb; ex.K = K; ex.yx_cur = yx_cur; ex.lab_n_moved = yx_up + K; ex.misc0 = s.at(s.d_misc, i0);
-    ex.h_cl = s.h_cl + (size_t)i0 * 4 * K; ex.h_stride = 4 * (size_t)K; ex.h_misc = status(s, i0);
+    ex.tab = reinterpret_cast<uint32_t* const*>(s.d_ptrs + kPtrExport);
+    ex.h_off = (size_t)i0 * 4 * K; ex.h_stride = 4 * (size_t)K; ex.misc_off = (size_t)kStatusWords * i0;
     cca_enqueue(s, c, i0, n, &ex);
-    if (timed) HIPCHK(hipEventRecord(s.ev[4], s.st));
+    if (timed) HIPCHK(hipEventRecord(ev[4], s.st));
     if (pre) HIPCHK(hipMemcpy2DAsync(s.h_upd + (size_t)i0 * K, sizeof(uint32_t) * (size_t)K, f.cl_upd, fb,
                                      sizeof(uint32_t) * (size_t)K, (size_t)n, hipMemcpyDeviceToHost, s.st));
     if (noq) HIPCHK(hipMemcpy2DAsync(s.h_clf + (size_t)i0 * 8 * K, sizeof(float) * 8 * (size_t)K, f.cl_f, fb,
@@ -425,7 +432,7 @@
     std::vector<unsigned char> key;
     auto put = [&](const void* p, size_t bytes) { const unsigned char* b = (const unsigned char*)p; key.insert(key.end(), b, b + bytes); };
     const int hdr[9] = {s.H, s.W, s.K, s.S, n, s.generic ? 1 : 0, (int)s.gen_step, s.sp_patch_uploaded ? 1 : 0, label_free_allowed(s) ? 1 : 0};
-    const void* const ptrs[9] = {s.h_cl, s.h_misc, s.d_ptrs, s.h_patch, s.d_gen, s.lsc_zero, s.d_patchf, s.h_clf, s.h_upd};
+    const void* const ptrs[7] = {s.d_ptrs, s.h_patch, s.d_gen, s.lsc_zero, s.d_patchf, s.h_clf, s.h_upd};
     put(hdr, sizeof hdr); put(ptrs, sizeof ptrs); put(&s.p, sizeof s.p); put(&s.f, sizeof s.f); put(&s.c, sizeof s.c);
     if (s.p.variant == FSLIC_VARIANT_LSC) put(&s.l, sizeof s.l);
     Slot::GraphEntry* ge = nullptr;
@@ -461,10 +468,17 @@
     } else {
         s.last_launch_mode = 2;
     }
-    HIPCHK(hipEventRecord(s.ev[0], s.st));
+    HIPCHK(hipEventRecord(s.pin().ev[0], s.st));
     HIPCHK(hipGraphLaunch(ge->exec, s.st));
-    HIPCHK(hipEventRecord(s.ev[4], s.st));
-    return FSLIC_OK;
+    HIPCHK(hipEventRecord(s.pin().ev[4], s.st));
+    return FSLIC_OK;
+}
+
+static bool debug_fail_here(fslic_engine* e, const Slot& s, int what) {
+    if (!s.nap_wait || e->debug_fail_what.load(std::memory_order_relaxed) != what) return false;
+    if (e->debug_fail_after.fetch_sub(1) != 0) return false;
+    e->debug_fail_what.store(-1);
+    return true;
 }
 
 int group_begin(fslic_engine* e, Slot& s, const GroupJob& job, bool record) {
@@ -476,9 +490,11 @@
     int rc = check_job(job, S);
     if (rc) return rc;
     if (record && n != 1) return fail(FSLIC_E_INTERNAL, "a recording group holds one frame");
+    if (debug_fail_here(e, s, 0)) return fail(FSLIC_E_INTERNAL, "testing aid: group_begin failed before it touched the slot");
     rc = ensure_prepared(e, s, H, W, K, S, n);
     if (rc) return rc;
     const int cap_frames = s.cap_frames;
+    s.par ^= 1;
     s.H = H; s.W = W; s.K = K; s.S = S; s.p = *p; s.nframes = n;
     if (s.store_labels && !(H == s.store_H && W == s.store_W && K == s.store_K && memcmp(&s.store_p, p, sizeof(fslic_params)) == 0)) { s.store_labels = false; s.store_seen_credit = false; }
     std::copy(job.clusters, job.clusters + n, s.clusters);
@@ -510,8 +526,12 @@
     stage_group(e, s, 0, n, true);
     rc = launch_group(e, s, n);
     if (rc) return rc;
+    if (debug_fail_here(e, s, 1)) return fail(FSLIC_E_INTERNAL, "testing aid: group_begin failed after it enqueued the group");
     s.have_pre = true;
     s.last_path = s.generic ? 1 : 0;
+    InFlight& g = s.fl[s.par];
+    g.job = job; g.S = S; g.par = s.par; g.generic = s.generic; g.launch_mode = s.last_launch_mode;
+    g.t_begun_us = now_us();
     if (knobs().host_timing) {
         fprintf(stderr, "[fslic host] group_begin n=%d: %.1f us | slot %d begin %.1f .. %.1f\n", n, now_us() - t_begin, (int)(&s - e->slots.data()), t_begin, now_us());
         s.t_begun_us = now_us();
@@ -519,43 +539,77 @@
     return FSLIC_OK;
 }
 
-static int nap_wait(Slot& s) {
-    const double t0 = now_us();
-    HIPCHK(hipEventRecord(s.ev[5], s.st));
-    const unsigned long long key = ((unsigned long long)(uint32_t)s.H << 48) ^ ((unsigned long long)(uint32_t)s.W << 32) ^ ((unsigned long long)(uint32_t)s.K << 16) ^
-                                   ((unsigned long long)(uint32_t)s.nframes << 8) ^ ((unsigned long long)(uint32_t)s.p.max_iter << 4) ^ (unsigned long long)(uint32_t)s.p.variant ^
-                                   ((unsigned long long)(uint32_t)s.p.preemptive << 60) ^ ((unsigned long long)(uint32_t)s.p.subsample_stride << 56);
+static double shortest_flight(Slot& s, const InFlight& g) {
+    const GroupJob& j = g.job;
+    const unsigned long long key = ((unsigned long long)(uint32_t)j.H << 48) ^ ((unsigned long long)(uint32_t)j.W << 32) ^ ((unsigned long long)(uint32_t)j.K << 16) ^
+                                   ((unsigned long long)(uint32_t)j.n << 8) ^ ((unsigned long long)(uint32_t)j.p.max_iter << 4) ^ (unsigned long long)(uint32_t)j.p.variant ^
+                                   ((unsigned long long)(uint32_t)j.p.preemptive << 60) ^ ((unsigned long long)(uint32_t)j.p.subsample_stride << 56);
     if (key != s.recent_wait_key) {
         s.recent_wait_key = key;
         for (double& w : s.recent_wait_us) w = 1e30;
     }
     double shortest = 1e30;
     for (double w : s.recent_wait_us) shortest = std::min(shortest, w);
+    return shortest;
+}
+
+static int nap_poll(const InFlight& g, hipEvent_t ev, double shortest, double deadline_us, bool& done) {
     auto nap = [](double us) { struct timespec ts; ts.tv_sec = 0; ts.tv_nsec = (long)(us * 1000.0); nanosleep(&ts, nullptr); };
-    if (shortest < 1e29 && shortest * 0.5 > 30.0) nap(std::min(shortest * 0.5, 20000.0));
+    if (shortest < 1e29 && shortest * 0.5 > 30.0) {
+        const double rest = std::min(g.t_begun_us + std::min(shortest * 0.5, 20000.0), deadline_us) - now_us();
+        if (rest > 1.0) nap(rest);
+    }
     for (;;) {
-        const hipError_t q = hipEventQuery(s.ev[5]);
-        if (q == hipSuccess) break;
+        const hipError_t q = hipEventQuery(ev);
+        done = q == hipSuccess;
+        if (done) return FSLIC_OK;
         if (q != hipErrorNotReady) return fail(FSLIC_E_HIP, std::string("hipEventQuery: ") + hipGetErrorString(q));
+        if (now_us() >= deadline_us) return FSLIC_OK;
         nap(10.0);
     }
-    s.recent_wait_us[s.recent_wait_i++ & 3] = now_us() - t0;
-    return FSLIC_OK;
-}
-
-int group_finish(fslic_engine* e, Slot& s) {
-    const double t_begin = now_us();
-    if (s.nap_wait) { const int rc = nap_wait(s); if (rc) return rc; }
-    HIPCHK(hipStreamSynchronize(s.st));
-    const double t_sync = now_us();
-    const int n = s.nframes, K = s.K, H = s.H, W = s.W;
+}
+
+static int nap_wait(Slot& s, const InFlight& g, bool successor) {
+    const hipEvent_t ev = s.set[g.par].ev[successor ? 4 : 5];
+    if (!successor) HIPCHK(hipEventRecord(ev, s.st));
+    bool done = false;
+    const int rc = nap_poll(g, ev, shortest_flight(s, g), 1e300, done);
+    if (rc) return rc;
+    s.recent_wait_us[s.recent_wait_i++ & 3] = now_us() - g.t_begun_us;
+    return FSLIC_OK;
+}
+
+constexpr double kOverlapMaxFlightUs = 4000.0;
+constexpr double kSuccessorLeadUs = 200.0;
+
+bool group_prewait(Slot& s, const InFlight& g, int& rc) {
+    rc = FSLIC_OK;
+    const double shortest = shortest_flight(s, g);
+    if (shortest > 1e29) return false;
+    if (shortest > kOverlapMaxFlightUs) return false;
+    bool done = false;
+    rc = nap_poll(g, s.set[g.par].ev[4], shortest, g.t_begun_us + shortest - kSuccessorLeadUs, done);
+    return rc == FSLIC_OK;
+}
+
+int group_wait(Slot& s, InFlight& g, bool successor) {
+    PinnedSet& ps = s.set[g.par];
+    if (successor) {
+        const int rc = nap_wait(s, g, true);
+        if (rc) return rc;
+        HIPCHK(hipEventSynchronize(ps.ev[4]));
+    } else {
+        if (s.nap_wait) { const int rc = nap_wait(s, g, false); if (rc) return rc; }
+        HIPCHK(hipStreamSynchronize(s.st));
+    }
     auto elapsed = [](float& ms, hipEvent_t a, hipEvent_t b) { if (hipEventElapsedTime(&ms, a, b) != hipSuccess) { ms = 0; (void)hipGetLastError(); } };
-    elapsed(s.total_ms, s.ev[0], s.ev[4]);
-    if (s.last_launch_mode == 0) {
-        elapsed(s.lab_ms, s.ev[0], s.ev[1]);
-        elapsed(s.loop_ms, s.ev[1], s.ev[2]);
-        elapsed(s.fa_ms, s.ev[2], s.ev[3]);
-        elapsed(s.cca_ms, s.ev[3], s.ev[4]);
+    elapsed(s.total_ms, ps.ev[0], ps.ev[4]);
+    g.total_ms = s.total_ms;
+    if (g.launch_mode == 0) {
+        elapsed(s.lab_ms, ps.ev[0], ps.ev[1]);
+        elapsed(s.loop_ms, ps.ev[1], ps.ev[2]);
+        elapsed(s.fa_ms, ps.ev[2], ps.ev[3]);
+        elapsed(s.cca_ms, ps.ev[3], ps.ev[4]);
     } else {
         s.lab_ms = s.loop_ms = s.fa_ms = s.cca_ms = 0;
     }
@@ -565,12 +619,49 @@
         elapsed(ms, s.ev_it[2 * it], s.ev_it[2 * it + 1]);
         s.assign_loop_ms += ms;
     }
+    return FSLIC_OK;
+}
+
+bool group_needs_host(const Slot& s, const InFlight& g) {
+    for (int i = 0; i < g.job.n; i++) {
+        const uint32_t* hm = status(s, g.par, i);
+        if (hm[kStSelect] == kSelectHost || (!g.generic && hm[kStFlags] != 0)) return true;
+    }
+    return false;
+}
+
+int make_current(Slot& s, const InFlight& g) {
+    const GroupJob& j = g.job;
+    s.par = g.par;
+    s.H = j.H; s.W = j.W; s.K = j.K; s.S = g.S; s.p = j.p; s.nframes = j.n;
+    s.generic = g.generic; s.recording = false;
+    std::copy(j.clusters, j.clusters + j.n, s.clusters);
+    return upload_ptrs(s, j.n, j.d_rgb, j.d_out);
+}
+
+int group_complete(fslic_engine* e, Slot& s, InFlight& g, bool from_scratch) {
+    if (debug_fail_here(e, s, 2)) return fail(FSLIC_E_INTERNAL, "testing aid: group_complete failed before the write-back");
+    const double t_ev = now_us();
+    const GroupJob& job = g.job;
+    const fslic_params& p = job.p;
+    const int n = job.n, K = job.K, H = job.H, W = job.W;
+    const PinnedSet& ps = s.set[g.par];
+    int n_host_topk = 0;
+    for (int i = 0; i < n; i++) n_host_topk += status(s, g.par, i)[kStSelect] == kSelectHost;
+    const bool host_steps = group_needs_host(s, g);
+    if (host_steps && s.par != g.par) return fail(FSLIC_E_INTERNAL, "host steps of a group that is not the slot's current one");
     const int thres = min_size_threshold(s);
-    const double t_ev = now_us();
-    int n_host_topk = 0;
-    for (int i = 0; i < n; i++) {
+    for (int i = 0; host_steps && i < n; i++) {
         const uint32_t* hm = status(s, i);
-        n_host_topk += hm[kStSelect] == kSelectHost;
+        if (from_scratch && hm[kStSelect] == kSelectHost && (s.generic || hm[kStFlags] == 0)) {
+            stage_group(e, s, i, 1, false);
+            s.gen_step = s.gen_span_prev;
+            s.gen_host += s.gen_step;
+            const bool separate = !cluster_pass_fused(s.f, s.p, n, W, H, s.generic, false);
+            const int rc = enqueue_frames(e, s, i, 1, s.generic, false, separate);
+            if (rc) return rc;
+            HIPCHK(hipStreamSynchronize(s.st));
+        }
         for (int attempt = 0; attempt < 2 && !s.generic && hm[kStFlags] != 0; attempt++) {
             const bool overflow = (hm[kStFlags] & kFlagListOverflow) != 0;
             const bool uncovered = (hm[kStFlags] & kFlagUncoveredPixel) != 0;
@@ -595,19 +686,19 @@
         }
         if (!s.generic && hm[kStFlags] != 0) return fail(FSLIC_E_INTERNAL, "a redone frame still carries a kernel flag");
     }
-    {
+    if (host_steps) {
         int rc = cca_finish_group(s, 0, n, s.f.labels, s.frame_bytes, K, thres);
         if (rc) return rc;
     }
-    s.n_host_topk = n_host_topk;
+    s.n_host_topk = g.n_host_topk = n_host_topk;
     const double t_cca = now_us();
-    const bool noq = s.p.variant == FSLIC_VARIANT_REALDIST_NOQ;
+    const bool noq = p.variant == FSLIC_VARIANT_REALDIST_NOQ;
     for (int i = 0; i < n; i++) {
-        const uint32_t* yx = s.h_cl + (size_t)i * 4 * K;
+        const uint32_t* yx = ps.h_cl + (size_t)i * 4 * K;
         const uint32_t* lab = yx + K;
         const uint32_t* nm = yx + 2 * (size_t)K;
         const uint32_t* moved = yx + 3 * (size_t)K;
-        fslic_cluster* cl = s.clusters[i];
+        fslic_cluster* cl = job.clusters[i];
         for (int k = 0; k < K; k++) {
             cl[k].r = (float)(lab[k] & 255u);
             cl[k].g = (float)((lab[k] >> 8) & 255u);
@@ -615,15 +706,24 @@
             const float* c = noq ? s.h_clf + ((size_t)i * K + k) * 8 : nullptr;
             if (moved[k] && c) { cl[k].r = c[2]; cl[k].g = c[3]; cl[k].b = c[4]; }
             cluster_position(moved[k] != 0, yx[k], c, cl[k], H, W, cl[k].y, cl[k].x);
-            if (s.p.max_iter > 0) cl[k].num_members = nm[k];
-            cl[k].is_updatable = s.p.preemptive ? (uint8_t)s.h_upd[(size_t)i * K + k] : 2;
+            if (p.max_iter > 0) cl[k].num_members = nm[k];
+            cl[k].is_updatable = p.preemptive ? (uint8_t)s.h_upd[(size_t)i * K + k] : 2;
             cl[k].is_active = 1;
         }
     }
     if (knobs().host_timing)
-        fprintf(stderr, "[fslic host] group_finish n=%d slot %d at %.1f .. %.1f: sync wait %.1f us, events %.1f us, host top-K (%d frames) %.1f us, write-back %.1f us (device %.1f us)\n",
-                n, (int)(&s - e->slots.data()), t_begin, now_us(), t_sync - t_begin, t_ev - t_sync, n_host_topk, t_cca - t_ev, now_us() - t_cca, s.total_ms * 1e3);
-    return FSLIC_OK;
+        fprintf(stderr, "[fslic host] group_complete n=%d slot %d .. %.1f: host steps (%d frames for top-K) %.1f us, write-back %.1f us (device %.1f us)\n",
+                n, (int)(&s - e->slots.data()), now_us(), n_host_topk, t_cca - t_ev, now_us() - t_cca, s.total_ms * 1e3);
+    return FSLIC_OK;
+}
+
+int group_finish(fslic_engine* e, Slot& s) {
+    const double t_begin = now_us();
+    InFlight& g = s.fl[s.par];
+    int rc = group_wait(s, g, false);
+    if (rc) return rc;
+    if (knobs().host_timing) fprintf(stderr, "[fslic host] group_finish n=%d slot %d at %.1f: wait + events %.1f us\n", g.job.n, (int)(&s - e->slots.data()), t_begin, now_us() - t_begin);
+    return group_complete(e, s, g, false);
 }
 
 void drain_failed(Slot& s) {
diff --git a/fast_slic_amd/csrc/host_utils.cpp b/fast_slic_amd/csrc/host_utils.cpp
--- a/fast_slic_amd/csrc/host_utils.cpp
+++ b/fast_slic_amd/csrc/host_utils.cpp
@@ -303,12 +303,12 @@
     hipError_t err = hipMemsetAsync(a, 1, bytes, s.st);
     double best = 0.0;
     for (int r = 0; r <= reps && err == hipSuccess; r++) {
-        err = hipEventRecord(s.ev[0], s.st);
+        err = hipEventRecord(s.pin().ev[0], s.st);
         launch_copy16(a, b, bytes, s.st);
-        if (err == hipSuccess) err = hipEventRecord(s.ev[1], s.st);
+        if (err == hipSuccess) err = hipEventRecord(s.pin().ev[1], s.st);
         if (err == hipSuccess) err = hipStreamSynchronize(s.st);
         float ms = 0.0f;
-        if (err == hipSuccess) err = hipEventElapsedTime(&ms, s.ev[0], s.ev[1]);
+        if (err == hipSuccess) err = hipEventElapsedTime(&ms, s.pin().ev[0], s.pin().ev[1]);
         if (r > 0 && ms > 0.0f) best = std::max(best, 2.0 * (double)bytes / ((double)ms * 1e-3) / 1e9);
     }
     if (err != hipSuccess) return fail(FSLIC_E_HIP, std::string("copy probe: ") + hipGetErrorString(err));
diff --git a/fast_slic_amd/csrc/kernels.h b/fast_slic_amd/csrc/kernels.h
--- a/fast_slic_amd/csrc/kernels.h
+++ b/fast_slic_amd/csrc/kernels.h
@@ -207,7 +207,7 @@
 
 void launch_rgb_to_lab(const FrameDev& f, int nframes, int convert, const LabTables& t, bool init_labels, hipStream_t st, uint32_t gen_step = 0,
                        void* zero_a = nullptr, size_t zero_a_bytes = 0, uint32_t* zero_b = nullptr, size_t zero_b_words = 0,
-                       const uint32_t* stage_yx = nullptr, size_t stage_stride = 0);
+                       const uint32_t* const* stage_tab = nullptr, size_t stage_off = 0, size_t stage_stride = 0);
 void launch_bin_clusters(const FrameDev& f, int nframes, int mode, int buf, int sbuf, const PassGeom& pg, hipStream_t st,
                          const uint32_t* src_yx = nullptr, size_t src_stride = 0);
 void launch_bin_clusters_lsc(const FrameDev& f, const LscDev& l, int nframes, int buf, int sbuf, hipStream_t st);
@@ -238,9 +238,8 @@
     const uint32_t* yx_cur;
     const uint32_t* lab_n_moved;
     const uint32_t* misc0;
-    uint32_t* h_cl;
-    size_t h_stride;
-    uint32_t* h_misc;
+    uint32_t* const* tab;
+    size_t h_off, h_stride, misc_off;
 };
 void launch_cca_phase2(const CcaDev& c, int nframes, hipStream_t st, const ExportDev* ex = nullptr);
 void launch_cca_gather_area(const CcaDev& c, hipStream_t st);
diff --git a/fast_slic_amd/csrc/lab.hip b/fast_slic_amd/csrc/lab.hip
--- a/fast_slic_amd/csrc/lab.hip
+++ b/fast_slic_amd/csrc/lab.hip
@@ -32,13 +32,13 @@
 __global__ __launch_bounds__(1024) void k_rgb_to_lab(FrameDev f, const uint16_t* __restrict__ g_gamma,
                                                      const uint16_t* __restrict__ g_labtbl, LabConst kc, int init_labels, uint32_t gen_step,
                                                      char* zero_a, unsigned zero_a_quads, uint32_t* zero_b, unsigned zero_b_words,
-                                                     const uint32_t* __restrict__ stage_yx, size_t stage_stride, int stage_K, int conv_blocks) {
+                                                     const uint32_t* const* __restrict__ stage_tab, size_t stage_off, size_t stage_stride, int stage_K, int conv_blocks) {
     __shared__ uint32_t s_gamma32[CONVERT ? 256 * 32 : 1];
     __shared__ uint16_t s_lab[8194];
     if (gen_step && blockIdx.x == 0 && blockIdx.y == 0 && threadIdx.x == 0) *f.gen_base += gen_step;
     f.select(blockIdx.y);
     if ((int)blockIdx.x >= conv_blocks) {
-        const uint32_t* src = stage_yx + (size_t)blockIdx.y * stage_stride;
+        const uint32_t* src = *stage_tab + stage_off + (size_t)blockIdx.y * stage_stride;
         for (int i = ((int)blockIdx.x - conv_blocks) * (int)blockDim.x + (int)threadIdx.x; i < stage_K; i += ((int)gridDim.x - conv_blocks) * (int)blockDim.x)
             f.cl_yx[i] = src[i];
         return;
@@ -116,7 +116,7 @@
 }
 
 void launch_rgb_to_lab(const FrameDev& f, int nframes, int convert, const LabTables& t, bool init_labels, hipStream_t st, uint32_t gen_step,
-                       void* zero_a, size_t zero_a_bytes, uint32_t* zero_b, size_t zero_b_words, const uint32_t* stage_yx, size_t stage_stride) {
+                       void* zero_a, size_t zero_a_bytes, uint32_t* zero_b, size_t zero_b_words, const uint32_t* const* stage_tab, size_t stage_off, size_t stage_stride) {
     LabConst kc;
     for (int i = 0; i < 3; i++) {
         for (int j = 0; j < 3; j++)
@@ -128,13 +128,13 @@
     const int cap = (512 + nframes - 1) / nframes;
     if (blocks > cap) blocks = cap;
     if (blocks < 1) blocks = 1;
-    const int stage_blocks = stage_yx ? (f.K + 1023) / 1024 : 0;
+    const int stage_blocks = stage_tab ? (f.K + 1023) / 1024 : 0;
     if (convert)
         launch(k_rgb_to_lab<true>, dim3(blocks + stage_blocks, nframes), dim3(1024), 0, st, f, t.gamma, t.labtbl, kc, init_labels ? 1 : 0, gen_step, (char*)zero_a, (unsigned)(zero_a_bytes / 16), zero_b, (unsigned)zero_b_words,
-               stage_yx, stage_stride, f.K, blocks);
+               stage_tab, stage_off, stage_stride, f.K, blocks);
     else
         launch(k_rgb_to_lab<false>, dim3(blocks + stage_blocks, nframes), dim3(1024), 0, st, f, t.gamma, t.labtbl, kc, init_labels ? 1 : 0, gen_step, (char*)zero_a, (unsigned)(zero_a_bytes / 16), zero_b, (unsigned)zero_b_words,
-               stage_yx, stage_stride, f.K, blocks);
+               stage_tab, stage_off, stage_stride, f.K, blocks);
 }
 
 }
diff --git a/fast_slic_amd/csrc/pipeline.cpp b/fast_slic_amd/csrc/pipeline.cpp
--- a/fast_slic_amd/csrc/pipeline.cpp
+++ b/fast_slic_amd/csrc/pipeline.cpp
@@ -118,35 +118,82 @@
 
 namespace {
 
-void pipeline_collect(fslic_engine* e, Slot& s) {
+void pipeline_collect(fslic_engine* e, Slot& s, const InFlight* g, int rc, const std::string& err, int frames, bool last_of_slot) {
     Slot::Async& a = *s.async;
-    if (a.rc != FSLIC_OK && e->pipe_rc == FSLIC_OK) { e->pipe_rc = a.rc; e->pipe_err = a.err; }
-    e->pipe_device_ms += s.total_ms;
+    if (rc != FSLIC_OK && e->pipe_rc == FSLIC_OK) { e->pipe_rc = rc; e->pipe_err = err; }
+    e->pipe_device_ms += g ? g->total_ms : 0.0f;
     e->pipe_groups += 1;
-    e->pipe_frames += s.nframes;
-    e->pipe_host_topk += s.n_host_topk;
-    s.pending = false;
+    e->pipe_frames += frames;
+    e->pipe_host_topk += g ? g->n_host_topk : 0;
+    e->pipe_inflight--;
+    if (last_of_slot) {
+        a.rc = rc; a.err = err;
+        a.done = true;
+        a.from_queue = false;
+        s.pending = false;
+    }
 }
 
 bool same_work(const GroupJob& a, const GroupJob& b) {
     return a.H == b.H && a.W == b.W && a.K == b.K && memcmp(&a.p, &b.p, sizeof(fslic_params)) == 0;
+}
+
+bool may_follow(const fslic_engine* e, const Slot& s, const InFlight& prev, const GroupJob& head) {
+    if (!e->pipe_overlap.load(std::memory_order_relaxed) || e->launch_timing || s.launch_timing) return false;
+    if (!same_work(prev.job, head) || head.p.debug_mode || head.p.preemptive || head.p.variant == FSLIC_VARIANT_REALDIST_NOQ) return false;
+    if (!prepared_for(e, s, head.H, head.W, head.K, head.n)) return false;
+    for (const Slot& o : e->slots)
+        if (!o.pending && !o.busy && o.wanted == 0) return false;
+    return true;
 }
 
 void slot_worker(fslic_engine* e, Slot* s) {
     Slot::Async& a = *s->async;
     (void)hipSetDevice(e->device);
     (void)prctl(PR_SET_TIMERSLACK, 1000UL);
+    InFlight* prev = nullptr;
+    auto collect = [&](const InFlight* g, int rc, int frames, bool last_of_slot) {
+        {
+            std::lock_guard<std::mutex> lk(e->mu);
+            pipeline_collect(e, *s, g, rc, rc ? last_error() : std::string(), frames, last_of_slot);
+        }
+        e->cv.notify_all();
+    };
+    auto finish = [&](InFlight& g, InFlight* next, bool& next_done) {
+        next_done = false;
+        g.total_ms = 0; g.n_host_topk = 0;
+        int rc = group_wait(*s, g, next != nullptr);
+        if (rc == FSLIC_OK && (next || s->par != g.par) && group_needs_host(*s, g)) {
+            if (next) {
+                next->total_ms = 0; next->n_host_topk = 0;
+                int rn = group_wait(*s, *next, false);
+                if (rn == FSLIC_OK) rn = group_complete(e, *s, *next, false);
+                if (rn != FSLIC_OK) drain_failed(*s);
+                collect(next, rn, next->job.n, false);
+                next_done = true;
+            }
+            rc = make_current(*s, g);
+            if (rc == FSLIC_OK) rc = group_complete(e, *s, g, true);
+        } else if (rc == FSLIC_OK) {
+            rc = group_complete(e, *s, g, false);
+        }
+        if (rc != FSLIC_OK) drain_failed(*s);
+        return rc;
+    };
     for (;;) {
         bool took = false;
+        bool look = false;
+        if (prev) { int rc_ignored; look = group_prewait(*s, *prev, rc_ignored); }
         {
             std::unique_lock<std::mutex> lk(e->mu);
-            e->cv_work.wait(lk, [&] { return a.has_job || a.quit || (!e->pipe_q.empty() && !e->pipe_gathering && !s->busy && !s->pending && e->sync_waiters == 0 && s->wanted == 0); });
-            if (a.quit) return;
-            if (!a.has_job) {
+            auto queue_open = [&] { return !e->pipe_q.empty() && !e->pipe_gathering && !s->busy && e->sync_waiters == 0 && s->wanted == 0; };
+            e->cv_work.wait(lk, [&] { return a.has_job || a.quit || prev || (queue_open() && !s->pending); });
+            if (a.quit && !prev) return;
+            if (!a.has_job && !a.quit && queue_open() && (!prev || (look && may_follow(e, *s, *prev, e->pipe_q.front())))) {
                 GroupJob& g = a.job;
                 const int unit = e->pipe_q.front().n;
                 g = e->pipe_q.front(); g.n = 0; a.jobs = 0;
-                const int limit = std::min(e->pipe_batch_frames, (int)kMaxGroup);
+                const int limit = std::min(std::min(e->pipe_batch_frames, (int)kMaxGroup), prev ? s->cap_frames : (int)kMaxGroup);
                 auto gather = [&](int max_jobs) {
                     while (!e->pipe_q.empty() && a.jobs < max_jobs) {
                         const GroupJob& j = e->pipe_q.front();
@@ -166,11 +213,45 @@
                     gather(kMaxGroup);
                 }
                 s->launch_timing = e->launch_timing;
-                a.has_job = true;
                 took = true;
             }
         }
-        if (took) { e->cv.notify_all(); e->cv_work.notify_all(); }
+        if (took) {
+            e->cv.notify_all(); e->cv_work.notify_all();
+            s->nap_wait = true;
+            const int frames = a.job.n;
+            int rc = group_begin(e, *s, a.job);
+            InFlight* const cur = rc == FSLIC_OK ? &s->fl[s->par] : nullptr;
+            if (prev && cur) e->overlapped_groups.fetch_add(1, std::memory_order_relaxed);
+            const std::string err = rc ? last_error() : std::string();
+            if (rc != FSLIC_OK) drain_failed(*s);
+            bool cur_done = false;
+            int rp = FSLIC_OK;
+            if (prev) {
+                rp = finish(*prev, cur, cur_done);
+                collect(prev, rp, prev->job.n, cur_done);
+                prev = nullptr;
+            }
+            if (rc != FSLIC_OK) {
+                set_last_error(err);
+                collect(nullptr, rc, frames, true);
+            } else if (!cur_done) {
+                if (rp == FSLIC_OK && e->pipe_overlap.load(std::memory_order_relaxed)) prev = cur;
+                else { bool unused; const int rf = finish(*cur, nullptr, unused); collect(cur, rf, frames, true); }
+            }
+            s->nap_wait = false;
+            continue;
+        }
+        if (prev) {
+            s->nap_wait = true;
+            bool unused;
+            const int rp = finish(*prev, nullptr, unused);
+            s->nap_wait = false;
+            collect(prev, rp, prev->job.n, true);
+            prev = nullptr;
+            continue;
+        }
+        if (!a.has_job) continue;
         s->nap_wait = true;
         const int rc = run_group(e, *s, a.job);
         s->nap_wait = false;
@@ -180,11 +261,6 @@
             a.err = rc ? last_error() : std::string();
             a.has_job = false;
             a.done = true;
-            if (a.from_queue) {
-                pipeline_collect(e, *s);
-                a.from_queue = false;
-                e->pipe_inflight--;
-            }
         }
         e->cv.notify_all();
     }
@@ -304,6 +380,12 @@
     std::lock_guard<std::mutex> lk(e->mu);
     e->pipe_batch_frames = max_frames_per_group;
     e->reserve_frames.store(max_frames_per_group);
+    return FSLIC_OK;
+}
+
+int fslic_hip_pipeline_overlap(fslic_engine* e, int on) {
+    if (!e) return fail(FSLIC_E_INVALID, "engine is NULL");
+    e->pipe_overlap.store(on != 0, std::memory_order_relaxed);
     return FSLIC_OK;
 }
 
diff --git a/include/fslic_hip.h b/include/fslic_hip.h
--- a/include/fslic_hip.h
+++ b/include/fslic_hip.h
@@ -124,6 +124,10 @@
 int fslic_hip_separate_pass_redos(fslic_engine* e, int slot);
 
 int fslic_hip_uncovered_redos(fslic_engine* e, int slot);
+
+long long fslic_hip_overlapped_groups(fslic_engine* e);
+
+int fslic_hip_pipeline_overlap(fslic_engine* e, int on);
 
 int fslic_hip_debug_forms_seen(uint32_t* codes, int cap, int clear);
 int fslic_hip_debug_forms_all(uint32_t* codes, int cap);
```

New measurement: 71320 megapixels/sec (median of 6 runs). 1.03x the previous value.
